# yuriyvnv/speech_transcript_embeddings

Measured on AMD Instinct MI355X. Metric: audio–text pairs/sec (whole node), 10s@16kHz + 64-tok, 1/2/4/8 MI355X, higher is better.
Workload: dtype bf16; 1 GPU; c2: global batch 64 = 1 GPU x 1 micro-batch(es) of 64 pairs, each pair 10s@16kHz audio + 64-tok clean + 64-tok corrupt; w2v-bert-2.0 Conformer 24L + XLM-R-base 12L, 3+3 unfrozen; GPU fbank -> fwd -> InfoNCE -> bwd -> allreduce -> clip+AdamW; global_batch=64, local_batch=64, micro_batch=64, accumulation_steps=1, seq_len_audio_frames=499, seq_len_text=64, parallelism=dp1

## Files before the change

### include/ste.h

```cpp
#ifndef STE_H_
#define STE_H_
#include <stdint.h>

#ifdef __cplusplus
extern "C" {
#endif

#define STE_OK 0
#define STE_ERR_ARG 1001
#define STE_ERR_SHAPE 1002

enum {
  STE_ACT_NONE = 0,
  STE_ACT_SWISH = 1,
  STE_ACT_GELU = 2,
  STE_ACT_TANH = 3,
  STE_ACT_RELU = 4,
  STE_ACT_SWISH_BWD = 11,
  STE_ACT_GELU_BWD = 12,
  STE_ACT_TANH_BWD_OUT = 13,
  STE_ACT_RELU_BWD = 14
};

typedef struct {
  int M, N, K, batch;
  const void* A; int64_t lda; int a_kc;
  const void* B; int64_t ldb; int b_kc;
  int64_t strideA, strideB, strideC, strideR;
  void* C; int64_t ldc; int c_bf16;
  void* C2; int64_t ldc2;
  void* C3; int64_t ldc3;
  const float* bias;
  const void* R; int64_t ldr; int r_bf16;
  const void* Z; int64_t ldz;
  float* colsum;
  const float* row_scale;
  float alpha, beta;
  int act;
  float drop_p; uint64_t seed; int64_t drop_ld;
  float* ws; int64_t ws_bytes;
  int c3_lo;
} ste_gemm_args;

int ste_gemm(const ste_gemm_args* args, void* stream);
int64_t ste_gemm_colsum_ws_floats(const ste_gemm_args* args);
int ste_gemm_tile_map(int t, int num_m, int num_n, int* tm, int* tn);

int ste_gemm_f32(const ste_gemm_args* args, void* stream);
int ste_gemm_f32_plan(const ste_gemm_args* args);
int ste_gemm_f32_plan_slab(const ste_gemm_args* args);
int64_t ste_gemm_f32_ws_floats(const ste_gemm_args* args);
int ste_gemm_f32_plan_tile(const ste_gemm_args* args);
int ste_gemm_f32_plan_max_tiles(int tiles);
int ste_gemm_f32_plan_small_tiles(int tiles);

#define STE_GEMM_KERNEL_SMALL 0
#define STE_GEMM_KERNEL_8PH 8
#define STE_GEMM_KERNEL_SPLITK 12
int ste_gemm_kernel(const ste_gemm_args* args);
int ste_gemm_kernel_name(const ste_gemm_args* args, char* buf, int len);

int ste_gemm_mx8(const ste_gemm_args* args, const void* a_scales, const void* b_scales, void* q_out, void* q_scales,
                 void* stream);
int ste_gemm_mx8_kernel(const ste_gemm_args* args, int q_out);
int ste_gemm_plan_min_tiles(int bf16_tiles, int mx8_tiles, int* prev_bf16, int* prev_mx8);
int ste_mx8_quant(const void* x, int64_t ldx, int rows, int K, void* q, void* scales, void* stream);

typedef struct {
  int rows, cols;
  const void* x; int64_t ldx; int x_bf16;
  const float* gamma; const float* beta; float eps;
  float* y; int64_t ldy;
  void* yb; int64_t ldyb;
  float* mean; float* rstd;
  const float* row_scale;
  int act;
  float drop_p; uint64_t seed;
  void* q8; void* q8s; int64_t ldq8;
  void* ylo; int64_t ldylo;
} ste_ln_fwd_args;
int ste_layernorm_fwd(const ste_ln_fwd_args* a, void* stream);

typedef struct {
  int rows, cols;
  const void* dy; int64_t lddy; int dy_bf16;
  const void* x; int64_t ldx; int x_bf16;
  const float* mean; const float* rstd;
  const float* gamma; const float* beta;
  const float* row_scale;
  int act;
  const float* dres; int64_t lddres;
  float* dx; int64_t lddx;
  void* dxb; int64_t lddxb;
  float* dgamma; float* dbeta;
  float drop_p; uint64_t seed; float out_scale;
  float in_drop_p; uint64_t in_seed;
  const float* out_row_scale;
  float* dsum;
  float* ws; int64_t ws_floats;
} ste_ln_bwd_args;
int ste_layernorm_bwd(const ste_ln_bwd_args* a, void* stream);
int64_t ste_layernorm_bwd_ws_floats(int rows, int cols);

int ste_layernorm_fwd_pair(const ste_ln_fwd_args* a, const ste_ln_fwd_args* b, void* stream);
int ste_layernorm_bwd_pair(const ste_ln_bwd_args* a, const ste_ln_bwd_args* b, void* stream);

typedef struct {
  int B, T, H;
  const void* q; int64_t ldq;
  const void* k; int64_t ldk;
  const void* v; int64_t ldv;
  void* o; int64_t ldo;
  float* lse;
  const int32_t* key_mask;
  const void* rel_E; int rel_left, rel_right;
  float scale;
  float drop_p; uint64_t seed;
  const void* dout; int64_t lddo;
  void* dq; int64_t lddq;
  void* dk; int64_t lddk;
  void* dv; int64_t lddv;
  float* delta;
  float* dE;
  float* gwork;
  void* o_lo; int64_t ldolo;
  int zero_masked_rows;
} ste_attn_args;
int ste_attention_fwd(const ste_attn_args* a, void* stream);
int ste_attention_fwd_f32(const ste_attn_args* a, float* o32, int64_t ldo32, void* stream);
int ste_attention_bwd(const ste_attn_args* a, void* stream);
int ste_attention_bwd_f32(const ste_attn_args* a, void* stream);

int ste_glu_dwconv_fwd(const void* pre, const float* w, void* out, int B, int T, int C, int K, void* stream);
int ste_glu_dwconv_bwd(const void* pre, const float* w, const void* dout, void* dpre, float* dw,
                       int B, int T, int C, int K, float* ws, int64_t ws_floats, void* stream);
int64_t ste_glu_dwconv_bwd_ws_floats(int B, int T, int C, int K);

int ste_fbank(const float* wav, int64_t ld_wav, const int32_t* lengths, int B, int Tmax, float pad_value,
              float* feats, int64_t* mask, int mask_mode, float* work, void* stream);

int ste_resample_plan(int sr_in, int sr_out, int* M, int* L, int* K);
int ste_resample_table(int sr_in, int sr_out, float* table, int64_t table_floats);
int ste_resample_tile(int M, int L, int K);
int ste_resample(const float* wav, int64_t ld_wav, const int32_t* lengths, int B, int M, int L, int K,
                 const float* table, float* out, int64_t ld_out, int n_out_max, int32_t* out_lengths, void* stream);

int ste_attn_pool_fwd(const void* t, const float* w2, const float* b2, const void* h, const int32_t* mask,
                      int B, int L, int Hh, int H, float* weights, float* pooled, void* pooled_bf16,
                      void* stream);
int ste_attn_pool_bwd_work_floats(int B, int L, int Hh);
int ste_attn_pool_bwd(const void* t, const float* w2, const void* h, const float* weights, const float* dpooled,
                      const int32_t* mask, int B, int L, int Hh, int H, float* dh, void* dt, void* dt_lo, float* dw2,
                      float* db2,
                      float* db1, float* work, void* stream);
int ste_attn_pool_fwd_f32(const float* t, const float* w2, const float* b2, const float* h, const int32_t* mask,
                          int B, int L, int Hh, int H, float* weights, float* pooled, void* pooled_bf16, void* stream);
int ste_attn_pool_bwd_f32(const float* t, const float* w2, const float* h, const float* weights, const float* dpooled,
                          const int32_t* mask, int B, int L, int Hh, int H, float* dh, float* dt, float* dw2,
                          float* db2, float* db1, float* work, void* stream);

int ste_mean_pool_fwd(const void* h, const int32_t* mask, int B, int L, int H, int cls, float* weights, float* pooled,
                      void* pooled_bf16, void* stream);
int ste_mean_pool_fwd_f32(const float* h, const int32_t* mask, int B, int L, int H, int cls, float* weights,
                          float* pooled, void* pooled_bf16, void* stream);
int ste_weighted_pool_bwd(const float* weights, const float* dpooled, int B, int L, int H, float* dh, void* stream);

int ste_xattn1_fwd(const float* q, const void* k, const void* v, int64_t ldkv, const int32_t* mask, int B, int S,
                   int P, int nh, float scale, float drop_p, uint64_t seed, float* probs, float* out, void* stream);
int ste_xattn1_bwd(const float* q, const void* k, const void* v, int64_t ldkv, const float* probs, const float* dout,
                   const int32_t* mask, int B, int S, int P, int nh, float scale, float drop_p, uint64_t seed,
                   float* dq, float* dk, float* dv, int64_t lddkv, void* stream);
int ste_xattn_fwd(const float* q, const void* k, const void* v, int64_t ldkv, const int32_t* mask, int B, int S, int P,
                  int nh, int nq, float scale, float drop_p, uint64_t seed0, uint64_t seed1, float* probs, float* out,
                  void* stream);
int ste_xattn_bwd(const float* q, const void* k, const void* v, int64_t ldkv, const float* probs, const float* dout,
                  const int32_t* mask, int B, int S, int P, int nh, int nq, float scale, float drop_p,
                  uint64_t seed0, uint64_t seed1, float* dq, float* dk, float* dv, int64_t lddkv, void* stream);
int ste_xattn_mq_fwd(const float* q, const int32_t* qrow, const void* k, const void* v, int64_t ldkv,
                     const int32_t* mask, int B, int C, int S, int P, int nh, float scale, float* out, void* stream);
int ste_xattn_gather_fwd(const float* q, const int32_t* qrow, const void* k, const void* v, int64_t ldkv,
                         const int32_t* kvblk, const int32_t* mask, int R, int S, int P, int nh, float scale,
                         float* out, void* stream);
int ste_xattn_bwd_bf16(const float* q, const void* k, const void* v, int64_t ldkv, const float* probs,
                       const float* dout, const int32_t* mask, int B, int S, int P, int nh, int nq, float scale,
                       float drop_p,
                       uint64_t seed0, uint64_t seed1, float* dq, void* dk, void* dv, int64_t lddkv,
                       float* colsum_part, void* stream);

int ste_align_attn_fwd(const void* q, int64_t ldq, const void* kv, int64_t ldkv, const int32_t* kmask, int B, int L,
                       int T, int P, int nh, float drop_p, uint64_t seed, float* probs, void* out, int64_t ldo,
                       void* stream);
int ste_align_attn_bwd(const void* q, int64_t ldq, const void* kv, int64_t ldkv, const float* probs,
                       const void* dout, int64_t lddo, int B, int L, int T, int P, int nh, float drop_p,
                       uint64_t seed, float* dsbuf, void* dq, int64_t lddq, float* dkv, int64_t lddkv, void* stream);
int ste_rank1_bwd(const float* a, const float* w, const void* z, int M, int K, int act, void* out, float* dw,
                  float* db, void* stream);

int ste_l2norm_fwd(const float* x, int rows, int cols, float* y, float* norms, void* stream);
int ste_l2norm_bwd(const float* y, const float* norms, const float* dy, int rows, int cols, float* dx,
                   void* stream);
int ste_similarity(const float* a, const float* t, int B, int NT, int P, float* S, void* stream);
int ste_pair_loss_fwd(const float* S, int64_t ldS, int off_neg, const float* align, int B, int L, float tau,
                      float aw, float gamma, float* s_pos, float* s_neg, float* loss, void* stream);
int ste_pair_loss_bwd(const float* s_pos, const float* s_neg, const float* align, int B, int L, float tau,
                      float aw, float gamma, const float* gscale, float* ds_pos, float* ds_neg, float* dalign,
                      void* stream);

int ste_pair_metrics(const float* S, int64_t ldS, int NB, int off_neg, float tau, const float* losses, int nloss,
                     float loss_w, double* acc, void* stream);
int ste_inbatch_ce(const float* S, int64_t ldS, int B, int NB, int row0, float tau, float weight, const float* gscale,
                   float* loss, float* dS, int64_t lddS, void* stream);
int ste_rowmat_f32(const float* X, int64_t sxr, int64_t sxc, const float* Y, int R, int C, int P, float* out,
                   void* stream);
int ste_pair_sim_bwd(const float* a, const float* tp, const float* tn, const float* ds_pos, const float* ds_neg,
                     int B, int P, float* da, float* dtp, float* dtn, void* stream);

int ste_text_embed_fwd(const int64_t* ids, int B, int L, int D, int pad_idx, const float* word, const float* pos,
                       const float* type0, float* out, int32_t* pos_ids, void* stream);
int ste_text_embed_bwd(const int64_t* ids, const int32_t* pos_ids, const float* dout, int B, int L, int D,
                       int pad_idx, float* dword, float* dpos, float* dtype0, float* ws, int64_t ws_floats,
                       void* stream);
int64_t ste_text_embed_bwd_ws_floats(int B, int L, int D);

int ste_rows_extract(const int64_t* ids, int n, int pad_idx, float* grad, int D, int32_t* flags,
                     int32_t* out_ids, float* rows, int cap, int32_t* count, void* stream);
int ste_rows_accumulate(float* grad, int D, const int32_t* ids, const float* rows, int cap, float scale,
                        void* stream);

int ste_sumsq(const float* g, int64_t n, double* acc, double* part, void* stream);
int ste_adamw(float* p, const float* g, float* m, float* v, void* p_bf16, int64_t n, float lr, float beta1,
              float beta2, float eps, float wd, int step, const double* sumsq, float max_norm, void* stream);

int ste_split_bf16(const float* x, int64_t ldx, int64_t rows, int K, void* y, int nblk, int lo_mask, void* stream);
int ste_cast_f32_bf16(const float* x, void* y, int64_t n, void* stream);
int ste_axpby2d(float* y, int64_t ldy, const float* x, int64_t ldx, int64_t rows, int cols, float alpha, float beta,
                void* stream);
int ste_copy2d(void* y, int64_t ldy, const void* x, int64_t ldx, int64_t rows, int cols, int elem_bytes,
               void* stream);
int ste_spec_mask_fwd(float* x, int64_t ld, const int32_t* spec, const float* valid, const float* embed,
                      int64_t rows, int cols, void* stream);
int ste_spec_mask_bwd(float* dx, int64_t ld, const int32_t* spec, const float* valid, float* dembed,
                      int64_t rows, int cols, float* ws, int64_t ws_floats, void* stream);
int64_t ste_spec_mask_bwd_ws_floats(int64_t rows, int cols);
int ste_transpose16(void* y, int64_t ldy, const void* x, int64_t ldx, int64_t rows, int cols, void* stream);
int ste_colsum(const void* x, int is_bf16, int64_t rows, int cols, int64_t ld, float* out, float* ws,
               int64_t ws_floats, void* stream);
int64_t ste_colsum_ws_floats(int64_t rows, int cols);
int ste_rowsum_ordered(const float* part, int64_t rows, int cols, int batch, float* out, void* stream);
int ste_scale_rows(float* x, const float* scale, int64_t rows, int cols, int64_t ld, void* stream);
int ste_mask_i64_to_f32(const int64_t* m, float* f, int32_t* i32, int64_t n, void* stream);

int ste_w2v_conv0_fwd(const float* wave, int64_t ldw, const float* w0, int B, int N, int T0, int C, int K0, int S0,
                      float* y, void* stream);
int64_t ste_w2v_gn_work(int B, int T0, int C, int K0);
int ste_w2v_gn_fwd(const float* y, const float* gamma, const float* beta, int B, int T0, int C, float eps,
                   float* mean, float* rstd, void* h, float* work, int64_t work_floats, void* stream);
int ste_w2v_gn_bwd(const float* dh, const float* y, const float* mean, const float* rstd, const float* gamma,
                   const float* beta, const float* wave, int64_t ldw, int B, int N, int T0, int C, int K0, int S0,
                   float* dgamma, float* dbeta, float* dw0, float* work, int64_t work_floats, void* stream);
int ste_w2v_slab_sum(float* out, const float* part, int64_t n, int S, void* stream);
int ste_w2v_conv_fold(const float* dcol, int64_t ldd, const void* z, int B, int Ti, int To, int C, int k, int s,
                      void* out, int out_bf16, void* stream);
int ste_w2v_perm12(const void* src, void* dst, int A, int P, int Q, int fp32_accumulate, void* stream);
int ste_w2v_pos_pack(const float* x, int B, int T, int D, int G, int K, int padl, void* out, void* stream);
int ste_w2v_pos_elem(int mode, const float* cpad, const float* bias, const float* src, const float* maskf, int B,
                     int T, int D, int Tp, float* out, void* stream);
int ste_w2v_wnorm_fwd(const float* v, const float* g, int D, int Cg, int K, float* norms, void* wr, void* wf,
                      void* stream);
int ste_w2v_wnorm_bwd(const float* dwr, const float* v, const float* g, const float* norms, int D, int Cg, int K,
                      float* dv, float* dg, void* stream);
int ste_w2v_frame_mask(const int64_t* mask, int B, int N, int Tf, int nconv, const int* kernels, const int* strides,
                       float* maskf, int32_t* mask32, void* stream);
int ste_w2v_wave_norm(const float* wave, int64_t ldw, const int32_t* lengths, int B, int N, float pad, float* out,
                      void* stream);
int ste_w2v_drop_rows(float* x, int M, int N, float p, uint64_t seed, const float* maskf, void* stream);

int ste_w2v_conv0_ln_fwd(const float* wave, int64_t ldw, const float* w0, const float* bias, const float* gamma,
                         const float* beta, int B, int N, int T0, int C, int K0, int S0, float eps, void* h,
                         float* mean, float* rstd, void* stream);
int64_t ste_w2v_conv0_ln_work(int B, int T0, int C, int K0);
int ste_w2v_conv0_ln_bwd(const float* dh, const float* wave, int64_t ldw, const float* mean, const float* rstd,
                         const float* w0, const float* bias, const float* gamma, const float* beta, int B, int N,
                         int T0, int C, int K0, int S0, float* dgamma, float* dbeta, float* dbias, float* dw0,
                         float* work, int64_t work_floats, void* stream);
int ste_w2v_ln_gelu_fwd(const void* z, const float* gamma, const float* beta, int64_t rows, int C, float eps, void* h,
                        int h_f32, float* mean, float* rstd, void* stream);
int64_t ste_w2v_ln_gelu_work(int64_t rows, int C);
int ste_w2v_ln_gelu_bwd(const void* dh, int dh_bf16, const void* z, const float* mean, const float* rstd,
                        const float* gamma, const float* beta, int64_t rows, int C, void* dz, float* dgamma,
                        float* dbeta, float* dbias, float* work, int64_t work_floats, void* stream);

int ste_topk_sim_plan(int Q, int N, int P, int k, int splits, int* splits_out, int64_t* ws_bytes);
int ste_topk_sim(const float* q, const void* corpus, int corpus_bf16, int Q, int N, int P, int k, int index_base,
                 const int32_t* target, const float* tscore, int splits, float* values, int32_t* indices,
                 int32_t* rank, void* ws, int64_t ws_bytes, void* stream);
int ste_topk_target_score(const float* q, const void* corpus, int corpus_bf16, int Q, int N, int P, int index_base,
                          const int32_t* target, float* tscore, void* stream);
int ste_topk_merge(const float* vals, const int32_t* idx, int Q, int C, int k, const int32_t* counts, int L,
                   float* out_v, int32_t* out_i, int32_t* out_rank, void* stream);

const char* ste_version(void);

#ifdef __cplusplus
}
#endif
#endif
```

### speech_transcript_embeddings_amd/_lib.py

```python
from __future__ import annotations

import ctypes as C
import os
from pathlib import Path

import torch

_PKG = Path(__file__).resolve().parent
LIB_PATH = Path(os.environ.get("STE_LIB", _PKG / "libste.so"))
AB_BUILD = LIB_PATH.name == "libste_ab.so"


def ab_env(name: str, default: str) -> str:
    return os.environ.get(name, default) if AB_BUILD else default

c_void_p, c_int, c_int64, c_float, c_uint64, c_char_p = C.c_void_p, C.c_int, C.c_int64, C.c_float, C.c_uint64, C.c_char_p
c_i32p = C.POINTER(C.c_int32)

ACT_NONE, ACT_SWISH, ACT_GELU, ACT_TANH, ACT_RELU = 0, 1, 2, 3, 4
ACT_SWISH_BWD, ACT_GELU_BWD, ACT_TANH_BWD_OUT, ACT_RELU_BWD = 11, 12, 13, 14


class GemmArgs(C.Structure):
    _fields_ = [
        ("M", c_int), ("N", c_int), ("K", c_int), ("batch", c_int),
        ("A", c_void_p), ("lda", c_int64), ("a_kc", c_int),
        ("B", c_void_p), ("ldb", c_int64), ("b_kc", c_int),
        ("strideA", c_int64), ("strideB", c_int64), ("strideC", c_int64), ("strideR", c_int64),
        ("C", c_void_p), ("ldc", c_int64), ("c_bf16", c_int),
        ("C2", c_void_p), ("ldc2", c_int64),
        ("C3", c_void_p), ("ldc3", c_int64),
        ("bias", c_void_p),
        ("R", c_void_p), ("ldr", c_int64), ("r_bf16", c_int),
        ("Z", c_void_p), ("ldz", c_int64),
        ("colsum", c_void_p),
        ("row_scale", c_void_p),
        ("alpha", c_float), ("beta", c_float),
        ("act", c_int),
        ("drop_p", c_float), ("seed", c_uint64), ("drop_ld", c_int64),
        ("ws", c_void_p), ("ws_bytes", c_int64),
        ("c3_lo", c_int),
    ]


class LnFwdArgs(C.Structure):
    _fields_ = [
        ("rows", c_int), ("cols", c_int),
        ("x", c_void_p), ("ldx", c_int64), ("x_bf16", c_int),
        ("gamma", c_void_p), ("beta", c_void_p), ("eps", c_float),
        ("y", c_void_p), ("ldy", c_int64),
        ("yb", c_void_p), ("ldyb", c_int64),
        ("mean", c_void_p), ("rstd", c_void_p),
        ("row_scale", c_void_p),
        ("act", c_int),
        ("drop_p", c_float), ("seed", c_uint64),
        ("q8", c_void_p), ("q8s", c_void_p), ("ldq8", c_int64),
        ("ylo", c_void_p), ("ldylo", c_int64),
    ]


class LnBwdArgs(C.Structure):
    _fields_ = [
        ("rows", c_int), ("cols", c_int),
        ("dy", c_void_p), ("lddy", c_int64), ("dy_bf16", c_int),
        ("x", c_void_p), ("ldx", c_int64), ("x_bf16", c_int),
        ("mean", c_void_p), ("rstd", c_void_p),
        ("gamma", c_void_p), ("beta", c_void_p),
        ("row_scale", c_void_p),
        ("act", c_int),
        ("dres", c_void_p), ("lddres", c_int64),
        ("dx", c_void_p), ("lddx", c_int64),
        ("dxb", c_void_p), ("lddxb", c_int64),
        ("dgamma", c_void_p), ("dbeta", c_void_p),
        ("drop_p", c_float), ("seed", c_uint64), ("out_scale", c_float),
        ("in_drop_p", c_float), ("in_seed", c_uint64),
        ("out_row_scale", c_void_p),
        ("dsum", c_void_p),
        ("ws", c_void_p), ("ws_floats", c_int64),
    ]


class AttnArgs(C.Structure):
    _fields_ = [
        ("B", c_int), ("T", c_int), ("H", c_int),
        ("q", c_void_p), ("ldq", c_int64),
        ("k", c_void_p), ("ldk", c_int64),
        ("v", c_void_p), ("ldv", c_int64),
        ("o", c_void_p), ("ldo", c_int64),
        ("lse", c_void_p),
        ("key_mask", c_void_p),
        ("rel_E", c_void_p), ("rel_left", c_int), ("rel_right", c_int),
        ("scale", c_float),
        ("drop_p", c_float), ("seed", c_uint64),
        ("dout", c_void_p), ("lddo", c_int64),
        ("dq", c_void_p), ("lddq", c_int64),
        ("dk", c_void_p), ("lddk", c_int64),
        ("dv", c_void_p), ("lddv", c_int64),
        ("delta", c_void_p),
        ("dE", c_void_p),
        ("gwork", c_void_p),
        ("o_lo", c_void_p), ("ldolo", c_int64),
        ("zero_masked_rows", c_int),
    ]


_SIGS = {
    "ste_gemm": (c_int, [C.POINTER(GemmArgs), c_void_p]),
    "ste_gemm_f32": (c_int, [C.POINTER(GemmArgs), c_void_p]),
    "ste_gemm_f32_plan": (c_int, [C.POINTER(GemmArgs)]),
    "ste_gemm_f32_plan_slab": (c_int, [C.POINTER(GemmArgs)]),
    "ste_gemm_f32_ws_floats": (c_int64, [C.POINTER(GemmArgs)]),
    "ste_gemm_f32_plan_max_tiles": (c_int, [c_int]),
    "ste_gemm_f32_plan_small_tiles": (c_int, [c_int]),
    "ste_gemm_f32_plan_tile": (c_int, [C.POINTER(GemmArgs)]),
    "ste_gemm_kernel": (c_int, [C.POINTER(GemmArgs)]),
    "ste_gemm_colsum_ws_floats": (c_int64, [C.POINTER(GemmArgs)]),
    "ste_gemm_tile_map": (c_int, [c_int, c_int, c_int, C.POINTER(c_int), C.POINTER(c_int)]),
    "ste_gemm_kernel_name": (c_int, [C.POINTER(GemmArgs), c_char_p, c_int]),
    "ste_rows_extract": (c_int, [c_void_p, c_int, c_int, c_void_p, c_int, c_void_p, c_void_p, c_void_p, c_int,
                                 c_void_p, c_void_p]),
    "ste_rows_accumulate": (c_int, [c_void_p, c_int, c_void_p, c_void_p, c_int, c_float, c_void_p]),
    "ste_layernorm_fwd": (c_int, [C.POINTER(LnFwdArgs), c_void_p]),
    "ste_layernorm_bwd": (c_int, [C.POINTER(LnBwdArgs), c_void_p]),
    "ste_layernorm_fwd_pair": (c_int, [C.POINTER(LnFwdArgs), C.POINTER(LnFwdArgs), c_void_p]),
    "ste_layernorm_bwd_pair": (c_int, [C.POINTER(LnBwdArgs), C.POINTER(LnBwdArgs), c_void_p]),
    "ste_layernorm_bwd_ws_floats": (c_int64, [c_int, c_int]),
    "ste_attention_fwd": (c_int, [C.POINTER(AttnArgs), c_void_p]),
    "ste_attention_bwd": (c_int, [C.POINTER(AttnArgs), c_void_p]),
    "ste_attention_fwd_f32": (c_int, [C.POINTER(AttnArgs), c_void_p, c_int64, c_void_p]),
    "ste_attention_bwd_f32": (c_int, [C.POINTER(AttnArgs), c_void_p]),
    "ste_split_bf16": (c_int, [c_void_p, c_int64, c_int64, c_int, c_void_p, c_int, c_int, c_void_p]),
    "ste_glu_dwconv_fwd": (c_int, [c_void_p, c_void_p, c_void_p, c_int, c_int, c_int, c_int, c_void_p]),
    "ste_glu_dwconv_bwd": (c_int, [c_void_p, c_void_p, c_void_p, c_void_p, c_void_p, c_int, c_int, c_int, c_int,
                                   c_void_p, c_int64, c_void_p]),
    "ste_glu_dwconv_bwd_ws_floats": (c_int64, [c_int, c_int, c_int, c_int]),
    "ste_fbank": (c_int, [c_void_p, c_int64, c_void_p, c_int, c_int, c_float, c_void_p, c_void_p, c_int, c_void_p,
                          c_void_p]),
    "ste_resample_plan": (c_int, [c_int, c_int, C.POINTER(c_int), C.POINTER(c_int), C.POINTER(c_int)]),
    "ste_resample_table": (c_int, [c_int, c_int, c_void_p, c_int64]),
    "ste_resample_tile": (c_int, [c_int, c_int, c_int]),
    "ste_resample": (c_int, [c_void_p, c_int64, c_void_p, c_int, c_int, c_int, c_int, c_void_p, c_void_p, c_int64,
                             c_int, c_void_p, c_void_p]),
    "ste_gemm_mx8": (c_int, [c_void_p, c_void_p, c_void_p, c_void_p, c_void_p, c_void_p]),
    "ste_gemm_mx8_kernel": (c_int, [C.POINTER(GemmArgs), c_int]),
    "ste_gemm_plan_min_tiles": (c_int, [c_int, c_int, C.POINTER(c_int), C.POINTER(c_int)]),
    "ste_mx8_quant": (c_int, [c_void_p, c_int64, c_int, c_int, c_void_p, c_void_p, c_void_p]),
    "ste_attn_pool_fwd": (c_int, [c_void_p, c_void_p, c_void_p, c_void_p, c_void_p, c_int, c_int, c_int, c_int,
                                  c_void_p, c_void_p, c_void_p, c_void_p]),
    "ste_attn_pool_bwd": (c_int, [c_void_p, c_void_p, c_void_p, c_void_p, c_void_p, c_void_p, c_int, c_int, c_int,
                                  c_int, c_void_p, c_void_p, c_void_p, c_void_p, c_void_p, c_void_p, c_void_p,
                                  c_void_p]),
    "ste_attn_pool_bwd_work_floats": (c_int, [c_int, c_int, c_int]),
    "ste_attn_pool_fwd_f32": (c_int, [c_void_p, c_void_p, c_void_p, c_void_p, c_void_p, c_int, c_int, c_int, c_int,
                                      c_void_p, c_void_p, c_void_p, c_void_p]),
    "ste_attn_pool_bwd_f32": (c_int, [c_void_p, c_void_p, c_void_p, c_void_p, c_void_p, c_void_p, c_int, c_int,
                                      c_int, c_int, c_void_p, c_void_p, c_void_p, c_void_p, c_void_p, c_void_p,
                                      c_void_p]),
    "ste_mean_pool_fwd": (c_int, [c_void_p, c_void_p, c_int, c_int, c_int, c_int, c_void_p, c_void_p, c_void_p,
                                  c_void_p]),
    "ste_mean_pool_fwd_f32": (c_int, [c_void_p, c_void_p, c_int, c_int, c_int, c_int, c_void_p, c_void_p, c_void_p,
                                      c_void_p]),
    "ste_weighted_pool_bwd": (c_int, [c_void_p, c_void_p, c_int, c_int, c_int, c_void_p, c_void_p]),
    "ste_xattn1_fwd": (c_int, [c_void_p, c_void_p, c_void_p, c_int64, c_void_p, c_int, c_int, c_int, c_int, c_float,
                               c_float, c_uint64, c_void_p, c_void_p, c_void_p]),
    "ste_xattn1_bwd": (c_int, [c_void_p, c_void_p, c_void_p, c_int64, c_void_p, c_void_p, c_void_p, c_int, c_int,
                               c_int, c_int, c_float, c_float, c_uint64, c_void_p, c_void_p, c_void_p, c_int64,
                               c_void_p]),
    "ste_xattn_fwd": (c_int, [c_void_p, c_void_p, c_void_p, c_int64, c_void_p, c_int, c_int, c_int, c_int, c_int,
                              c_float, c_float, c_uint64, c_uint64, c_void_p, c_void_p, c_void_p]),
    "ste_xattn_bwd": (c_int, [c_void_p, c_void_p, c_void_p, c_int64, c_void_p, c_void_p, c_void_p, c_int, c_int,
                              c_int, c_int, c_int, c_float, c_float, c_uint64, c_uint64, c_void_p, c_void_p,
                              c_void_p, c_int64, c_void_p]),
    "ste_xattn_bwd_bf16": (c_int, [c_void_p, c_void_p, c_void_p, c_int64, c_void_p, c_void_p, c_void_p, c_int,
                                   c_int, c_int, c_int, c_int, c_float, c_float, c_uint64, c_uint64, c_void_p,
                                   c_void_p, c_void_p, c_int64, c_void_p, c_void_p]),
    "ste_xattn_mq_fwd": (c_int, [c_void_p, c_void_p, c_void_p, c_void_p, c_int64, c_void_p, c_int, c_int, c_int,
                                 c_int, c_int, c_float, c_void_p, c_void_p]),
    "ste_xattn_gather_fwd": (c_int, [c_void_p, c_void_p, c_void_p, c_void_p, c_int64, c_void_p, c_void_p, c_int,
                                     c_int, c_int, c_int, c_float, c_void_p, c_void_p]),
    "ste_align_attn_fwd": (c_int, [c_void_p, c_int64, c_void_p, c_int64, c_void_p, c_int, c_int, c_int, c_int, c_int,
                                   c_float, c_uint64, c_void_p, c_void_p, c_int64, c_void_p]),
    "ste_align_attn_bwd": (c_int, [c_void_p, c_int64, c_void_p, c_int64, c_void_p, c_void_p, c_int64, c_int, c_int,
                                   c_int, c_int, c_int, c_float, c_uint64, c_void_p, c_void_p, c_int64, c_void_p,
                                   c_int64, c_void_p]),
    "ste_rank1_bwd": (c_int, [c_void_p, c_void_p, c_void_p, c_int, c_int, c_int, c_void_p, c_void_p, c_void_p,
                              c_void_p]),
    "ste_l2norm_fwd": (c_int, [c_void_p, c_int, c_int, c_void_p, c_void_p, c_void_p]),
    "ste_l2norm_bwd": (c_int, [c_void_p, c_void_p, c_void_p, c_int, c_int, c_void_p, c_void_p]),
    "ste_similarity": (c_int, [c_void_p, c_void_p, c_int, c_int, c_int, c_void_p, c_void_p]),
    "ste_pair_loss_fwd": (c_int, [c_void_p, c_int64, c_int, c_void_p, c_int, c_int, c_float, c_float, c_float,
                                  c_void_p, c_void_p, c_void_p, c_void_p]),
    "ste_pair_loss_bwd": (c_int, [c_void_p, c_void_p, c_void_p, c_int, c_int, c_float, c_float, c_float, c_void_p,
                                  c_void_p, c_void_p, c_void_p, c_void_p]),
    "ste_pair_sim_bwd": (c_int, [c_void_p, c_void_p, c_void_p, c_void_p, c_void_p, c_int, c_int, c_void_p, c_void_p,
                                 c_void_p, c_void_p]),
    "ste_pair_metrics": (c_int, [c_void_p, c_int64, c_int, c_int, c_float, c_void_p, c_int, c_float, c_void_p,
                                 c_void_p]),
    "ste_inbatch_ce": (c_int, [c_void_p, c_int64, c_int, c_int, c_int, c_float, c_float, c_void_p, c_void_p, c_void_p,
                               c_int64, c_void_p]),
    "ste_rowmat_f32": (c_int, [c_void_p, c_int64, c_int64, c_void_p, c_int, c_int, c_int, c_void_p, c_void_p]),
    "ste_text_embed_fwd": (c_int, [c_void_p, c_int, c_int, c_int, c_int, c_void_p, c_void_p, c_void_p, c_void_p,
                                   c_void_p, c_void_p]),
    "ste_text_embed_bwd": (c_int, [c_void_p, c_void_p, c_void_p, c_int, c_int, c_int, c_int, c_void_p, c_void_p,
                                   c_void_p, c_void_p, c_int64, c_void_p]),
    "ste_text_embed_bwd_ws_floats": (c_int64, [c_int, c_int, c_int]),
    "ste_sumsq": (c_int, [c_void_p, c_int64, c_void_p, c_void_p, c_void_p]),
    "ste_adamw": (c_int, [c_void_p, c_void_p, c_void_p, c_void_p, c_void_p, c_int64, c_float, c_float, c_float,
                          c_float, c_float, c_int, c_void_p, c_float, c_void_p]),
    "ste_cast_f32_bf16": (c_int, [c_void_p, c_void_p, c_int64, c_void_p]),
    "ste_colsum": (c_int, [c_void_p, c_int, c_int64, c_int, c_int64, c_void_p, c_void_p, c_int64, c_void_p]),
    "ste_colsum_ws_floats": (c_int64, [c_int64, c_int]),
    "ste_rowsum_ordered": (c_int, [c_void_p, c_int64, c_int, c_int, c_void_p, c_void_p]),
    "ste_axpby2d": (c_int, [c_void_p, c_int64, c_void_p, c_int64, c_int64, c_int, c_float, c_float, c_void_p]),
    "ste_copy2d": (c_int, [c_void_p, c_int64, c_void_p, c_int64, c_int64, c_int, c_int, c_void_p]),
    "ste_transpose16": (c_int, [c_void_p, c_int64, c_void_p, c_int64, c_int64, c_int, c_void_p]),
    "ste_spec_mask_fwd": (c_int, [c_void_p, c_int64, c_void_p, c_void_p, c_void_p, c_int64, c_int, c_void_p]),
    "ste_spec_mask_bwd": (c_int, [c_void_p, c_int64, c_void_p, c_void_p, c_void_p, c_int64, c_int, c_void_p, c_int64,
                                  c_void_p]),
    "ste_spec_mask_bwd_ws_floats": (c_int64, [c_int64, c_int]),
    "ste_scale_rows": (c_int, [c_void_p, c_void_p, c_int64, c_int, c_int64, c_void_p]),
    "ste_mask_i64_to_f32": (c_int, [c_void_p, c_void_p, c_void_p, c_int64, c_void_p]),
    "ste_w2v_conv0_fwd": (c_int, [c_void_p, c_int64, c_void_p, c_int, c_int, c_int, c_int, c_int, c_int, c_void_p,
                                  c_void_p]),
    "ste_w2v_gn_work": (c_int64, [c_int, c_int, c_int, c_int]),
    "ste_w2v_gn_fwd": (c_int, [c_void_p, c_void_p, c_void_p, c_int, c_int, c_int, c_float, c_void_p, c_void_p,
                               c_void_p, c_void_p, c_int64, c_void_p]),
    "ste_w2v_gn_bwd": (c_int, [c_void_p, c_void_p, c_void_p, c_void_p, c_void_p, c_void_p, c_void_p, c_int64, c_int,
                               c_int, c_int, c_int, c_int, c_int, c_void_p, c_void_p, c_void_p, c_void_p, c_int64,
                               c_void_p]),
    "ste_w2v_slab_sum": (c_int, [c_void_p, c_void_p, c_int64, c_int, c_void_p]),
    "ste_w2v_conv_fold": (c_int, [c_void_p, c_int64, c_void_p, c_int, c_int, c_int, c_int, c_int, c_int, c_void_p,
                                  c_int, c_void_p]),
    "ste_w2v_perm12": (c_int, [c_void_p, c_void_p, c_int, c_int, c_int, c_int, c_void_p]),
    "ste_w2v_pos_pack": (c_int, [c_void_p, c_int, c_int, c_int, c_int, c_int, c_int, c_void_p, c_void_p]),
    "ste_w2v_pos_elem": (c_int, [c_int, c_void_p, c_void_p, c_void_p, c_void_p, c_int, c_int, c_int, c_int, c_void_p,
                                 c_void_p]),
    "ste_w2v_wnorm_fwd": (c_int, [c_void_p, c_void_p, c_int, c_int, c_int, c_void_p, c_void_p, c_void_p, c_void_p]),
    "ste_w2v_wnorm_bwd": (c_int, [c_void_p, c_void_p, c_void_p, c_void_p, c_int, c_int, c_int, c_void_p, c_void_p,
                                  c_void_p]),
    "ste_w2v_frame_mask": (c_int, [c_void_p, c_int, c_int, c_int, c_int, C.POINTER(c_int), C.POINTER(c_int), c_void_p,
                                   c_void_p, c_void_p]),
    "ste_w2v_wave_norm": (c_int, [c_void_p, c_int64, c_void_p, c_int, c_int, c_float, c_void_p, c_void_p]),
    "ste_w2v_drop_rows": (c_int, [c_void_p, c_int, c_int, c_float, c_uint64, c_void_p, c_void_p]),
    "ste_w2v_conv0_ln_fwd": (c_int, [c_void_p, c_int64, c_void_p, c_void_p, c_void_p, c_void_p, c_int, c_int, c_int,
                                     c_int, c_int, c_int, c_float, c_void_p, c_void_p, c_void_p, c_void_p]),
    "ste_w2v_conv0_ln_work": (c_int64, [c_int, c_int, c_int, c_int]),
    "ste_w2v_conv0_ln_bwd": (c_int, [c_void_p, c_void_p, c_int64, c_void_p, c_void_p, c_void_p, c_void_p, c_void_p,
                                     c_void_p, c_int, c_int, c_int, c_int, c_int, c_int, c_void_p, c_void_p,
                                     c_void_p, c_void_p, c_void_p, c_int64, c_void_p]),
    "ste_w2v_ln_gelu_fwd": (c_int, [c_void_p, c_void_p, c_void_p, c_int64, c_int, c_float, c_void_p, c_int, c_void_p,
                                    c_void_p, c_void_p]),
    "ste_w2v_ln_gelu_work": (c_int64, [c_int64, c_int]),
    "ste_w2v_ln_gelu_bwd": (c_int, [c_void_p, c_int, c_void_p, c_void_p, c_void_p, c_void_p, c_void_p, c_int64, c_int,
                                    c_void_p, c_void_p, c_void_p, c_void_p, c_void_p, c_int64, c_void_p]),
    "ste_topk_sim_plan": (c_int, [c_int, c_int, c_int, c_int, c_int, C.POINTER(c_int), C.POINTER(c_int64)]),
    "ste_topk_sim": (c_int, [c_void_p, c_void_p, c_int, c_int, c_int, c_int, c_int, c_int, c_void_p, c_void_p, c_int,
                             c_void_p, c_void_p, c_void_p, c_void_p, c_int64, c_void_p]),
    "ste_topk_target_score": (c_int, [c_void_p, c_void_p, c_int, c_int, c_int, c_int, c_int, c_void_p, c_void_p,
                                      c_void_p]),
    "ste_topk_merge": (c_int, [c_void_p, c_void_p, c_int, c_int, c_int, c_void_p, c_int, c_void_p, c_void_p, c_void_p,
                               c_void_p]),
    "ste_version": (C.c_char_p, []),
}

SYMBOLS = tuple(_SIGS)
_lib = None


class SteError(RuntimeError):
    pass


def load() -> C.CDLL:
    global _lib
    if _lib is None:
        if not LIB_PATH.exists():
            raise SteError(f"{LIB_PATH} not found — build it with __graft_entry__.build() "
                           "(speech_transcript_embeddings_amd/_build.py); there is no fallback path")
        _lib = C.CDLL(str(LIB_PATH))
    return _lib


_fns: dict = {}


def fn(name: str):
    f = _fns.get(name)
    if f is None:
        f = getattr(load(), name)
        f.restype, f.argtypes = _SIGS[name]
        _fns[name] = f
    return f


def call(name: str, *args) -> None:
    rc = fn(name)(*args)
    if rc != 0:
        raise SteError(f"{name} failed with status {rc}")


def stream_ptr(device=None) -> int:
    return torch.cuda.current_stream(device).cuda_stream


def ptr(t) -> int | None:
    return None if t is None else t.data_ptr()
```

### speech_transcript_embeddings_amd/csrc/embed_optim.hip

```cpp
#include "common.h"
#include "../../include/ste.h"

namespace {

constexpr int NT = 256;

__global__ __launch_bounds__(NT) void embed_fwd_kernel(const int64_t* ids, int L, int D, int pad, const float* word,
                                                     const float* pos, const float* type0, float* out,
                                                     int32_t* pos_ids) {
  __shared__ int spos[2048];
  const int b = blockIdx.x, tid = threadIdx.x;
  if (tid == 0) {
    int c = 0;
    for (int l = 0; l < L; ++l) {
      const int nz = ids[(int64_t)b * L + l] != pad;
      c += nz;
      spos[l] = nz ? c + pad : pad;
    }
  }
  __syncthreads();
  for (int l = tid; l < L; l += NT) pos_ids[(int64_t)b * L + l] = spos[l];
  for (int i = tid * 4; i < L * D; i += NT * 4) {
    const int l = i / D, c = i % D;
    const int64_t id = ids[(int64_t)b * L + l];
    f32x4 v = *reinterpret_cast<const f32x4*>(word + id * D + c);
    v += *reinterpret_cast<const f32x4*>(pos + (int64_t)spos[l] * D + c);
    v += *reinterpret_cast<const f32x4*>(type0 + c);
    *reinterpret_cast<f32x4*>(out + ((int64_t)b * L + l) * D + c) = v;
  }
}

constexpr int EMB_WAVES = 16;
constexpr int EMB_LDS_IDS = 16384;
template <typename IdT>
__global__ __launch_bounds__(EMB_WAVES * 64) void embed_rows_ordered_kernel(const IdT* __restrict__ ids, int rows,
                                                                          int D, int pad,
                                                                          const float* __restrict__ dout,
                                                                          float* __restrict__ table) {
  extern __shared__ int sids[];
  const bool in_lds = rows <= EMB_LDS_IDS;
  if (in_lds)
    for (int i = threadIdx.x; i < rows; i += EMB_WAVES * 64) sids[i] = (int)ids[i];
  __syncthreads();
  const int lane = threadIdx.x & 63, r = blockIdx.x * EMB_WAVES + (threadIdx.x >> 6);
  if (r >= rows) return;
  auto id_at = [&](int j) { return in_lds ? sids[j] : (int)ids[j]; };
  const int id = id_at(r);
  if (id == pad || id < 0) return;
  for (int j0 = 0; j0 < r; j0 += 64) {
    const int j = j0 + lane;
    if (__ballot(j < r && id_at(j) == id)) return;
  }
  f32x4 acc[4] = {};
  for (int j0 = r; j0 < rows; j0 += 64) {
    const int j = j0 + lane;
    uint64_t m = __ballot(j < rows && id_at(j) == id);
    while (m) {
      const int k = __builtin_ctzll(m);
      m &= m - 1;
      const float* src = dout + (int64_t)(j0 + k) * D;
#pragma unroll
      for (int q = 0; q < 4; ++q) {
        const int c = (lane + 64 * q) * 4;
        if (c < D) acc[q] += *reinterpret_cast<const f32x4*>(src + c);
      }
    }
  }
  float* dst = table + (int64_t)id * D;
#pragma unroll
  for (int q = 0; q < 4; ++q) {
    const int c = (lane + 64 * q) * 4;
    if (c < D) *reinterpret_cast<f32x4*>(dst + c) += acc[q];
  }
}

__global__ __launch_bounds__(NT) void sumsq_kernel(const float* g, int64_t n, double* acc, double* part) {
  __shared__ double red[NT / 64];
  double s = 0.0;
  float sf = 0.f;
  int cnt = 0;
  for (int64_t i = ((int64_t)blockIdx.x * NT + threadIdx.x) * 4; i < n; i += (int64_t)gridDim.x * NT * 4) {
    if (i + 3 < n) {
      const f32x4 v = *reinterpret_cast<const f32x4*>(g + i);
      sf += v[0] * v[0] + v[1] * v[1] + v[2] * v[2] + v[3] * v[3];
    } else {
      for (int64_t j = i; j < n; ++j) sf += g[j] * g[j];
    }
    if (++cnt == 64) { s += sf; sf = 0.f; cnt = 0; }
  }
  s += sf;
  s = wave_sum_d(s);
  const int w = threadIdx.x >> 6, lane = threadIdx.x & 63;
  if (lane == 0) red[w] = s;
  __syncthreads();
  if (threadIdx.x == 0) {
    double t = 0.0;
    for (int i = 0; i < NT / 64; ++i) t += red[i];
    if (part) part[blockIdx.x] = t;
    else atomicAdd(acc, t);
  }
}

__global__ __launch_bounds__(64) void sumsq_final_kernel(const double* part, int nb, double* acc) {
  double t = 0.0;
  for (int b = threadIdx.x; b < nb; b += 64) t += part[b];
  t = wave_sum_d(t);
  if (threadIdx.x == 0) acc[0] += t;
}

__device__ __forceinline__ void adamw_elem(float& p, float g, float& m, float& v, float coef, float decay, float b1,
                                           float b2, float step, float bc2_sqrt, float eps) {
#pragma clang fp contract(off)
  const float gc = g * coef;
  m = __builtin_fmaf(b1, m, (1.f - b1) * gc);
  v = __builtin_fmaf(b2, v, ((1.f - b2) * gc) * gc);
  const float den = sqrtf(v) / bc2_sqrt + eps;
  p = __builtin_fmaf(-step, m / den, p * decay);
}

template <bool NTL>
__global__ __launch_bounds__(NT) void adamw_kernel(float* __restrict__ p, const float* __restrict__ g,
                                                 float* __restrict__ m, float* __restrict__ v, bf16* __restrict__ pb,
                                                 int64_t n, float lr, float b1, float b2, float eps, float wd,
                                                 float bc1, float bc2_sqrt, const double* sumsq, float max_norm) {
  float coef = 1.f;
  if (sumsq) {
    const float tn = (float)sqrt(*sumsq);
    coef = fminf(1.f, max_norm / (tn + 1e-6f));
  }
  const float step = lr / bc1;
  const float decay = 1.f - lr * wd;
  auto upd4 = [&](f32x4& pv, const f32x4& gv, f32x4& mv, f32x4& vv) {
#pragma unroll
    for (int e = 0; e < 4; ++e) {
      float pe = pv[e], me = mv[e], ve = vv[e];
      adamw_elem(pe, gv[e], me, ve, coef, decay, b1, b2, step, bc2_sqrt, eps);
      pv[e] = pe;
      mv[e] = me;
      vv[e] = ve;
    }
  };
  auto ld = [](const float* q) -> f32x4 {
    if constexpr (NTL) return __builtin_nontemporal_load(reinterpret_cast<const f32x4*>(q));
    else return *reinterpret_cast<const f32x4*>(q);
  };
  auto st = [](float* q, f32x4 x) {
    if constexpr (NTL) __builtin_nontemporal_store(x, reinterpret_cast<f32x4*>(q));
    else *reinterpret_cast<f32x4*>(q) = x;
  };
  const int64_t stride = (int64_t)gridDim.x * NT * 4;
  int64_t i = ((int64_t)blockIdx.x * NT + threadIdx.x) * 4;
  for (; i + stride + 3 < n; i += 2 * stride) {
    f32x4 pv0 = ld(p + i), pv1 = ld(p + i + stride);
    const f32x4 gv0 = ld(g + i), gv1 = ld(g + i + stride);
    f32x4 mv0 = ld(m + i), mv1 = ld(m + i + stride);
    f32x4 vv0 = ld(v + i), vv1 = ld(v + i + stride);
    upd4(pv0, gv0, mv0, vv0);
    upd4(pv1, gv1, mv1, vv1);
    st(p + i, pv0);
    st(m + i, mv0);
    st(v + i, vv0);
    st(p + i + stride, pv1);
    st(m + i + stride, mv1);
    st(v + i + stride, vv1);
    if (pb) {
      store_bf16x4(pb + i, pv0);
      store_bf16x4(pb + i + stride, pv1);
    }
  }
  for (; i < n; i += stride) {
    if (i + 3 < n) {
      f32x4 pv = *reinterpret_cast<f32x4*>(p + i);
      const f32x4 gv = *reinterpret_cast<const f32x4*>(g + i);
      f32x4 mv = *reinterpret_cast<f32x4*>(m + i);
      f32x4 vv = *reinterpret_cast<f32x4*>(v + i);
      upd4(pv, gv, mv, vv);
      *reinterpret_cast<f32x4*>(p + i) = pv;
      *reinterpret_cast<f32x4*>(m + i) = mv;
      *reinterpret_cast<f32x4*>(v + i) = vv;
      if (pb) store_bf16x4(pb + i, pv);
    } else {
      for (int64_t j = i; j < n; ++j) {
        float pv = p[j], mv = m[j], vv = v[j];
        adamw_elem(pv, g[j], mv, vv, coef, decay, b1, b2, step, bc2_sqrt, eps);
        p[j] = pv;
        m[j] = mv;
        v[j] = vv;
        if (pb) pb[j] = (bf16)pv;
      }
    }
  }
}

inline unsigned grid_for(int64_t n) {
  int64_t b = (n / 4 + NT - 1) / NT;
  if (b > 8192) b = 8192;
  return (unsigned)(b < 1 ? 1 : b);
}

}

namespace {
__global__ __launch_bounds__(NT) void rows_reset_kernel(int32_t* out_ids, int cap, int32_t* count) {
  const int i = blockIdx.x * NT + threadIdx.x;
  if (i < cap) out_ids[i] = -1;
  if (i == 0) *count = 0;
}
__global__ __launch_bounds__(NT) void rows_claim_kernel(const int64_t* ids, int n, int pad, int32_t* flags,
                                                       int32_t* out_ids, int cap, int32_t* count) {
  const int i = blockIdx.x * NT + threadIdx.x;
  if (i >= n) return;
  const int64_t id = ids[i];
  if (id == pad || id < 0) return;
  if (atomicCAS(flags + id, 0, 1) == 0) {
    const int slot = atomicAdd(count, 1);
    if (slot < cap) out_ids[slot] = (int32_t)id;
  }
}
__global__ __launch_bounds__(NT) void rows_extract_kernel(float* grad, int D, const int32_t* out_ids, int32_t* flags,
                                                         float* rows) {
  const int sidx = blockIdx.x;
  const int id = out_ids[sidx];
  float* dst = rows + (int64_t)sidx * D;
  if (id < 0) {
    for (int c = threadIdx.x * 4; c < D; c += NT * 4) *reinterpret_cast<f32x4*>(dst + c) = f32x4{0.f, 0.f, 0.f, 0.f};
    return;
  }
  float* src = grad + (int64_t)id * D;
  for (int c = threadIdx.x * 4; c < D; c += NT * 4) {
    *reinterpret_cast<f32x4*>(dst + c) = *reinterpret_cast<const f32x4*>(src + c);
    *reinterpret_cast<f32x4*>(src + c) = f32x4{0.f, 0.f, 0.f, 0.f};
  }
  if (threadIdx.x == 0) flags[id] = 0;
}
__global__ __launch_bounds__(NT) void rows_accumulate_kernel(float* grad, int D, const int32_t* ids, const float* rows,
                                                            float scale) {
  const int sidx = blockIdx.x;
  const int id = ids[sidx];
  if (id < 0) return;
  float* dst = grad + (int64_t)id * D;
  const float* src = rows + (int64_t)sidx * D;
  for (int c = threadIdx.x * 4; c < D; c += NT * 4)
    *reinterpret_cast<f32x4*>(dst + c) += *reinterpret_cast<const f32x4*>(src + c) * scale;
}
}

extern "C" int ste_rows_extract(const int64_t* ids, int n, int pad_idx, float* grad, int D, int32_t* flags,
                                int32_t* out_ids, float* rows, int cap, int32_t* count, void* stream) {
  if (n < 0 || cap <= 0 || (D & 3) || !grad || !flags || !out_ids || !rows || !count) return STE_ERR_ARG;
  hipStream_t s = (hipStream_t)stream;
  hipLaunchKernelGGL(rows_reset_kernel, dim3((cap + NT - 1) / NT), dim3(NT), 0, s, out_ids, cap, count);
  STE_CHECK_LAUNCH();
  if (n > 0) {
    hipLaunchKernelGGL(rows_claim_kernel, dim3((n + NT - 1) / NT), dim3(NT), 0, s, ids, n, pad_idx, flags, out_ids,
                       cap, count);
    STE_CHECK_LAUNCH();
  }
  hipLaunchKernelGGL(rows_extract_kernel, dim3(cap), dim3(NT), 0, s, grad, D, out_ids, flags, rows);
  STE_CHECK_LAUNCH();
  return 0;
}

extern "C" int ste_rows_accumulate(float* grad, int D, const int32_t* ids, const float* rows, int cap, float scale,
                                   void* stream) {
  if (cap <= 0 || (D & 3) || !grad || !ids || !rows) return STE_ERR_ARG;
  hipLaunchKernelGGL(rows_accumulate_kernel, dim3(cap), dim3(NT), 0, (hipStream_t)stream, grad, D, ids, rows, scale);
  STE_CHECK_LAUNCH();
  return 0;
}



extern "C" int ste_text_embed_fwd(const int64_t* ids, int B, int L, int D, int pad_idx, const float* word,
                                  const float* pos, const float* type0, float* out, int32_t* pos_ids, void* stream) {
  if (B <= 0 || L <= 0 || L > 2048 || (D & 3)) return STE_ERR_SHAPE;
  hipLaunchKernelGGL(embed_fwd_kernel, dim3(B), dim3(NT), 0, (hipStream_t)stream, ids, L, D, pad_idx, word, pos, type0,
                     out, pos_ids);
  STE_CHECK_LAUNCH();
  return 0;
}

extern "C" int64_t ste_text_embed_bwd_ws_floats(int B, int L, int D) {
  return ste_colsum_ws_floats((int64_t)B * L, D);
}

extern "C" int ste_text_embed_bwd(const int64_t* ids, const int32_t* pos_ids, const float* dout, int B, int L, int D,
                                  int pad_idx, float* dword, float* dpos, float* dtype0, float* ws, int64_t ws_floats,
                                  void* stream) {
  const int rows = B * L;
  if (rows <= 0 || (D & 3) || D > 1024) return STE_ERR_SHAPE;
  hipStream_t s = (hipStream_t)stream;
  const dim3 grid((rows + EMB_WAVES - 1) / EMB_WAVES);
  const size_t lds = rows <= EMB_LDS_IDS ? (size_t)rows * 4 : 0;
  if (dword) {
    hipLaunchKernelGGL(embed_rows_ordered_kernel<int64_t>, grid, dim3(EMB_WAVES * 64), lds, s, ids, rows, D, pad_idx,
                       dout, dword);
    STE_CHECK_LAUNCH();
  }
  if (dpos) {
    hipLaunchKernelGGL(embed_rows_ordered_kernel<int32_t>, grid, dim3(EMB_WAVES * 64), lds, s, pos_ids, rows, D,
                       pad_idx, dout, dpos);
    STE_CHECK_LAUNCH();
  }
  if (dtype0) return ste_colsum(dout, 0, rows, D, D, dtype0, ws, ws_floats, stream);
  return 0;
}

extern "C" int ste_sumsq(const float* g, int64_t n, double* acc, double* part, void* stream) {
  if (n <= 0) return 0;
  if (((uintptr_t)g) & 15) return STE_ERR_ARG;
  unsigned gr = grid_for(n);
  if (gr > 2048) gr = 2048;
  hipLaunchKernelGGL(sumsq_kernel, dim3(gr), dim3(NT), 0, (hipStream_t)stream, g, n, acc, part);
  STE_CHECK_LAUNCH();
  if (part) {
    hipLaunchKernelGGL(sumsq_final_kernel, dim3(1), dim3(64), 0, (hipStream_t)stream, part, (int)gr, acc);
    STE_CHECK_LAUNCH();
  }
  return 0;
}

extern "C" int ste_adamw(float* p, const float* g, float* m, float* v, void* p_bf16, int64_t n, float lr, float beta1,
                         float beta2, float eps, float wd, int step, const double* sumsq, float max_norm,
                         void* stream) {
  if (n <= 0) return 0;
  if (step < 1) return STE_ERR_ARG;
  if ((((uintptr_t)p) | ((uintptr_t)g) | ((uintptr_t)m) | ((uintptr_t)v)) & 15) return STE_ERR_ARG;
  if (p_bf16 && (((uintptr_t)p_bf16) & 7)) return STE_ERR_ARG;
  const float bc1 = 1.f - powf(beta1, (float)step);
  const float bc2s = sqrtf(1.f - powf(beta2, (float)step));
  const char* ent = STE_AB_ENV("STE_ADAMW_NT");
  if (!(ent && ent[0] == '0'))
    hipLaunchKernelGGL(adamw_kernel<true>, dim3(grid_for(n)), dim3(NT), 0, (hipStream_t)stream, p, g, m, v,
                       (bf16*)p_bf16, n, lr, beta1, beta2, eps, wd, bc1, bc2s, sumsq, max_norm);
  else
  hipLaunchKernelGGL(adamw_kernel<false>, dim3(grid_for(n)), dim3(NT), 0, (hipStream_t)stream, p, g, m, v, (bf16*)p_bf16, n,
                     lr, beta1, beta2, eps, wd, bc1, bc2s, sumsq, max_norm);
  STE_CHECK_LAUNCH();
  return 0;
}
```

### speech_transcript_embeddings_amd/engine.py

```python
from __future__ import annotations

import math

import torch

from . import _lib, ops
from ._lib import (ACT_GELU, ACT_GELU_BWD, ACT_NONE, ACT_RELU, ACT_RELU_BWD, ACT_SWISH, ACT_SWISH_BWD,
                   ACT_TANH)

BF16, F32 = torch.bfloat16, torch.float32
_GOLD = 0x9E3779B97F4A7C15
_M64 = (1 << 64) - 1


def _site_seed(base: int, site: int) -> int:
    x = (base + (site + 1) * _GOLD) & _M64
    x ^= x >> 31
    return (x * 0xBF58476D1CE4E5B9) & _M64


XLMR_NAMES = dict(layer="text_encoder.encoder.layer.{i}.", q="attention.self.query", o="attention.output.dense",
                  ln1="attention.output.LayerNorm", fi="intermediate.dense", fo="output.dense", ln2="output.LayerNorm")
W2V2_NAMES = dict(layer="audio_encoder.encoder.layers.{i}.", q="attention.q_proj", o="attention.out_proj",
                  ln1="layer_norm", fi="feed_forward.intermediate_dense", fo="feed_forward.output_dense",
# ... 394 lines not shown
        ap = c.attention_probs_dropout_prob if train else 0.0
        x = self._e(M, D)
        if self.precise_text:
            xb = self._e(M, 2 * D, dtype=BF16)
            st = self._ln(emb, "text_encoder.embeddings.LayerNorm", c.layer_norm_eps, y=x, yb=xb[:, :D], ylo=xb[:, D:],
                          drop_p=hp, seed=_site_seed(base_seed, 1))
        else:
            xb = self._e(M, D, dtype=BF16)
            st = self._ln(emb, "text_encoder.embeddings.LayerNorm", c.layer_norm_eps, y=x, yb=xb, drop_p=hp,
                          seed=_site_seed(base_seed, 1))
        ctx.update(t_nb=nb, t_L=L, t_mask32=mask32, t_ids=ids, t_emb=emb, t_pos=pos_ids, t_st=st, t_hp=hp, t_ap=ap,
                   t_seed=base_seed)
        layers = []
        for i in range(c.num_hidden_layers):
            x, xb, sv = self._xlmr_fwd(i, x, xb, nb, L, mask32, hp, ap, _site_seed(base_seed, 10 + i), save)
            layers.append(sv if save else None)
        ctx["t_layers"] = layers
        return x, (xb[:, :D] if self.precise_text else xb)

    def _xlmr_fwd(self, i, x, xb, nb, L, mask32, hp, ap, seed, save=True):
        if self.precise_text:
            return self._postln_fwd_x2(self.tcfg, XLMR_NAMES, i, x, xb, nb, L, mask32, hp, ap, seed, save)
        return self._postln_fwd(self.tcfg, XLMR_NAMES, i, x, xb, nb, L, mask32, hp, ap, seed, save)

    def _xlmr_bwd(self, i, sv, dx2, nb, L, mask32, hp, ap):
        if self.precise_text and self.precise_text_bwd:
            return self._postln_bwd_x2(self.tcfg, XLMR_NAMES, i, sv, dx2, nb, L, mask32, hp, ap)
        return self._postln_bwd(self.tcfg, XLMR_NAMES, i, sv, dx2, nb, L, mask32, hp, ap)

    def _postln_fwd(self, c, nm, i, x, xb, nb, L, mask32, hp, ap, seed, save=True, act_p=0.0):
        s = self.s
        pre = nm["layer"].format(i=i)
        M, D, F_ = x.shape[0], c.hidden_size, c.intermediate_size
        H = c.num_attention_heads
        eps = c.layer_norm_eps
        tr = s.trainable_layer(pre + nm["q"] + ".weight")
        sv = {"tr": tr, "seed": seed, "act_p": act_p}
        qkv = ops.linear(xb, s.fused(pre + nm["q"] + ".weight", 3, "w"), s.fused(pre + nm["q"] + ".bias", 3, "p"),
                         out_bf16=True)
        o = self._e(M, D, dtype=BF16)
        o_lo = self._e(M, D, dtype=BF16) if save else None
        lse = self._e(nb * H * L)
        ops.attention_fwd(qkv[:, :D], qkv[:, D:2 * D], qkv[:, 2 * D:], B=nb, T=L, H=H, o=o, lse=lse,
                          key_mask=mask32, scale=1.0 / math.sqrt(D // H), drop_p=ap, seed=_site_seed(seed, 1),
                          o_lo=o_lo, zero_masked_rows=True)
        y1 = ops.linear(o, s.w(pre + nm["o"] + ".weight"), s.p(pre + nm["o"] + ".bias"),
                        residual=x, drop_p=hp, seed=_site_seed(seed, 2))
        x1 = self._e(M, D)
        x1b = self._e(M, D, dtype=BF16)
        sv["st1"] = self._ln(y1, pre + nm["ln1"], eps, y=x1, yb=x1b)
        zt = self._e(M, F_, dtype=BF16) if save else None
        h = ops.linear(x1b, s.w(pre + nm["fi"] + ".weight"), s.p(pre + nm["fi"] + ".bias"),
                       act=ACT_GELU, pre_out=zt, out_bf16=True, drop_p=act_p, seed=_site_seed(seed, 4))
        y2 = ops.linear(h, s.w(pre + nm["fo"] + ".weight"), s.p(pre + nm["fo"] + ".bias"), residual=x1, drop_p=hp,
                        seed=_site_seed(seed, 3))
        x2 = self._e(M, D)
        x2b = self._e(M, D, dtype=BF16)
        sv["st2"] = self._ln(y2, pre + nm["ln2"], eps, y=x2, yb=x2b)
        sv.update(qkv=qkv, o=o, o_lo=o_lo, lse=lse, y1=y1, zt=zt, y2=y2)
        if tr:
            sv.update(xb=xb, x1b=x1b, h=h)
        return x2, x2b, sv

    def _postln_fwd_x2(self, c, nm, i, x, xs, nb, L, mask32, hp, ap, seed, save=True, act_p=0.0):
        s = self.s
        pre = nm["layer"].format(i=i)
        M, D, F_ = x.shape[0], c.hidden_size, c.intermediate_size
        H = c.num_attention_heads
        eps = c.layer_norm_eps
        tr = s.trainable_layer(pre + nm["q"] + ".weight")
        sv = {"tr": tr, "seed": seed, "act_p": act_p}
        qkvb = self._e(M, 3 * D, dtype=BF16) if (save and not self.precise_text_bwd) else None
        qkv = ops.linear(xs, s.w2(pre + nm["q"] + ".weight", 3), s.fused(pre + nm["q"] + ".bias", 3, "p"),
                         out_bf16_copy=qkvb)
        os_ = self._e(M, 2 * D, dtype=BF16)
        lse = self._e(nb * H * L)
        ops.attention_fwd_f32(qkv[:, :D], qkv[:, D:2 * D], qkv[:, 2 * D:], B=nb, T=L, H=H, o32=None, lse=lse,
                              o=os_[:, :D], o_lo=os_[:, D:], key_mask=mask32, scale=1.0 / math.sqrt(D // H),
                              drop_p=ap, seed=_site_seed(seed, 1), zero_masked_rows=True)
        y1 = ops.linear(os_, s.w2(pre + nm["o"] + ".weight"), s.p(pre + nm["o"] + ".bias"), residual=x, drop_p=hp,
                        seed=_site_seed(seed, 2))
        x1 = self._e(M, D)
        x1s = self._e(M, 2 * D, dtype=BF16)
        sv["st1"] = self._ln(y1, pre + nm["ln1"], eps, y=x1, yb=x1s[:, :D], ylo=x1s[:, D:])
        zt = self._e(M, F_, dtype=BF16) if save else None
        hs_ = self._e(M, 2 * F_, dtype=BF16)
        ops.linear(x1s, s.w2(pre + nm["fi"] + ".weight"), s.p(pre + nm["fi"] + ".bias"), act=ACT_GELU, pre_out=zt,
                   drop_p=act_p, seed=_site_seed(seed, 4), out=hs_[:, :F_], out_bf16_copy=hs_[:, F_:], copy_lo=True)
        y2 = ops.linear(hs_, s.w2(pre + nm["fo"] + ".weight"), s.p(pre + nm["fo"] + ".bias"), residual=x1, drop_p=hp,
                        seed=_site_seed(seed, 3), ws=self.ws)
        x2 = self._e(M, D)
        x2s = self._e(M, 2 * D, dtype=BF16)
        sv["st2"] = self._ln(y2, pre + nm["ln2"], eps, y=x2, yb=x2s[:, :D], ylo=x2s[:, D:])
        if save and self.precise_text_bwd:
            sv.update(qkv=qkv, os=os_, lse=lse, y1=y1, zt=zt, y2=y2)
            if tr:
                sv.update(xs=xs, x1s=x1s, hs=hs_)
        elif save:
            sv.update(qkv=qkvb, o=os_[:, :D], o_lo=os_[:, D:], lse=lse, y1=y1, zt=zt, y2=y2)
            if tr:
                sv.update(xb=xs[:, :D], x1b=x1s[:, :D], h=hs_[:, :F_])
        return x2, x2s, sv

    def _dw2(self, dys, xs, wname, fused=1):
        g = self.s.fused(wname, fused, "g")
        if g is None:
            return
        g2 = g.view(g.shape[0], -1)
        n, k = dys.shape[1] // 2, xs.shape[1] // 2
        for dy, x in ((dys[:, :n], xs[:, :k]), (dys[:, n:], xs[:, :k]), (dys[:, :n], xs[:, k:])):
            ops.linear_dw(dy, x, out=g2, beta=1.0, ws=self.ws)

    def _postln_bwd_x2(self, c, nm, i, sv, dx2, nb, L, mask32, hp, ap):
        s = self.s
        pre = nm["layer"].format(i=i)
        M, D, F_ = dx2.shape[0], c.hidden_size, c.intermediate_size
        H = c.num_attention_heads
        tr = sv["tr"]
        seed = sv["seed"]
        dy2 = self._e(M, D)
        self._ln_bwd(dx2, sv["y2"], sv["st2"], pre + nm["ln2"], dx=dy2, drop_p=hp, seed=_site_seed(seed, 3),
                     dsum=s.g(pre + nm["fo"] + ".bias"))
        dy2s = ops.split_bf16(dy2, 2, 2)
        dzs = self._e(M, 2 * F_, dtype=BF16)
        ops.linear(dy2s, s.wt2(pre + nm["fo"] + ".weight"), act=ACT_GELU_BWD, z=sv["zt"], out=dzs[:, :F_],
                   out_bf16_copy=dzs[:, F_:], copy_lo=True, colsum=s.g(pre + nm["fi"] + ".bias"),
                   drop_p=sv["act_p"], seed=_site_seed(seed, 4), ws=self.ws)
        if tr:
            self._dw2(dy2s, sv["hs"], pre + nm["fo"] + ".weight")
        del dy2s
        dx1 = ops.linear(dzs, s.wt2(pre + nm["fi"] + ".weight"), residual=dy2, ws=self.ws)
        if tr:
            self._dw2(dzs, sv["x1s"], pre + nm["fi"] + ".weight")
        del dzs, dy2
        dy1 = self._e(M, D)
        self._ln_bwd(dx1, sv["y1"], sv["st1"], pre + nm["ln1"], dx=dy1, drop_p=hp, seed=_site_seed(seed, 2),
                     dsum=s.g(pre + nm["o"] + ".bias"))
        del dx1
        dy1s = ops.split_bf16(dy1, 2, 2)
        do = ops.linear(dy1s, s.wt2(pre + nm["o"] + ".weight"), ws=self.ws)
        if tr:
            self._dw2(dy1s, sv["os"], pre + nm["o"] + ".weight")
        del dy1s
        qkv, os_ = sv["qkv"], sv["os"]
        dqkv = self._e(M, 3 * D)
        ops.attention_bwd_f32(qkv[:, :D], qkv[:, D:2 * D], qkv[:, 2 * D:], os_[:, :D], os_[:, D:], sv["lse"], do,
                              dqkv[:, :D], dqkv[:, D:2 * D], dqkv[:, 2 * D:], B=nb, T=L, H=H, key_mask=mask32,
                              scale=1.0 / math.sqrt(D // H), drop_p=ap, seed=_site_seed(seed, 1),
                              zero_masked_rows=True)
        del do
        if tr:
            self._db(dqkv, pre + nm["q"] + ".bias", fused=3)
        dqkvs = ops.split_bf16(dqkv, 2, 2)
        del dqkv
        dx0 = ops.linear(dqkvs, s.wt2(pre + nm["q"] + ".weight", 3), residual=dy1, ws=self.ws)
        if tr:
            self._dw2(dqkvs, sv["xs"], pre + nm["q"] + ".weight", fused=3)
        return dx0

    def _postln_bwd(self, c, nm, i, sv, dx2, nb, L, mask32, hp, ap):
        s = self.s
        pre = nm["layer"].format(i=i)
        M, D = dx2.shape[0], c.hidden_size
        H = c.num_attention_heads
        tr = sv["tr"]
        seed = sv["seed"]
        dy2 = self._e(M, D)
        dy2b = self._e(M, D, dtype=BF16)
        self._ln_bwd(dx2, sv["y2"], sv["st2"], pre + nm["ln2"], dx=dy2, dxb=dy2b, drop_p=hp,
                     seed=_site_seed(seed, 3), dsum=s.g(pre + nm["fo"] + ".bias"))
        dzt = self._dx(dy2b, pre + nm["fo"] + ".weight", act=ACT_GELU_BWD, z=sv["zt"], out_bf16=True,
                       colsum=s.g(pre + nm["fi"] + ".bias"), drop_p=sv["act_p"], seed=_site_seed(seed, 4))
        if tr:
            self._dw(dy2b, sv["h"], pre + nm["fo"] + ".weight")
        del dy2b
        dx1 = self._dx(dzt, pre + nm["fi"] + ".weight", residual=dy2)
        if tr:
            self._dw(dzt, sv["x1b"], pre + nm["fi"] + ".weight")
        del dzt, dy2
        dy1 = self._e(M, D)
        dy1b = self._e(M, D, dtype=BF16)
        self._ln_bwd(dx1, sv["y1"], sv["st1"], pre + nm["ln1"], dx=dy1, dxb=dy1b, drop_p=hp,
                     seed=_site_seed(seed, 2), dsum=s.g(pre + nm["o"] + ".bias"))
        del dx1
        do = self._dx(dy1b, pre + nm["o"] + ".weight", out_bf16=True)
        if tr:
            self._dw(dy1b, sv["o"], pre + nm["o"] + ".weight")
        del dy1b
        qkv = sv["qkv"]
        dqkv = self._e(M, 3 * D, dtype=BF16)
        delta = self._e(nb * H * L)
        ops.attention_bwd(qkv[:, :D], qkv[:, D:2 * D], qkv[:, 2 * D:], sv["o"], sv["lse"], do, dqkv[:, :D],
                          dqkv[:, D:2 * D], dqkv[:, 2 * D:], B=nb, T=L, H=H, delta=delta, key_mask=mask32,
                          scale=1.0 / math.sqrt(D // H), drop_p=ap, seed=_site_seed(seed, 1), o_lo=sv["o_lo"])
        del do, delta
        dx0 = self._dx(dqkv, pre + nm["q"] + ".weight", 3, residual=dy1)
        if tr:
            self._dw(dqkv, sv["xb"], pre + nm["q"] + ".weight", fused=3)
            self._db(dqkv, pre + nm["q"] + ".bias", fused=3)
        return dx0

    def _preln_fwd(self, c, nm, i, x, nb, L, mask32, hp, ap, seed, save=True, act_p=0.0):
        s = self.s
        pre = nm["layer"].format(i=i)
        M, D, F_ = x.shape[0], c.hidden_size, c.intermediate_size
        H = c.num_attention_heads
        eps = c.layer_norm_eps
        tr = s.trainable_layer(pre + nm["q"] + ".weight")
        sv = {"tr": tr, "seed": seed, "act_p": act_p}
        a1 = self._e(M, D, dtype=BF16)
        sv["st1"] = self._ln(x, pre + nm["ln1"], eps, yb=a1)
        qkv = ops.linear(a1, s.fused(pre + nm["q"] + ".weight", 3, "w"), s.fused(pre + nm["q"] + ".bias", 3, "p"),
                         out_bf16=True)
        o = self._e(M, D, dtype=BF16)
        o_lo = self._e(M, D, dtype=BF16) if save else None
        lse = self._e(nb * H * L)
        ops.attention_fwd(qkv[:, :D], qkv[:, D:2 * D], qkv[:, 2 * D:], B=nb, T=L, H=H, o=o, lse=lse,
                          key_mask=mask32, scale=1.0 / math.sqrt(D // H), drop_p=ap, seed=_site_seed(seed, 1),
                          o_lo=o_lo, zero_masked_rows=True)
        x1 = ops.linear(o, s.w(pre + nm["o"] + ".weight"), s.p(pre + nm["o"] + ".bias"),
                        residual=x, drop_p=hp, seed=_site_seed(seed, 2))
        a2 = self._e(M, D, dtype=BF16)
        sv["st2"] = self._ln(x1, pre + nm["ln2"], eps, yb=a2)
        zt = self._e(M, F_, dtype=BF16) if save else None
        h = ops.linear(a2, s.w(pre + nm["fi"] + ".weight"), s.p(pre + nm["fi"] + ".bias"),
                       act=ACT_GELU, pre_out=zt, out_bf16=True, drop_p=act_p, seed=_site_seed(seed, 4))
        x2 = ops.linear(h, s.w(pre + nm["fo"] + ".weight"), s.p(pre + nm["fo"] + ".bias"), residual=x1, drop_p=hp,
                        seed=_site_seed(seed, 3))
        sv.update(qkv=qkv, o=o, o_lo=o_lo, lse=lse, x=x, x1=x1, zt=zt)
        if tr:
            sv.update(a1=a1, a2=a2, h=h)
        return x2, sv

    def _preln_out_grad(self, c, nm, i, sv, hp):
        pre = nm["layer"].format(i=i)
        M, D = sv["x"].shape
        return dict(dxb=self._e(M, D, dtype=BF16), drop_p=hp, seed=_site_seed(sv["seed"], 3),
                    dsum=self.s.g(pre + nm["fo"] + ".bias"))

    def _preln_bwd(self, c, nm, i, sv, dx2, dx2b, nb, L, mask32, hp, ap, below=None):
        s = self.s
        pre = nm["layer"].format(i=i)
        M, D = dx2.shape[0], c.hidden_size
        H = c.num_attention_heads
        tr = sv["tr"]
        seed = sv["seed"]
        dzt = self._dx(dx2b, pre + nm["fo"] + ".weight", act=ACT_GELU_BWD, z=sv["zt"], out_bf16=True,
                       colsum=s.g(pre + nm["fi"] + ".bias"), drop_p=sv["act_p"], seed=_site_seed(seed, 4))
        if tr:
            self._dw(dx2b, sv["h"], pre + nm["fo"] + ".weight")
        da2 = self._dx(dzt, pre + nm["fi"] + ".weight", out_bf16=True)
        if tr:
            self._dw(dzt, sv["a2"], pre + nm["fi"] + ".weight")
        del dzt
        dx1 = self._e(M, D)
        dx1b = self._e(M, D, dtype=BF16)
        self._ln_bwd(da2, sv["x1"], sv["st2"], pre + nm["ln2"], dres=dx2, dx=dx1, dxb=dx1b, drop_p=hp,
                     seed=_site_seed(seed, 2), dsum=s.g(pre + nm["o"] + ".bias"))
        del da2
        do = self._dx(dx1b, pre + nm["o"] + ".weight", out_bf16=True)
        if tr:
            self._dw(dx1b, sv["o"], pre + nm["o"] + ".weight")
        del dx1b
        qkv = sv["qkv"]
        dqkv = self._e(M, 3 * D, dtype=BF16)
        delta = self._e(nb * H * L)
        ops.attention_bwd(qkv[:, :D], qkv[:, D:2 * D], qkv[:, 2 * D:], sv["o"], sv["lse"], do, dqkv[:, :D],
                          dqkv[:, D:2 * D], dqkv[:, 2 * D:], B=nb, T=L, H=H, delta=delta, key_mask=mask32,
                          scale=1.0 / math.sqrt(D // H), drop_p=ap, seed=_site_seed(seed, 1), o_lo=sv["o_lo"])
        del do, delta
        da1 = self._dx(dqkv, pre + nm["q"] + ".weight", 3, out_bf16=True)
        if tr:
            self._dw(dqkv, sv["a1"], pre + nm["q"] + ".weight", fused=3)
            self._db(dqkv, pre + nm["q"] + ".bias", fused=3)
        del dqkv
        dx0 = self._e(M, D)
        self._ln_bwd(da1, sv["x"], sv["st1"], pre + nm["ln1"], dres=dx1, dx=dx0, **(below or {}))
        return dx0

    def text_backward(self, dh, ctx, layers_done=None):
        c = self.tcfg
        s = self.s
        nb, L = ctx["t_nb"], ctx["t_L"]
        lo = next((i for i in range(c.num_hidden_layers)
                   if s.trainable_layer(XLMR_NAMES["layer"].format(i=i) + XLMR_NAMES["q"] + ".weight")), None)
        if lo is None and layers_done is not None:
            layers_done()
        dx = dh
        for i in reversed(range(c.num_hidden_layers)):
            dx = self._xlmr_bwd(i, ctx["t_layers"][i], dx, nb, L, ctx["t_mask32"], ctx["t_hp"], ctx["t_ap"])
            ctx["t_layers"][i] = None
            if i == lo and layers_done is not None:
                layers_done()
        gw = s.g("text_encoder.embeddings.word_embeddings.weight")
        gp = s.g("text_encoder.embeddings.position_embeddings.weight")
        gt = s.g("text_encoder.embeddings.token_type_embeddings.weight")
        ln_needed = any(g is not None for g in (gw, gp, gt, s.g("text_encoder.embeddings.LayerNorm.weight")))
        if not ln_needed:
            return
        demb = self._e(dx.shape[0], c.hidden_size)
        self._ln_bwd(dx, ctx["t_emb"], ctx["t_st"], "text_encoder.embeddings.LayerNorm", dx=demb,
                     in_drop_p=ctx["t_hp"], in_seed=_site_seed(ctx["t_seed"], 1))
        if gw is not None or gp is not None or gt is not None:
            ops.text_embed_bwd(ctx["t_ids"], ctx["t_pos"], demb, c.pad_token_id, gw, gp, gt)

    def _w32(self, name):
        w = self.s.p(name)
        return w.view(w.shape[0], -1)

    def _dw32(self, dy, x, wname):
        g = self.s.g(wname)
        if g is not None:
            ops.linear_dw(dy, x, out=g.view(g.shape[0], -1), beta=1.0, ws=self.ws)

    def _db32(self, dy, bname):
        g = self.s.g(bname)
        if g is not None:
            ops.colsum(dy, g)

    def _proj_fwd(self, name, x, rows, train, seed, sv):
        s = self.s
        p_drop = self.m.dropout if train else 0.0
        zp = self._e(rows, s.slots[name + ".projection.0.weight"].shape[0])
        h = ops.linear(x, self._w32(name + ".projection.0.weight"), s.p(name + ".projection.0.bias"), act=ACT_GELU,
                       pre_out=zp, drop_p=p_drop, seed=seed)
        y = ops.linear(h, self._w32(name + ".projection.3.weight"), s.p(name + ".projection.3.bias"))
        out = self._e(rows, y.shape[1])
        st = self._ln(y, name + ".projection.4", 1e-5, y=out)
        sv.update(x=x, zp=zp, h=h, y=y, st=st, p=p_drop, seed=seed)
        return out

    def _proj_bwd(self, name, sv, dout, dx_out):
        s = self.s
        dy = self._e(*dout.shape)
        self._ln_bwd(dout, sv["y"], sv["st"], name + ".projection.4", dx=dy, dsum=s.g(name + ".projection.3.bias"))
        dz = ops.linear_dx(dy, self._w32(name + ".projection.3.weight"), act=ACT_GELU_BWD, z=sv["zp"], drop_p=sv["p"],
                           seed=sv["seed"], colsum=s.g(name + ".projection.0.bias"))
        self._dw32(dy, sv["h"], name + ".projection.3.weight")
        ops.linear_dx(dz, self._w32(name + ".projection.0.weight"), out=dx_out, beta=1.0)
        self._dw32(dz, sv["x"], name + ".projection.0.weight")

    def _pool_fwd(self, name, h, hb, mask32, nb, L, sv, hs=None):
        s = self.s
        H = h.shape[1]
        w = self._e(nb * L)
        pooled = self._e(nb, H)
        if not self.m.use_attentive_pooling:
            ops.mean_pool_fwd(h, mask32, nb, L, name == "text_pooling", w, pooled)
            sv.update(w=w)
            return pooled
        f32 = name == "text_pooling" or hb is None or hs is not None
        w2, b2 = s.p(name + ".attention.2.weight").view(-1), s.p(name + ".attention.2.bias")
        if f32:
            if hs is not None:
                t = ops.linear(hs, s.w2(name + ".attention.0.weight"), s.p(name + ".attention.0.bias"), act=ACT_TANH)
            else:
                t = ops.linear(h, self._w32(name + ".attention.0.weight"), s.p(name + ".attention.0.bias"),
                               act=ACT_TANH)
            ops.attn_pool_fwd_f32(t, w2, b2, h, mask32, nb, L, w, pooled)
            sv.update(hs=hs)
        else:
            t = ops.linear(hb, s.w(name + ".attention.0.weight"), s.p(name + ".attention.0.bias"), act=ACT_TANH,
                           out_bf16=True)
            ops.attn_pool_fwd(t, w2, b2, hb, mask32, nb, L, w, pooled)
        sv.update(t=t, w=w, h=h if f32 else hb, mask=mask32, f32=f32)
        return pooled

    def _pool_bwd(self, name, sv, dpooled, dh, nb, L):
        s = self.s
        if not self.m.use_attentive_pooling:
            ops.weighted_pool_bwd(sv["w"], dpooled, nb, L, dh)
            return
        t = sv["t"]
        gw1 = s.g(name + ".attention.0.weight")
        gw2 = s.g(name + ".attention.2.weight")
        w2 = s.p(name + ".attention.2.weight").view(-1)
        dw2 = None if gw2 is None else gw2.view(-1)
        if sv["f32"]:
            dz = self._e(*t.shape)
            ops.attn_pool_bwd_f32(t, w2, sv["h"], sv["w"], dpooled, nb, L, dh, dz, dw2, s.g(name + ".attention.2.bias"),
                                  db1=s.g(name + ".attention.0.bias"), mask=sv["mask"])
            hs = sv.get("hs")
            if hs is None:
                ops.linear_dx(dz, self._w32(name + ".attention.0.weight"), out=dh, beta=1.0)
                self._dw32(dz, sv["h"], name + ".attention.0.weight")
                return
            Hh, D = t.shape[1], hs.shape[1] // 2
            dzs = ops.split_bf16(dz, 2, 2)
            ops.linear_dx(dzs[:, :Hh], s.w(name + ".attention.0.weight"), out=dh, beta=1.0)
            if gw1 is not None:
                self._dw(dzs[:, :Hh], hs[:, :D], name + ".attention.0.weight")
                self._dw(dzs[:, Hh:], hs[:, :D], name + ".attention.0.weight")
                self._dw(dzs[:, :Hh], hs[:, D:], name + ".attention.0.weight")
            return
        dz = self._e(*t.shape, dtype=BF16)
        dz_lo = self._e(*t.shape, dtype=BF16) if gw1 is not None else None
        ops.attn_pool_bwd(t, w2, sv["h"], sv["w"], dpooled, nb, L, dh, dz, dw2, s.g(name + ".attention.2.bias"),
                          db1=s.g(name + ".attention.0.bias"), dz_lo=dz_lo, mask=sv["mask"])
        ops.linear_dx(dz, s.w(name + ".attention.0.weight"), out=dh, beta=1.0)
        self._dw(dz, sv["h"], name + ".attention.0.weight")
        if dz_lo is not None:
            self._dw(dz_lo, sv["h"], name + ".attention.0.weight")

    def _xq_fwd(self, name, qin, kv, mask32, B, S, seeds, p_x):
        s = self.s
        rows, P = qin.shape
        nh = self.m.xattn_heads
        q = ops.linear(qin, self._w32(name + ".query.weight"), s.p(name + ".query.bias"))
        probs = self._e(rows * nh * S)
        att = self._e(rows, P)
        ops.xattn_fwd(q, kv[:, :P], kv[:, P:], mask32, B, S, nh, probs, att, seeds, drop_p=p_x)
        cat = self._e(rows, 2 * P)
        ops.linear(att, self._w32(name + ".out_proj.weight"), s.p(name + ".out_proj.bias"), out=cat[:, P:])
        ops.copy2d(cat[:, :P], qin)
        return cat, dict(qin=qin, q=q, probs=probs, att=att, cat=cat, kv=kv, mask=mask32, B=B, S=S, seeds=seeds, p=p_x)

    def _xq_bwd(self, name, xs, dcat, d_qin, dkvb):
        s = self.s
        P = d_qin.shape[1]
        datt = dcat[:, P:]
        _add_(d_qin, dcat[:, :P])
        dq_in = ops.linear_dx(datt, self._w32(name + ".out_proj.weight"))
        self._dw32(datt, xs["att"], name + ".out_proj.weight")
        self._db32(datt, name + ".out_proj.bias")
        dq = self._e(*xs["q"].shape)
        kv = xs["kv"]
        ops.xattn_bwd(xs["q"], kv[:, :P], kv[:, P:], xs["probs"], dq_in, xs["B"], xs["S"], self.m.xattn_heads, dq,
                      dkvb[:, :P], dkvb[:, P:], xs["seeds"], drop_p=xs["p"],
                      colsum=s.fused(name + ".key.bias", 2, "g") if dkvb.dtype == BF16 else None, mask=xs["mask"])
        ops.linear_dx(dq, self._w32(name + ".query.weight"), out=d_qin, beta=1.0)
        self._dw32(dq, xs["qin"], name + ".query.weight")
        self._db32(dq, name + ".query.bias")

    def _kv_src_bwd(self, name, src, dkvb, seqb, xb, dx):
        s = self.s
        if dkvb.dtype == F32:
            P2 = dkvb.shape[1]
            dkvs = ops.split_bf16(dkvb, 2, 2)
            self._db(dkvb, name + ".key.bias", fused=2)
            self._dw(dkvs[:, :P2], seqb, name + ".key.weight", fused=2)
            self._dw(dkvs[:, P2:], seqb, name + ".key.weight", fused=2)
            dseq = ops.linear(dkvs, s.wt2(name + ".key.weight", 2), colsum=s.g(src + ".bias"))
            P = dseq.shape[1]
            dseqs = ops.split_bf16(dseq, 2, 2)
            self._dw(dseqs[:, :P], xb, src + ".weight")
            self._dw(dseqs[:, P:], xb, src + ".weight")
            ops.linear(dseqs, s.wt2(src + ".weight"), out=dx, beta=1.0)
            return
        dseqb = self._dx(dkvb, name + ".key.weight", 2, out_bf16=True, colsum=s.g(src + ".bias"))
        self._dw(dkvb, seqb, name + ".key.weight", fused=2)
        self._dx(dseqb, src + ".weight", out=dx, beta=1.0)
        self._dw(dseqb, xb, src + ".weight")

    def _fuse_fwd(self, name, cat):
        y = ops.linear(cat, self._w32(name + ".0.weight"), self.s.p(name + ".0.bias"))
        out = self._e(*y.shape)
        st = self._ln(y, name + ".1", 1e-5, y=out)
        return out, (y, st, cat)

    def _fuse_bwd(self, name, d_out, saved):
        y, st, cat = saved
        dy = self._e(*d_out.shape)
        self._ln_bwd(d_out, y, st, name + ".1", dx=dy, dsum=self.s.g(name + ".0.bias"))
        dcat = ops.linear_dx(dy, self._w32(name + ".0.weight"))
        self._dw32(dy, cat, name + ".0.weight")
        return dcat

    def _kv(self, name, src, xb):
        s = self.s
        seqb = ops.linear(xb, s.w(src + ".weight"), s.p(src + ".bias"), out_bf16=True)
        kv = ops.linear(seqb, s.fused(name + ".key.weight", 2, "w"), s.fused(name + ".key.bias", 2, "p"), out_bf16=True)
        return kv, seqb

    def heads_forward(self, th, thb, ah, ahb, train, base_seed, ctx):
        self._await_params("late", "text")
        m = self.m
        nb, L = ctx["t_nb"], ctx["t_L"]
        b = nb // 2
        ab, T = ctx["a_b"], ctx["a_T"]
        hs = {}
        tpool_sv, apool_sv, tproj_sv, aproj_sv = {}, {}, {}, {}
        tpooled = self._pool_fwd("text_pooling", th, thb, ctx["t_mask32"], nb, L, tpool_sv)
        apooled = self._pool_fwd("audio_pooling", ah, ahb, ctx["a_mask32"], ab, T, apool_sv, hs=ctx.get("a_hs"))
        tproj = self._proj_fwd("text_projection", tpooled, nb, train, _site_seed(base_seed, 201), tproj_sv)
        aproj = self._proj_fwd("audio_projection", apooled, ab, train, _site_seed(base_seed, 202), aproj_sv)
        hs.update(tpool=tpool_sv, apool=apool_sv, tproj=tproj_sv, aproj=aproj_sv)
        if m.use_cross_modal:
            p_x = m.dropout if train else 0.0
            kva, aseqb = self._kv("text_to_audio_attention", "audio_seq_to_projection", ahb)
            seed_t = _site_seed(base_seed, 203)
            tcat, hs["tx"] = self._xq_fwd("text_to_audio_attention", tproj, kva, ctx["a_mask32"], b, T,
                                          (_site_seed(seed_t, 0), _site_seed(seed_t, 1)), p_x)
            kvt, tseqb = self._kv("audio_to_text_attention", "text_seq_to_projection", thb[: b * L])
            acat, hs["ax"] = self._xq_fwd("audio_to_text_attention", aproj[:b], kvt, ctx["t_mask32"][: b * L], b, L,
                                          (_site_seed(base_seed, 204),), p_x)
            tfused, hs["tf"] = self._fuse_fwd("text_fusion", tcat)
            afused, hs["af"] = self._fuse_fwd("audio_fusion", acat)
            hs.update(aseqb=aseqb, tseqb=tseqb)
        else:
            tfused, afused = tproj, aproj[:b]
        align = None
        if m.use_word_alignment:
            align = self._align_fwd(th, thb[: b * L], ahb, b, L, T, ctx, train, _site_seed(base_seed, 205), hs)
        ctx["heads"] = hs
        return tfused, afused, align

    def heads_backward(self, d_tfused, d_afused, d_align, ctx, dth, dah):
        m = self.m
        hs = ctx["heads"]
        nb, L = ctx["t_nb"], ctx["t_L"]
        b = nb // 2
        ab, T = ctx["a_b"], ctx["a_T"]
        P = m.projection_dim
        d_tproj = self._z(nb, P)
        d_aproj = self._z(ab, P)
        if d_align is not None and m.use_word_alignment:
            self._align_bwd(d_align, hs, ctx, dth, dah)
        if m.use_cross_modal:
            dtcat = self._fuse_bwd("text_fusion", d_tfused, hs["tf"])
            dacat = self._fuse_bwd("audio_fusion", d_afused, hs["af"])
            dkvb = self._e(ab * T, 2 * P, dtype=BF16)
            self._xq_bwd("text_to_audio_attention", hs["tx"], dtcat, d_tproj, dkvb)
            self._kv_src_bwd("text_to_audio_attention", "audio_seq_to_projection", dkvb, hs["aseqb"], ctx["_ahb"],
                             dah)
            del dkvb
            dkvtb = self._e(b * L, 2 * P, dtype=BF16)
            self._xq_bwd("audio_to_text_attention", hs["ax"], dacat, d_aproj[:b], dkvtb)
            self._kv_src_bwd("audio_to_text_attention", "text_seq_to_projection", dkvtb, hs["tseqb"],
                             ctx["_thb"][: b * L], dth[: b * L])
        else:
            _add_(d_tproj, d_tfused)
            _add_(d_aproj[:b], d_afused)
        dtpooled = self._z(nb, self.tcfg.hidden_size)
        dapooled = self._z(ab, self.acfg.hidden_size)
        self._proj_bwd("text_projection", hs["tproj"], d_tproj, dtpooled)
        self._proj_bwd("audio_projection", hs["aproj"], d_aproj, dapooled)
        self._pool_bwd("text_pooling", hs["tpool"], dtpooled, dth, nb, L)
        self._pool_bwd("audio_pooling", hs["apool"], dapooled, dah, ab, T)

    def _mask32(self, mask_i64, n):
        m = self._e(n, dtype=torch.int32)
        _lib.call("ste_mask_i64_to_f32", mask_i64.contiguous().data_ptr(), None, m.data_ptr(), n, _lib.stream_ptr())
        return m

    def cross_forward(self, tproj, th, tmask, aproj, ah, amask, train, seed):
        m = self.m
        b, L, Ht = th.shape
        T, Ha = ah.shape[1], ah.shape[2]
        p_x = m.dropout if train else 0.0
        thb = ops.cast_bf16(th.contiguous(), self._e(b * L, Ht, dtype=BF16))
        ahb = ops.cast_bf16(ah.contiguous(), self._e(b * T, Ha, dtype=BF16))
        tm32 = self._mask32(tmask, b * L) if tmask is not None else None
        if amask is not None and self.raw_audio and amask.shape[-1] != T:
            from .wav2vec2 import frame_mask
            am32 = frame_mask(self.acfg, amask, b, amask.shape[-1], T, self.s.device)[1]
        else:
            am32 = self._mask32(amask, b * T) if amask is not None else None
        kva, aseqb = self._kv("text_to_audio_attention", "audio_seq_to_projection", ahb)
        tcat, tx = self._xq_fwd("text_to_audio_attention", tproj.float().contiguous(), kva, am32, b, T,
                                (_site_seed(seed, 1),), p_x)
        kvt, tseqb = self._kv("audio_to_text_attention", "text_seq_to_projection", thb)
        acat, ax = self._xq_fwd("audio_to_text_attention", aproj.float().contiguous(), kvt, tm32, b, L,
                                (_site_seed(seed, 2),), p_x)
        tfused, tf = self._fuse_fwd("text_fusion", tcat)
        afused, af = self._fuse_fwd("audio_fusion", acat)
        sv = dict(b=b, L=L, T=T, thb=thb, ahb=ahb, aseqb=aseqb, tseqb=tseqb, tx=tx, ax=ax, tf=tf, af=af)
        return tfused, afused, sv

    @torch.no_grad()
    def score_pairs(self, tproj, th, tmask, aproj, ah, amask, candidates, audio_context=None):
        m, dev = self.m, self.s.device
        U, L, Ht = th.shape
        B, T, Ha = ah.shape
        P = m.projection_dim
        cand = candidates.to(dev, torch.int32).contiguous()
        if cand.dim() != 2 or cand.shape[0] != B or cand.shape[1] < 1:
            raise ValueError(f"candidates must be [{B}, C >= 1], got {tuple(cand.shape)}")
        C = cand.shape[1]
        lo, hi = (int(x) for x in torch.stack((cand.min(), cand.max())).tolist())
        if lo < -1 or hi >= U:
            raise ValueError(f"candidates must lie in [-1, {U}), got [{lo}, {hi}]")
        if audio_context is not None and not 0 <= int(audio_context) < C:
            raise ValueError(f"audio_context must be a column of candidates, got {audio_context}")
        R = B * C
        slot = cand.view(-1)
        tproj, aproj = tproj.float().contiguous(), aproj.float().contiguous()
        scores = torch.full((R,), float("-inf"), device=dev, dtype=F32)

        def unit(x):
            y = self._e(*x.shape)
            ops.l2norm_fwd(x, y, self._e(x.shape[0]))
            return y

        arep = torch.arange(B, device=dev, dtype=torch.int32).repeat_interleave(C)
        if not m.use_cross_modal:
            ops.topk_target_score(unit(aproj).index_select(0, arep.long()), unit(tproj), slot, scores)
            return scores.view(B, C)
        nh = m.xattn_heads
        thb = ops.cast_bf16(th.contiguous(), self._e(U * L, Ht, dtype=BF16))
        ahb = ops.cast_bf16(ah.contiguous(), self._e(B * T, Ha, dtype=BF16))
        tm32 = self._mask32(tmask, U * L) if tmask is not None else None
        if amask is not None and self.raw_audio and amask.shape[-1] != T:
            from .wav2vec2 import frame_mask
            am32 = frame_mask(self.acfg, amask, B, amask.shape[-1], T, dev)[1]
        else:
            am32 = self._mask32(amask, B * T) if amask is not None else None
        kva, _ = self._kv("text_to_audio_attention", "audio_seq_to_projection", ahb)
# ... 132 lines not shown
```

### speech_transcript_embeddings_amd/ops.py

```python
from __future__ import annotations

import ctypes as C
import os

import torch

from . import _lib
from ._lib import GemmArgs, LnFwdArgs, LnBwdArgs, AttnArgs, ptr, call, fn

BF16 = torch.bfloat16
F32 = torch.float32


def _s():
    return _lib.stream_ptr()


def _ld(t: torch.Tensor) -> int:
    assert t.dim() >= 2 and t.stride(-1) == 1, "row-major operand required"
    return t.stride(-2)


ATOMIC_SUMS = _lib.ab_env("STE_ATOMIC_SUMS", "0") == "1"
_WS = {}
# ... 412 lines not shown
def fbank(wav, lengths, Tmax, *, pad_value=1.0, mask_mode=0, feats=None, mask=None, work=None):
    B = wav.shape[0]
    dev = wav.device
    if feats is None:
        feats = torch.empty((B, Tmax, 160), device=dev, dtype=F32)
    if mask is None:
        mask = torch.empty((B, Tmax), device=dev, dtype=torch.int64)
    if work is None:
        work = torch.empty(B * 2 * Tmax * 80 + B * 160, device=dev, dtype=F32)
    nbytes = 4 * B * wav.shape[1] + _nb(feats) + _nb(mask)
    _traced("fbank", nbytes, lambda: call("ste_fbank", ptr(wav), wav.stride(0), ptr(lengths), B, Tmax,
                                          float(pad_value), ptr(feats), ptr(mask), int(mask_mode), ptr(work), _s()))
    return feats, mask


def resample_plan(sr_in, sr_out=16000):
    M, L, K = C.c_int(), C.c_int(), C.c_int()
    call("ste_resample_plan", int(sr_in), int(sr_out), C.byref(M), C.byref(L), C.byref(K))
    return M.value, L.value, K.value


def resampled_length(n, sr_in, sr_out=16000):
    if sr_in == sr_out:
        return int(n)
    M, L, _ = resample_plan(sr_in, sr_out)
    return (int(n) * L + M - 1) // M


def resample_tile(sr_in, sr_out=16000):
    return fn("ste_resample_tile")(*resample_plan(sr_in, sr_out))


_RESAMPLE_TABLES = {}


def _resample_table(sr_in, sr_out, dev):
    key = (int(sr_in), int(sr_out), dev)
    t = _RESAMPLE_TABLES.get(key)
    if t is None:
        _, L, K = resample_plan(sr_in, sr_out)
        host = torch.empty(L * K, dtype=F32)
        call("ste_resample_table", int(sr_in), int(sr_out), host.data_ptr(), host.numel())
        t = _RESAMPLE_TABLES[key] = host.to(dev)
    return t


def resample(wav, lengths, sr_in, sr_out=16000, *, out=None):
    if int(sr_in) == int(sr_out):
        return wav, lengths
    M, L, K = resample_plan(sr_in, sr_out)
    B, N = wav.shape
    dev = wav.device
    if not wav.is_cuda or lengths.device != dev or lengths.shape != (B,):
        raise ValueError("resample expects wav [B, N] and lengths [B] on the same GPU")
    assert wav.dtype == F32 and wav.stride(1) == 1 and lengths.dtype == torch.int32 and lengths.is_contiguous()
    if out is None:
        out = torch.empty((B, (N * L + M - 1) // M), device=dev, dtype=F32)
    assert out.device == dev and out.dtype == F32 and out.shape[0] == B and (out.shape[1] <= 1 or out.stride(1) == 1)
    if B == 0 or N == 0 or out.shape[1] == 0:
        return out.zero_(), torch.zeros(B, device=dev, dtype=torch.int32)
    out_lengths = torch.empty(B, device=dev, dtype=torch.int32)
    table = _resample_table(sr_in, sr_out, dev)
    call("ste_resample", ptr(wav), wav.stride(0), ptr(lengths), B, M, L, K, ptr(table), ptr(out),
         out.stride(0), out.shape[1], ptr(out_lengths), _s())
    return out, out_lengths


def attn_pool_fwd(t, w2, b2, h, mask, B, L, weights, pooled, pooled_bf16=None):
    call("ste_attn_pool_fwd", ptr(t), ptr(w2), ptr(b2), ptr(h), ptr(mask), B, L, t.shape[-1], h.shape[-1],
         ptr(weights), ptr(pooled), ptr(pooled_bf16), _s())


def attn_pool_fwd_f32(t, w2, b2, h, mask, B, L, weights, pooled, pooled_bf16=None):
    assert t.dtype == F32 and h.dtype == F32
    call("ste_attn_pool_fwd_f32", ptr(t), ptr(w2), ptr(b2), ptr(h), ptr(mask), B, L, t.shape[-1], h.shape[-1],
         ptr(weights), ptr(pooled), ptr(pooled_bf16), _s())


def attn_pool_bwd_f32(t, w2, h, weights, dpooled, B, L, dh, dz, dw2=None, db2=None, db1=None, mask=None):
    assert t.dtype == F32 and h.dtype == F32 and dz.dtype == F32
    nwork = fn("ste_attn_pool_bwd_work_floats")(B, L, t.shape[-1])
    if nwork < 0:
        raise _lib.SteError(f"ste_attn_pool_bwd_work_floats failed with status {nwork}")
    work = torch.empty(nwork, device=t.device, dtype=F32)
    call("ste_attn_pool_bwd_f32", ptr(t), ptr(w2), ptr(h), ptr(weights), ptr(dpooled), ptr(mask), B, L, t.shape[-1],
         h.shape[-1], ptr(dh), ptr(dz), ptr(dw2), ptr(db2), ptr(db1), ptr(work), _s())


def attn_pool_bwd(t, w2, h, weights, dpooled, B, L, dh, dz, dw2=None, db2=None, db1=None, dz_lo=None, mask=None):
    nwork = fn("ste_attn_pool_bwd_work_floats")(B, L, t.shape[-1])
    if nwork < 0:
        raise _lib.SteError(f"ste_attn_pool_bwd_work_floats failed with status {nwork}")
    work = torch.empty(nwork, device=t.device, dtype=F32)
    call("ste_attn_pool_bwd", ptr(t), ptr(w2), ptr(h), ptr(weights), ptr(dpooled), ptr(mask), B, L, t.shape[-1],
         h.shape[-1], ptr(dh), ptr(dz), ptr(dz_lo), ptr(dw2), ptr(db2), ptr(db1), ptr(work), _s())


def mean_pool_fwd(h, mask, B, L, cls, weights, pooled, pooled_bf16=None):
    if h.dtype == F32:
        call("ste_mean_pool_fwd_f32", ptr(h), ptr(mask), B, L, h.shape[-1], int(bool(cls)), ptr(weights), ptr(pooled),
             ptr(pooled_bf16), _s())
        return
    call("ste_mean_pool_fwd", ptr(h), ptr(mask), B, L, h.shape[-1], int(bool(cls)), ptr(weights), ptr(pooled),
         ptr(pooled_bf16), _s())


def weighted_pool_bwd(weights, dpooled, B, L, dh):
    call("ste_weighted_pool_bwd", ptr(weights), ptr(dpooled), B, L, dh.shape[-1], ptr(dh), _s())


def xattn1_fwd(q, k, v, mask, B, S, nh, probs, out, drop_p=0.0, seed=0):
    P = q.shape[-1]
    call("ste_xattn1_fwd", ptr(q), ptr(k), ptr(v), _ld(k), ptr(mask), B, S, P, nh, float((P // nh) ** -0.5),
         float(drop_p), int(seed) & (2**64 - 1), ptr(probs), ptr(out), _s())


def xattn1_bwd(q, k, v, probs, dout, B, S, nh, dq, dk, dv, drop_p=0.0, seed=0, colsum=None, mask=None):
    if dk.dtype == BF16:
        return xattn_bwd(q, k, v, probs, dout, B, S, nh, dq, dk, dv, (seed,), drop_p=drop_p, colsum=colsum,
                         mask=mask)
    P = q.shape[-1]
    assert _ld(dk) == _ld(dv)
    call("ste_xattn1_bwd", ptr(q), ptr(k), ptr(v), _ld(k), ptr(probs), ptr(dout), ptr(mask), B, S, P, nh,
         float((P // nh) ** -0.5), float(drop_p), int(seed) & (2**64 - 1), ptr(dq), ptr(dk), ptr(dv), _ld(dk), _s())


def xattn_fwd(q, k, v, mask, B, S, nh, probs, out, seeds, drop_p=0.0):
    P = q.shape[-1]
    nq = len(seeds)
    assert q.shape[0] == nq * B and out.shape[0] == nq * B and probs.numel() >= nq * B * nh * S
    call("ste_xattn_fwd", ptr(q), ptr(k), ptr(v), _ld(k), ptr(mask), B, S, P, nh, nq, float((P // nh) ** -0.5),
         float(drop_p), int(seeds[0]) & (2**64 - 1), int(seeds[-1]) & (2**64 - 1), ptr(probs), ptr(out), _s())


def xattn_mq_fwd(q, qrow, k, v, mask, B, C, S, nh, out):
    P = q.shape[-1]
    assert q.dtype == F32 and q.is_contiguous() and qrow.dtype == torch.int32 and qrow.numel() == B * C
    assert k.dtype == BF16 and v.dtype == BF16 and _ld(k) == _ld(v) and k.shape[0] >= B * S
    assert out.dtype == F32 and out.is_contiguous() and out.shape == (B * C, P)
    assert mask is None or (mask.dtype == torch.int32 and mask.numel() == B * S)
    call("ste_xattn_mq_fwd", ptr(q), ptr(qrow), ptr(k), ptr(v), _ld(k), ptr(mask), B, C, S, P, nh,
         float((P // nh) ** -0.5), ptr(out), _s())


def xattn_gather_fwd(q, qrow, k, v, kvblk, mask, R, S, nh, out):
    P = q.shape[-1]
    assert q.dtype == F32 and q.is_contiguous() and out.dtype == F32 and out.shape == (R, P) and out.is_contiguous()
    assert qrow.dtype == torch.int32 and kvblk.dtype == torch.int32 and qrow.numel() == R and kvblk.numel() == R
    assert k.dtype == BF16 and v.dtype == BF16 and _ld(k) == _ld(v)
    assert mask is None or mask.dtype == torch.int32
    call("ste_xattn_gather_fwd", ptr(q), ptr(qrow), ptr(k), ptr(v), _ld(k), ptr(kvblk), ptr(mask), R, S, P, nh,
         float((P // nh) ** -0.5), ptr(out), _s())


def xattn_bwd(q, k, v, probs, dout, B, S, nh, dq, dk, dv, seeds, drop_p=0.0, colsum=None, mask=None):
    P = q.shape[-1]
    nq = len(seeds)
    assert _ld(dk) == _ld(dv) and q.shape[0] == nq * B and dq.shape[0] == nq * B and dout.shape[0] == nq * B
    if dk.dtype == BF16:
        assert dv.dtype == BF16
        part = torch.empty(B, 2 * P, device=q.device, dtype=F32)
        call("ste_xattn_bwd_bf16", ptr(q), ptr(k), ptr(v), _ld(k), ptr(probs), ptr(dout), ptr(mask), B, S, P, nh, nq,
             float((P // nh) ** -0.5), float(drop_p), int(seeds[0]) & (2**64 - 1), int(seeds[-1]) & (2**64 - 1),
             ptr(dq), ptr(dk), ptr(dv), _ld(dk), ptr(part), _s())
        if colsum is not None:
            w = _red_ws(q.device, int(fn("ste_colsum_ws_floats")(B, 2 * P)))
            call("ste_colsum", ptr(part), 0, B, 2 * P, 2 * P, ptr(colsum), *_ws_args(w), _s())
        return
    assert colsum is None
    call("ste_xattn_bwd", ptr(q), ptr(k), ptr(v), _ld(k), ptr(probs), ptr(dout), ptr(mask), B, S, P, nh, nq,
         float((P // nh) ** -0.5), float(drop_p), int(seeds[0]) & (2**64 - 1), int(seeds[-1]) & (2**64 - 1),
         ptr(dq), ptr(dk), ptr(dv), _ld(dk), _s())


def align_attn_fwd(q, kv, kmask, B, L, T, nh, probs, out, drop_p=0.0, seed=0):
    P = kv.shape[-1] // 2
    call("ste_align_attn_fwd", ptr(q), _ld(q), ptr(kv), _ld(kv), ptr(kmask), B, L, T, P, nh, float(drop_p),
         int(seed) & (2**64 - 1), ptr(probs), ptr(out), _ld(out), _s())


def align_attn_bwd(q, kv, probs, dout, B, L, T, nh, dsbuf, dq, dkv, drop_p=0.0, seed=0):
    P = kv.shape[-1] // 2
    call("ste_align_attn_bwd", ptr(q), _ld(q), ptr(kv), _ld(kv), ptr(probs), ptr(dout), _ld(dout), B, L, T, P, nh,
         float(drop_p), int(seed) & (2**64 - 1), ptr(dsbuf), ptr(dq), _ld(dq), ptr(dkv), _ld(dkv), _s())


def rank1_bwd(a, w, z, act, out, dw=None, db=None):
    M, K = z.shape
    call("ste_rank1_bwd", ptr(a), ptr(w), ptr(z), M, K, int(act), ptr(out), ptr(dw), ptr(db), _s())


def l2norm_fwd(x, y, norms):
    call("ste_l2norm_fwd", ptr(x), x.shape[0], x.shape[1], ptr(y), ptr(norms), _s())


def l2norm_bwd(y, norms, dy, dx):
    call("ste_l2norm_bwd", ptr(y), ptr(norms), ptr(dy), y.shape[0], y.shape[1], ptr(dx), _s())


def similarity(a, t, S):
    call("ste_similarity", ptr(a), ptr(t), a.shape[0], t.shape[0], a.shape[1], ptr(S), _s())


def topk_sim_plan(Q, N, P, k, splits=0):
    s, b = C.c_int(), C.c_int64()
    call("ste_topk_sim_plan", int(Q), int(N), int(P), int(k), int(splits), C.byref(s), C.byref(b))
    return s.value, b.value


def _corpus(corpus, P):
    if corpus.dtype not in (F32, BF16):
        raise TypeError(f"corpus must be fp32 or bf16, got {corpus.dtype}")
    if corpus.dim() != 2 or corpus.shape[1] != P or not corpus.is_contiguous():
        raise ValueError(f"corpus must be contiguous [N, {P}], got {tuple(corpus.shape)}")
    return int(corpus.dtype == BF16)


def topk_sim(q, corpus, k, *, index_base=0, target=None, tscore=None, splits=0):
    Q, P = q.shape
    assert q.dtype == F32 and q.is_contiguous()
    bf = _corpus(corpus, P)
    N = corpus.shape[0]
    _, ws_bytes = topk_sim_plan(Q, N, P, k, splits)
    dev = q.device
    values = torch.empty(Q, k, device=dev, dtype=F32)
    indices = torch.empty(Q, k, device=dev, dtype=torch.int32)
    ranks = None
    if target is not None:
        assert target.dtype == torch.int32 and target.shape == (Q,) and target.is_contiguous()
        assert tscore is None or (tscore.dtype == F32 and tscore.shape == (Q,) and tscore.is_contiguous())
        ranks = torch.empty(Q, device=dev, dtype=torch.int32)
    ws = torch.empty(ws_bytes, device=dev, dtype=torch.uint8)
    call("ste_topk_sim", ptr(q), ptr(corpus), bf, Q, N, P, int(k), int(index_base), ptr(target), ptr(tscore),
         int(splits), ptr(values), ptr(indices), ptr(ranks), ptr(ws), ws_bytes, _s())
    return (values, indices) if ranks is None else (values, indices, ranks)


def topk_target_score(q, corpus, target, tscore, *, index_base=0):
    Q, P = q.shape
    bf = _corpus(corpus, P)
    call("ste_topk_target_score", ptr(q), ptr(corpus), bf, Q, corpus.shape[0], P, int(index_base), ptr(target),
         ptr(tscore), _s())
    return tscore


def topk_merge(values, indices, k, counts=None):
    Q, Cn = values.shape
    assert values.dtype == F32 and indices.dtype == torch.int32 and indices.shape == values.shape
    values, indices = values.contiguous(), indices.contiguous()
    ov = torch.empty(Q, k, device=values.device, dtype=F32)
    oi = torch.empty(Q, k, device=values.device, dtype=torch.int32)
    ranks, L = None, 0
    if counts is not None:
        assert counts.dtype == torch.int32 and counts.shape[0] == Q
        counts, L = counts.contiguous(), counts.shape[1]
        ranks = torch.empty(Q, device=values.device, dtype=torch.int32)
    call("ste_topk_merge", ptr(values), ptr(indices), Q, Cn, int(k), ptr(counts), L, ptr(ov), ptr(oi), ptr(ranks), _s())
    return (ov, oi) if ranks is None else (ov, oi, ranks)


def pair_loss_fwd(S, off_neg, align, B, L, tau, aw, gamma, s_pos, s_neg, loss):
    call("ste_pair_loss_fwd", ptr(S), _ld(S), off_neg, ptr(align), B, L, float(tau), float(aw), float(gamma),
         ptr(s_pos), ptr(s_neg), ptr(loss), _s())


def pair_loss_bwd(s_pos, s_neg, align, B, L, tau, aw, gamma, gscale, ds_pos, ds_neg, dalign=None):
    call("ste_pair_loss_bwd", ptr(s_pos), ptr(s_neg), ptr(align), B, L, float(tau), float(aw), float(gamma),
         ptr(gscale), ptr(ds_pos), ptr(ds_neg), ptr(dalign), _s())


def pair_sim_bwd(a, tp, tn, ds_pos, ds_neg, da, dtp, dtn):
    call("ste_pair_sim_bwd", ptr(a), ptr(tp), ptr(tn), ptr(ds_pos), ptr(ds_neg), a.shape[0], a.shape[1], ptr(da),
         ptr(dtp), ptr(dtn), _s())


def pair_metrics(S, off_neg, tau, acc, losses=None, loss_w=1.0):
    call("ste_pair_metrics", ptr(S), _ld(S), S.shape[0], int(off_neg), float(tau), ptr(losses),
         0 if losses is None else losses.numel(), float(loss_w), ptr(acc), _s())


def inbatch_ce(S, B, NB, row0, tau, weight, gscale, loss, dS):
    call("ste_inbatch_ce", ptr(S), _ld(S), B, NB, int(row0), float(tau), float(weight), ptr(gscale), ptr(loss),
         ptr(dS), _ld(dS), _s())


def rowmat(X, Y, out, transpose_x=False):
    if transpose_x:
        C, R = X.shape
        sxr, sxc = X.stride(1), X.stride(0)
    else:
        R, C = X.shape
        sxr, sxc = X.stride(0), X.stride(1)
    assert Y.shape[0] == C and Y.is_contiguous() and out.shape == (R, Y.shape[1]) and out.is_contiguous()
    call("ste_rowmat_f32", ptr(X), sxr, sxc, ptr(Y), R, C, Y.shape[1], ptr(out), _s())
    return out


def text_embed_fwd(ids, pad_idx, word, pos, type0, out, pos_ids):
    B, L = ids.shape
    call("ste_text_embed_fwd", ptr(ids), B, L, word.shape[1], pad_idx, ptr(word), ptr(pos), ptr(type0), ptr(out),
         ptr(pos_ids), _s())


def text_embed_bwd(ids, pos_ids, dout, pad_idx, dword, dpos, dtype0):
    B, L = ids.shape
    ws = _red_ws(dout.device, int(fn("ste_text_embed_bwd_ws_floats")(B, L, dout.shape[-1]))) if dtype0 is not None \
        else None
    call("ste_text_embed_bwd", ptr(ids), ptr(pos_ids), ptr(dout), B, L, dout.shape[-1], pad_idx, ptr(dword),
         ptr(dpos), ptr(dtype0), *_ws_args(ws), _s())


SUMSQ_PARTS = 2048


def sumsq(g, acc, part=None):
    if ATOMIC_SUMS:
        part = None
    assert part is None or (part.dtype == torch.float64 and part.numel() >= SUMSQ_PARTS)
    _traced("sumsq", 4 * g.numel(), lambda: call("ste_sumsq", ptr(g), g.numel(), ptr(acc), ptr(part), _s()))


def adamw(p, g, m, v, p_bf16, *, lr, beta1, beta2, eps, wd, step, sumsq_acc=None, max_norm=1.0):
    nbytes = p.numel() * (28 + (2 if p_bf16 is not None else 0))
    _traced("adamw", nbytes, lambda: call("ste_adamw", ptr(p), ptr(g), ptr(m), ptr(v), ptr(p_bf16), p.numel(), float(lr),
                                          float(beta1), float(beta2), float(eps), float(wd), int(step), ptr(sumsq_acc),
                                          float(max_norm), _s()))


def cast_bf16(x, y):
    call("ste_cast_f32_bf16", ptr(x), ptr(y), x.numel(), _s())
    return y


def axpby(y, x, alpha=1.0, beta=1.0):
    y2 = y if y.dim() == 2 else y.view(1, -1)
    x2 = x if x.dim() == 2 else x.view(1, -1)
    assert y2.shape == x2.shape and y.dtype == F32 and x.dtype == F32
    call("ste_axpby2d", ptr(y2), _ld(y2), ptr(x2), _ld(x2), y2.shape[0], y2.shape[1], float(alpha), float(beta), _s())
    return y


def copy2d(dst, src):
    assert dst.shape == src.shape and dst.dtype == src.dtype
    d2 = dst if dst.dim() == 2 else dst.view(1, -1)
    s2 = src if src.dim() == 2 else src.view(1, -1)
    call("ste_copy2d", ptr(d2), _ld(d2), ptr(s2), _ld(s2), d2.shape[0], d2.shape[1], dst.element_size(), _s())
    return dst


def spec_mask_fwd(x, spec, valid, embed):
    call("ste_spec_mask_fwd", ptr(x), _ld(x), ptr(spec), ptr(valid), ptr(embed), x.shape[0], x.shape[1], _s())


def spec_mask_bwd(dx, spec, valid, dembed=None):
    ws = _red_ws(dx.device, int(fn("ste_spec_mask_bwd_ws_floats")(dx.shape[0], dx.shape[1]))) if dembed is not None \
        else None
    call("ste_spec_mask_bwd", ptr(dx), _ld(dx), ptr(spec), ptr(valid), ptr(dembed), dx.shape[0], dx.shape[1],
         *_ws_args(ws), _s())


def transpose16(src, dst=None):
    assert src.dim() == 2 and src.stride(1) == 1 and src.element_size() == 2
    rows, cols = src.shape
    if dst is None:
        dst = torch.empty(cols, rows, device=src.device, dtype=src.dtype)
    assert dst.shape == (cols, rows) and dst.stride(1) == 1 and dst.dtype == src.dtype
    call("ste_transpose16", ptr(dst), _ld(dst), ptr(src), _ld(src), rows, cols, _s())
    return dst


def colsum(x, out):
    ws = _red_ws(x.device, int(fn("ste_colsum_ws_floats")(x.shape[0], x.shape[1])))
    call("ste_colsum", ptr(x), int(x.dtype == BF16), x.shape[0], x.shape[1], _ld(x), ptr(out), *_ws_args(ws), _s())
    return out


def rows_extract(ids, pad_idx, grad2d, flags, out_ids, rows, count):
    assert ids.dtype == torch.int64 and grad2d.dtype == F32 and rows.shape[0] == out_ids.numel()
    call("ste_rows_extract", ptr(ids), ids.numel(), int(pad_idx), ptr(grad2d), grad2d.shape[1], ptr(flags),
         ptr(out_ids), ptr(rows), out_ids.numel(), ptr(count), _s())


def rows_accumulate(grad2d, ids, rows, scale):
    call("ste_rows_accumulate", ptr(grad2d), grad2d.shape[1], ptr(ids), ptr(rows), ids.numel(), float(scale), _s())
```

### speech_transcript_embeddings_amd/store.py

```python
from __future__ import annotations

from dataclasses import dataclass

import torch

from . import ops

ALIGN = 8


def _fuse_groups(names):
    groups = {}
    sets = [("attention.self.query", "attention.self.key", "attention.self.value"),
            ("self_attn.linear_q", "self_attn.linear_k", "self_attn.linear_v"),
            ("attention.q_proj", "attention.k_proj", "attention.v_proj"),
            ("_attention.key", "_attention.value")]
    nameset = set(names)
    for n in names:
        for trio in sets:
            for leaf in ("weight", "bias"):
                head = trio[0] + "." + leaf
                if n.endswith(head):
                    prefix = n[: -len(head)]
                    grp = tuple(prefix + t + "." + leaf for t in trio)
                    if all(g in nameset for g in grp):
                        for g in grp:
                            groups[g] = grp
    return groups


@dataclass
class Slot:
    name: str
    offset: int
    numel: int
    shape: tuple
    segment: str

    @property
    def has_grad(self) -> bool:
        return self.segment in ("enc", "head")


@dataclass(frozen=True)
class Form:
    source: str
    build: object
    prebuilt: bool = False


def _twice(wt, old):
    n, k = wt.shape
    dst = old if old is not None else torch.empty((n, 2 * k), device=wt.device, dtype=wt.dtype)
    ops.copy2d(dst[:, :k], wt)
    ops.copy2d(dst[:, k:], wt)
    return dst


def _mx8(src, old):
    return ops.mx8_quant(src, *(old or (None, None)))


FORMS = {"wt": Form("shadow", lambda w, old: ops.transpose16(w, old), prebuilt=True),
         "w2": Form("master", lambda p, old: ops.split_bf16(p, 2, 0, old), prebuilt=True),
         "wt2": Form("wt", _twice),
         "wq": Form("shadow", _mx8),
         "wtq": Form("wt", _mx8)}


class ParamStore:
    def __init__(self, model: torch.nn.Module, device, has_grad: set[str]):
        named = list(model.named_parameters())
        names = [n for n, _ in named]
        params = dict(named)
        groups = _fuse_groups(names)

        def seg_of(n, p):
            if not p.requires_grad:
                return "frozen"
            if n not in has_grad:
                return "nograd"
            return "enc" if ("text_encoder" in n or "audio_encoder" in n) else "head"

        order = {"enc": [], "head": [], "nograd": [], "frozen": []}
        seen = set()
        for n, p in named:
            if n in seen:
                continue
            grp = groups.get(n, (n,))
            segs = {seg_of(g, params[g]) for g in grp}
            if len(segs) != 1:
                grp = (n,)
            for g in grp:
                order[seg_of(g, params[g])].append(g)
                seen.add(g)
        self.slots: dict[str, Slot] = {}
        off = 0
        self.seg_range = {}
        for seg in ("enc", "head", "nograd", "frozen"):
            start = off
            for n in order[seg]:
                p = params[n]
                grp = groups.get(n)
                if grp is None or n == grp[0]:
                    off = (off + ALIGN - 1) // ALIGN * ALIGN
                self.slots[n] = Slot(n, off, p.numel(), tuple(p.shape), seg)
                off += p.numel()
            off = (off + ALIGN - 1) // ALIGN * ALIGN
            self.seg_range[seg] = (start, off)
        self.numel = off
        self.n_grad = self.seg_range["head"][1]
        self.device = torch.device(device)
        self.master = torch.zeros(self.numel, device=self.device, dtype=torch.float32)
        self.shadow = torch.zeros(self.numel, device=self.device, dtype=torch.bfloat16)
        self.grad = torch.zeros(self.n_grad, device=self.device, dtype=torch.float32)
        for n, s in self.slots.items():
            p = params[n]
            view = self.master[s.offset:s.offset + s.numel].view(s.shape)
            if p.device.type != "meta":
                with torch.no_grad():
                    view.copy_(p.detach().to(self.device, torch.float32))
            owner, leaf = (model.get_submodule(n.rsplit(".", 1)[0]), n.rsplit(".", 1)[1]) if "." in n \
                else (model, n)
            newp = torch.nn.Parameter(view, requires_grad=p.requires_grad)
            owner._parameters[leaf] = newp
            params[n] = newp
        self.params = params
        self._versions = {}
        self._cache = {form: {} for form in FORMS}
        self._members = {}
        self.opt_epoch = 0
        self._prebuilt = None
        self.sync_shadow(force=True)

    def p(self, name):
        s = self.slots[name]
        return self.master[s.offset:s.offset + s.numel].view(s.shape)

    def w(self, name, rows=None):
        s = self.slots[name]
        v = self.shadow[s.offset:s.offset + s.numel]
        return v.view(s.shape[0], -1) if rows is None else v.view(rows, -1)

    def g(self, name):
        s = self.slots[name]
        if not s.has_grad:
            return None
        return self.grad[s.offset:s.offset + s.numel].view(s.shape)

    def fused(self, first: str, count: int, which: str):
        s = self.slots[first]
        n = s.numel * count
        if which == "w":
            return self.shadow[s.offset:s.offset + n].view(s.shape[0] * count, -1)
        if which == "p":
            base = self.master[s.offset:s.offset + n]
            return base.view(s.shape[0] * count, *s.shape[1:]) if len(s.shape) > 1 else base
        if not s.has_grad:
            return None
        base = self.grad[s.offset:s.offset + n]
        return base.view(s.shape[0] * count, *s.shape[1:]) if len(s.shape) > 1 else base

    def _token(self, name, count):
        names = self._members.get((name, count))
        if names is None:
            s = self.slots[name]
            names = self._members[name, count] = (name,) if count == 1 else tuple(
                n for n, t in self.slots.items() if s.offset <= t.offset < s.offset + s.numel * count)
        return tuple(self.params[n]._version for n in names), self.opt_epoch if self.slots[name].has_grad else None

    def _form(self, form, name, count):
        f = FORMS[form]
        if f.source == "wt":
            src, _, token = self._form("wt", name, count)
        else:
            token = self._token(name, count)
        ent = self._cache[form].get((name, count))
        if ent is not None:
            if f.prebuilt:
                self._wait_prebuilt()
            if ent[1] == token:
                return ent
        if f.source != "wt":
            src = self.fused(name, count, "w" if f.source == "shadow" else "p").flatten(1)
        old, builds = (ent[0], ent[2]) if ent is not None else (None, 0)
        ent = self._cache[form][name, count] = (f.build(src, old), token, builds + 1)
        return ent

    def _wait_prebuilt(self):
        if self._prebuilt is None:
            return
        ev, stream, waited = self._prebuilt
        cur = torch.cuda.current_stream(self.device)
        if cur.cuda_stream != stream.cuda_stream and cur.cuda_stream not in waited:
            cur.wait_event(ev)
            waited.add(cur.cuda_stream)

    def cached(self, form: str) -> int:
        return len(self._cache[form])

    def wt(self, name: str, count: int = 1):
        return self._form("wt", name, count)[0]

    def w2(self, name: str, count: int = 1):
        return self._form("w2", name, count)[0]

    def wt2(self, name: str, count: int = 1):
        return self._form("wt2", name, count)[0]

    def wq(self, name: str, count: int = 1):
        return self._form("wq", name, count)[0]

    def wtq(self, name: str, count: int = 1):
        return self._form("wtq", name, count)[0]

    def _stale_prebuilt(self, inside=lambda slot: True):
        return [(form, *key) for form, f in FORMS.items() if f.prebuilt
                for key, ent in self._cache[form].items()
                if self.slots[key[0]].has_grad and ent[1][1] != self.opt_epoch and inside(self.slots[key[0]])]

    def refresh_transposes(self, stream):
        if stream is None or self.device.type != "cuda":
            return
        stale = self._stale_prebuilt()
        if not stale:
            return
        stream.wait_stream(torch.cuda.current_stream(self.device))
        self._prebuilt = None
        with torch.cuda.stream(stream):
            for key in stale:
                self._form(*key)
            ev = torch.cuda.Event()
            ev.record(stream)
        self._prebuilt = (ev, stream, set())

    def refresh_transposes_in(self, runs):
        if self.device.type != "cuda":
            return
        self._prebuilt = None
        for key in self._stale_prebuilt(lambda slot: any(a <= slot.offset < b for a, b in runs)):
            self._form(*key)

    def trainable_layer(self, name: str) -> bool:
        return self.slots[name].has_grad

    def sync_shadow(self, force=False):
        if self.device.type != "cuda":
            return
        for n, s in self.slots.items():
            v = self.params[n]._version
            if force or self._versions.get(n) != v:
                src = self.master[s.offset:s.offset + s.numel]
                dst = self.shadow[s.offset:s.offset + s.numel]
                ops.cast_bf16(src, dst)
                self._versions[n] = self.params[n]._version

    def mark_synced(self):
        for n in self.slots:
            self._versions[n] = self.params[n]._version
        self.opt_epoch += 1

    def attach_grads(self):
        names = [n for n, s in self.slots.items() if s.has_grad]
        reset = any(self.params[n].grad is None for n in names)
        if reset:
            self.grad.zero_()
            for n in names:
                self.params[n].grad = self.g(n)
        return reset
```

### speech_transcript_embeddings_amd/train.py

```python
from __future__ import annotations

import math

import torch
import torch.distributed as dist

from . import _lib, ops
from .model import EnhancedAudioTextModel

F32 = torch.float32


class LinearWarmupSchedule:

    def __init__(self, warmup: int, total: int):
        self.warmup, self.total, self.step_count = warmup, total, 0

    def factor(self, step=None):
        s = self.step_count if step is None else step
        if s < self.warmup:
            return s / max(1, self.warmup)
        return max(0.0, (self.total - s) / max(1, self.total - self.warmup))

    def step(self):
        self.step_count += 1


class FusedAdamW:

    def __init__(self, model: EnhancedAudioTextModel, lr=2.1e-3, encoder_lr_div=50.0, weight_decay=0.01,
                 betas=(0.9, 0.999), eps=1e-8, max_norm=1.0):
        st = model.store
        self.model = model
        self.store = st
        self.partial = getattr(model, "freeze_encoders", "partial") == "partial"
        div = encoder_lr_div if self.partial else 1.0
        self.groups = [{"range": st.seg_range["enc"], "lr": lr / div},
                       {"range": st.seg_range["head"], "lr": lr}]
        self.wd, self.betas, self.eps, self.max_norm = weight_decay, betas, eps, max_norm
        self.exp_avg = torch.zeros(st.n_grad, device=st.device, dtype=F32)
        self.exp_avg_sq = torch.zeros(st.n_grad, device=st.device, dtype=F32)
        self.sumsq = torch.zeros(1, device=st.device, dtype=torch.float64)
        self.sumsq_part = torch.zeros(ops.SUMSQ_PARTS, device=st.device, dtype=torch.float64)
        self.t = 0
        self.last_factor = 1.0
        self.tail = None

    def sync(self):
        if self.tail is not None:
            torch.cuda.current_stream(self.store.device).wait_event(self.tail)

    def _ref_groups(self):
        named = [(n, p) for n, p in self.model.named_parameters() if p.requires_grad]
        if not self.partial:
            return [[n for n, _ in named]]
        enc = [n for n, _ in named if "text_encoder" in n or "audio_encoder" in n]
        rest = [n for n, _ in named if not ("text_encoder" in n or "audio_encoder" in n)]
        return [enc, rest]

    def _group_hparams(self, gi):
        base = self.groups[0]["lr"] if (self.partial and gi == 0) else self.groups[1]["lr"]
        return {"lr": base * self.last_factor, "weight_decay": self.wd, "betas": tuple(self.betas), "eps": self.eps,
                "amsgrad": False, "maximize": False, "foreach": None, "capturable": False, "differentiable": False,
                "fused": None, "decoupled_weight_decay": True, "initial_lr": base}

    def state_dict(self, lr_factor: float | None = None):
        if lr_factor is not None:
            saved, self.last_factor = self.last_factor, lr_factor
            try:
                return self.state_dict()
            finally:
                self.last_factor = saved
        self.sync()
        st = self.store
        state, groups, idx = {}, [], 0
        for gi, names in enumerate(self._ref_groups()):
            ids = []
            for n in names:
                s = st.slots[n]
                if self.t > 0 and s.has_grad:
                    sl = slice(s.offset, s.offset + s.numel)
                    state[idx] = {"step": torch.tensor(float(self.t), dtype=F32),
                                  "exp_avg": self.exp_avg[sl].view(s.shape).clone(),
                                  "exp_avg_sq": self.exp_avg_sq[sl].view(s.shape).clone()}
                ids.append(idx)
                idx += 1
            groups.append({**self._group_hparams(gi), "params": ids})
        return {"state": state, "param_groups": groups}

    def load_state_dict(self, sd):
        st = self.store
        self.sync()
        ref = self._ref_groups()
        pgs = sd["param_groups"]
        if len(pgs) != len(ref) or any(len(g["params"]) != len(r) for g, r in zip(pgs, ref)):
            raise ValueError("optimizer state_dict does not match this model's parameter groups "
                             f"({[len(g['params']) for g in pgs]} vs {[len(r) for r in ref]})")
        steps = set()
        self.exp_avg.zero_()
        self.exp_avg_sq.zero_()
        for g, names in zip(pgs, ref):
            for i, n in zip(g["params"], names):
                ps = sd["state"].get(i)
                if ps is None:
                    continue
                s = st.slots[n]
                if not s.has_grad:
                    continue
                sl = slice(s.offset, s.offset + s.numel)
                self.exp_avg[sl].copy_(ps["exp_avg"].reshape(-1).to(self.exp_avg.device, F32))
                self.exp_avg_sq[sl].copy_(ps["exp_avg_sq"].reshape(-1).to(self.exp_avg_sq.device, F32))
                steps.add(int(float(ps["step"])))
        if len(steps) > 1:
            raise ValueError(f"parameters at different step counts {sorted(steps)}: not supported by the fused "
                             "optimizer (one shared step)")
        self.t = steps.pop() if steps else 0
        bases = [g.get("initial_lr", g["lr"]) for g in pgs]
        if self.partial:
            self.groups[0]["lr"], self.groups[1]["lr"] = bases[0], bases[1]
            self.last_factor = pgs[1]["lr"] / bases[1] if bases[1] else 1.0
        else:
            self.groups[0]["lr"] = self.groups[1]["lr"] = bases[0]
            self.last_factor = pgs[0]["lr"] / bases[0] if bases[0] else 1.0
        g0 = pgs[0]
        self.wd, self.betas, self.eps = float(g0["weight_decay"]), tuple(g0["betas"]), float(g0["eps"])

    def total_norm(self):
        self.sync()
        return math.sqrt(float(self.sumsq.item()))

    def step(self, lr_factor: float = 1.0, phases=None, on_phase=None):
        st = self.store
        self.t += 1
        self.last_factor = lr_factor
        self.sumsq.zero_()
        if self.max_norm is not None:
            ops.sumsq(st.grad[: st.n_grad], self.sumsq, self.sumsq_part)

        def upd(a, b, lr):
            ops.adamw(st.master[a:b], st.grad[a:b], self.exp_avg[a:b], self.exp_avg_sq[a:b], st.shadow[a:b],
                      lr=lr * lr_factor, beta1=self.betas[0], beta2=self.betas[1], eps=self.eps, wd=self.wd,
                      step=self.t, sumsq_acc=self.sumsq if self.max_norm is not None else None,
                      max_norm=self.max_norm or 1.0)
        events = {}
        if phases is None:
            for gr in self.groups:
                a, b = gr["range"]
                if b > a:
                    upd(a, b, gr["lr"])
            st.mark_synced()
            return events
        st.mark_synced()
        for name, runs in phases:
            for a, b in runs:
                gr = next(g for g in self.groups if g["range"][0] <= a and b <= g["range"][1])
                upd(a, b, gr["lr"])
            if on_phase is not None:
                on_phase(runs)
            ev = torch.cuda.Event()
            ev.record()
            events[name] = ev
        return events

    def zero_grad(self):
        self.sync()
        self.store.grad.zero_()


class GradSync:

    WORDS = "text_encoder.embeddings.word_embeddings.weight"
    STAGES = ("heads", "audio_layers", "audio", "text_layers", "text")

    def __init__(self, store, bucket_mb: int = 256, pad_id: int = 1, word_capacity: int | None = None):
        self.store = store
        self.bucket = max(1, bucket_mb * 1024 * 1024 // 4)
        self.pad_id = pad_id
        self.works = []
        self.sparse = None
        self.capacity = None if word_capacity is None else int(word_capacity)
        self.configured = word_capacity is not None
        self._agreed = False
        self._pending_cap = None
        self._cap_stream = None
        grad_slots = [sl for sl in store.slots.values() if sl.has_grad]

        ordered = sorted(grad_slots, key=lambda x: x.offset)

        def span(pred):
            runs, cur = [], None
            for x in ordered:
                if pred(x):
                    cur = [x.offset, x.offset + x.numel] if cur is None else [cur[0], x.offset + x.numel]
                elif cur is not None:
                    runs.append(tuple(cur))
                    cur = None
            if cur is not None:
                runs.append(tuple(cur))
            return runs

        words = store.slots.get(self.WORDS)
        self.words = words if words is not None and words.segment == "enc" else None
        self.ranges = {"heads": span(lambda x: x.segment == "head"),
                       "audio_layers": span(lambda x: x.segment == "enc" and
                                            x.name.startswith("audio_encoder.encoder.layers.")),
                       "audio": span(lambda x: x.segment == "enc" and x.name.startswith("audio_encoder.") and
                                     not x.name.startswith("audio_encoder.encoder.layers.")),
                       "text_layers": span(lambda x: x.segment == "enc" and
                                           x.name.startswith("text_encoder.encoder.layer.")),
                       "text": span(lambda x: x.segment == "enc" and x.name.startswith("text_encoder.") and
                                    not x.name.startswith("text_encoder.encoder.layer."))}
        if self.words is not None and self.ranges["text"]:
            w0, w1 = self.words.offset, self.words.offset + self.words.numel
            cut = []
            for a, b in self.ranges["text"]:
                cut += [r for r in ((a, min(b, w0)), (max(a, w1), b)) if r[1] > r[0]] if a < w1 and w0 < b else [(a, b)]
            self.ranges["text"] = cut
        cov = sorted(r for rs in self.ranges.values() for r in rs)
        for (a0, b0), (a1, b1) in zip(cov, cov[1:]):
            assert b0 <= a1, "gradient blocks overlap"
        for x in grad_slots:
            if self.words is not None and x.name == self.WORDS:
                continue
            inside = [k for k, rs in self.ranges.items()
                      if any(a <= x.offset and x.offset + x.numel <= b for a, b in rs)]
            assert len(inside) == 1, f"gradient slot {x.name} is in {len(inside)} sync blocks"
        self._flags = None

    @staticmethod
    def active():
        return dist.is_available() and dist.is_initialized() and dist.get_world_size() > 1

    def _avg_op(self):
        return dist.ReduceOp.AVG if dist.get_backend() == "nccl" else dist.ReduceOp.SUM

    def _reduce(self, ranges):
        g = self.store.grad
        ws = dist.get_world_size()
        op = self._avg_op()
        for a, b in ranges:
            for c in range(a, b, self.bucket):
                t = g[c:min(b, c + self.bucket)]
                if op == dist.ReduceOp.SUM:
                    t.mul_(1.0 / ws)
                self.works.append(dist.all_reduce(t, op=op, async_op=True))

    def ensure_capacity(self, n_ids: int) -> int:
        if not self.active() or self.words is None:
            return int(n_ids)
        if not self.configured:
            dev = self.store.device
            t = torch.tensor([int(n_ids)], dtype=torch.int64,
                             device=dev if dist.get_backend() == "nccl" and dev.type == "cuda" else "cpu")
            dist.all_reduce(t, op=dist.ReduceOp.MAX)
            self.capacity = int(t.item())
            self._agreed = True
            self._pending_cap = None
        elif n_ids > self.capacity:
            raise RuntimeError(f"{n_ids} token ids in one step exceed the word-table exchange capacity "
                               f"{self.capacity} (TrainStep(micro_batch=, max_text_length=) sets it)")
        return self.capacity

    def start_capacity(self, n_ids: int):
        if not self.active() or self.words is None:
            return
        dev = self.store.device
        if self.configured or not (dist.get_backend() == "nccl" and dev.type == "cuda"):
            self.ensure_capacity(n_ids)
            return
        if self._cap_stream is None:
            self._cap_stream = torch.cuda.Stream(device=dev)
        with torch.cuda.stream(self._cap_stream):
            t = torch.tensor([int(n_ids)], dtype=torch.int64, device=dev)
            dist.all_reduce(t, op=dist.ReduceOp.MAX, async_op=True).wait()
            host = torch.empty(1, dtype=torch.int64, pin_memory=True)
            host.copy_(t, non_blocking=True)
            ev = torch.cuda.Event()
            ev.record()
        self._pending_cap = (ev, host, t)
        self._agreed = True

    def _agreed_capacity(self) -> int:
        if self._pending_cap is not None:
            ev, host, _ = self._pending_cap
            ev.synchronize()
            self.capacity = int(host.item())
            self._pending_cap = None
        return self.capacity

    def _sparse_words(self, ids, cap_ids):
        st, sl = self.store, self.words
        D = sl.shape[1]
        g2 = st.grad[sl.offset:sl.offset + sl.numel].view(sl.shape)
        dev = st.device
        if self._flags is None:
            self._flags = torch.zeros(sl.shape[0], device=dev, dtype=torch.int32)
        cap = min(cap_ids, sl.shape[0])
        out_ids = torch.empty(cap, device=dev, dtype=torch.int32)
        rows = torch.empty(cap, D, device=dev, dtype=F32)
        count = torch.empty(1, device=dev, dtype=torch.int32)
        ops.rows_extract(ids, self.pad_id, g2, self._flags, out_ids, rows, count)
        ws = dist.get_world_size()
        all_ids = torch.empty(ws * cap, device=dev, dtype=torch.int32)
        all_rows = torch.empty(ws * cap, D, device=dev, dtype=F32)
        w1 = dist.all_gather_into_tensor(all_ids, out_ids, async_op=True)
        w2 = dist.all_gather_into_tensor(all_rows, rows, async_op=True)
        self.sparse = (g2, all_ids, all_rows, cap, ws, (w1, w2), (out_ids, rows))

    def sparse_pays(self, n_ids: int) -> bool:
        ws = dist.get_world_size()
        return ws * min(n_ids, self.words.shape[0]) < self.words.shape[0] // 2

    def stage_done(self, stage, ids=None):
        if not self.active():
            return
        self._reduce(self.ranges[stage])
        if stage == "text" and self.words is not None:
            if self.configured or not self._agreed:
                n = self.ensure_capacity(ids.numel() if ids is not None else 0)
            else:
                n = self._agreed_capacity()
            self._agreed = False
            if ids is not None and self.sparse_pays(n):
                self._sparse_words(ids, n)
            else:
                self._reduce([(self.words.offset, self.words.offset + self.words.numel)])

    def finish(self):
        for w in self.works:
            w.wait()
        self.works = []
        if self.sparse is not None:
            g2, all_ids, all_rows, cap, ws, waits, keep = self.sparse
            for w in waits:
                w.wait()
            if all_ids.is_cuda:
                cur = torch.cuda.current_stream(all_ids.device)
                for t in (all_ids, all_rows, *keep):
                    t.record_stream(cur)
            for r in range(ws):
                ops.rows_accumulate(g2, all_ids[r * cap:(r + 1) * cap], all_rows[r * cap:(r + 1) * cap], 1.0 / ws)
            self.sparse = None


class EmbeddingExchange:

    FORCE_COLLECTIVES = False

    def __init__(self, tau: float = 0.1, in_batch_weight: float = 0.0):
        self.tau, self.weight = float(tau), float(in_batch_weight)
        self.acc = None
        self.steps = 0
        self._pending = None

    @staticmethod
    def world():
        if dist.is_available() and dist.is_initialized():
            return dist.get_world_size(), dist.get_rank()
        return 1, 0

    def _collective(self, ws):
        return ws > 1 or (self.FORCE_COLLECTIVES and dist.is_available() and dist.is_initialized())

    def start(self, an, tn_all):
        ws, rank = self.world()
        B, P = an.shape
        NB = ws * B
        if not self._collective(ws):
            self._pending = (an, tn_all, [], B, 1, 0)
            return
        A_g = torch.empty(NB, P, device=an.device, dtype=F32)
        T_g = torch.empty(2 * NB, P, device=an.device, dtype=F32)
        works = [dist.all_gather_into_tensor(A_g, an, async_op=True),
                 dist.all_gather_into_tensor(T_g[:NB], tn_all[:B], async_op=True),
                 dist.all_gather_into_tensor(T_g[NB:], tn_all[B:], async_op=True)]
        self._pending = (A_g, T_g, works, B, ws, rank)

    def _wait(self):
        A_g, T_g, works, B, ws, rank = self._pending
        for w in works:
            w.wait()
        self._pending = (A_g, T_g, [], B, ws, rank)
        return A_g, T_g, B, ws, rank

    def in_batch(self, an, gscale, loss, dan, dtp):
        A_g, T_g, B, ws, rank = self._wait()
        NB = ws * B
        e = lambda *sh: torch.empty(sh, device=an.device, dtype=F32)
        S = e(B, NB)
        ops.similarity(an, T_g[:NB], S)
        dS = e(B, NB)
        ops.inbatch_ce(S, B, NB, rank * B, self.tau, self.weight, gscale, loss, dS)
        ops.rowmat(dS, T_g[:NB], dan)
        dT = torch.zeros(NB, an.shape[1], device=an.device, dtype=F32)
        ops.rowmat(dS, an, dT, transpose_x=True)
        if self._collective(ws):
            if dist.get_backend() == "gloo" and dT.is_cuda:
                mine = torch.empty(B, an.shape[1], dtype=F32)
                dist.reduce_scatter_tensor(mine, dT.cpu(), op=dist.ReduceOp.SUM, async_op=True).wait()
                mine = mine.to(dT.device)
            else:
                mine = e(B, an.shape[1])
                dist.reduce_scatter_tensor(mine, dT, op=dist.ReduceOp.SUM, async_op=True).wait()
            ops.axpby(dtp, mine)
        else:
            ops.axpby(dtp, dT)

    def finish(self, loss):
        if self._pending is None:
            return
        A_g, T_g, B, ws, rank = self._wait()
        self._pending = None
        NB = ws * B
        dev = A_g.device
        if self.acc is None:
            self.acc = torch.zeros(6, device=dev, dtype=torch.float64)
        S = torch.empty(NB, 2 * NB, device=dev, dtype=F32)
        ops.similarity(A_g, T_g, S)
        ops.pair_metrics(S, NB, self.tau, self.acc, losses=loss, loss_w=float(B))
        self.last_S = S
        self.steps += 1

    def epoch_metrics(self, reset: bool = True):
        ws, _ = self.world()
        if self.acc is None:
            if ws > 1:
                raise RuntimeError("epoch_metrics() before any finish() on this rank")
            return {}
        a = self.acc.cpu().tolist()
        if ws > 1:
            lsum = self.acc[5:6].clone()
            if dist.get_backend() == "gloo" and lsum.is_cuda:
                lsum = lsum.cpu()
            dist.all_reduce(lsum, op=dist.ReduceOp.SUM)
            a[5] = float(lsum.item())
        n = a[4]
        if n == 0:
            return {}
        out = {"loss": a[5] / n, "clean_similarity": a[0] / n, "corrupt_similarity": a[1] / n,
               "similarity_gap": (a[0] - a[1]) / n, "pair_accuracy": a[2] / n, "in_batch_top1": a[3] / n,
               "samples": int(n)}
        if reset:
            self.acc.zero_()
        return out


class TrainStep:

    def __init__(self, model: EnhancedAudioTextModel, lr=2.1e-3, warmup=100, total_steps=10000, temperature=0.1,
                 alignment_weight=0.5, corrupt_gamma=0.35, max_norm=1.0, pad_value=1.0, gather_embeddings=True,
                 accumulation_steps=1, in_batch_weight=0.0, micro_batch=None, max_text_length=None,
                 overlap_optimizer=False):
        self.model = model
        self.acc = max(1, int(accumulation_steps))
        self._micro = 0
        self._ids = []
        self.opt = FusedAdamW(model, lr=lr, max_norm=max_norm)
        self.sched = LinearWarmupSchedule(warmup, total_steps)
        cap = None
        if micro_batch is not None and max_text_length is not None:
            cap = 2 * int(micro_batch) * int(max_text_length) * self.acc
        self.gradsync = GradSync(model.store, pad_id=model.text_cfg.pad_token_id, word_capacity=cap)
        self.tau, self.aw, self.gamma = temperature, alignment_weight, corrupt_gamma
        self.pad_value = pad_value
        self.gather_embeddings = gather_embeddings or in_batch_weight > 0
        self.exchange = EmbeddingExchange(temperature, in_batch_weight) if self.gather_embeddings else None
        self.in_batch_weight = float(in_batch_weight)
        self.last = {}
        st = model.store
        self.overlap = bool(overlap_optimizer) and st.device.type == "cuda"
        self._opt_stream = torch.cuda.Stream(device=st.device) if self.overlap else None
        self._opt_tail = None
        if self.overlap:
            gs = self.gradsync
            text = gs.ranges["text"] + gs.ranges["text_layers"]
            if gs.words is not None:
                text = text + [(gs.words.offset, gs.words.offset + gs.words.numel)]
            self._phases = [("audio", gs.ranges["audio"]), ("text", sorted(text)),
                            ("late", gs.ranges["audio_layers"] + gs.ranges["heads"])]
        self._sync_layerdrop_seed()

    def _sync_layerdrop_seed(self):
        seed = torch.randint(0, 2**62, (1,), dtype=torch.int64)
        if GradSync.active():
            t = seed.to(self.model.store.device) if dist.get_backend() == "nccl" else seed.clone()
            dist.broadcast(t, src=0)
            seed = t.cpu()
        self.model.engine.layerdrop_gen = torch.Generator().manual_seed(int(seed.item()))

    def features(self, wav, lengths):
        if self.model.engine.raw_audio:
            from .wav2vec2 import wave_normalize
            B, n = wav.shape
            lengths = lengths.to(device=wav.device, dtype=torch.int32)
            mask = (torch.arange(n, device=wav.device).view(1, n) < lengths.view(B, 1)).to(torch.int64)
            return wave_normalize(wav, lengths), mask
        n = int(wav.shape[1])
        T = ((1 + (n - 400) // 160) + 1) // 2
        lengths = lengths.to(device=wav.device, dtype=torch.int32, non_blocking=True)
        return ops.fbank(wav, lengths, T, pad_value=self.pad_value, mask_mode=0)

    def __call__(self, wav, lengths, ids_pos, mask_pos, ids_neg, mask_neg, sampling_rate=None):
        host = lengths.tolist() if lengths.device.type == "cpu" else None
        if sampling_rate is not None and int(sampling_rate) != 16000:
            wav, lengths = ops.resample(wav, lengths.to(device=wav.device, dtype=torch.int32), int(sampling_rate))
            if host is not None:
                host = [ops.resampled_length(n, sampling_rate) for n in host]
        feats, amask = self.features(wav, lengths)
        batch = {"input_ids_pos": ids_pos, "attention_mask_pos": mask_pos, "input_ids_neg": ids_neg,
                 "attention_mask_neg": mask_neg, "input_values": feats, "attention_mask_audio": amask}
        if host is not None:
            from .features import num_frames
            batch["audio_lengths"] = host if self.model.engine.raw_audio else [num_frames(int(x)) for x in host]
        return self.step_batch(batch)

    def step_batch(self, batch):
        m = self.model
        m.train()
        st = m.store
        st.sync_shadow()
        eng = m.engine
        if self._micro + 1 == self.acc:
            n_ids = batch["input_ids_pos"].numel() + batch["input_ids_neg"].numel()
            self.gradsync.start_capacity(n_ids + sum(int(t.numel()) for t in (self._ids if self._micro else [])))
        tf_p, tf_n, af, align, ctx = eng.forward(batch, True)
        B, P = af.shape
        e = lambda *s: torch.empty(s, device=st.device, dtype=F32)
        tn_all = e(2 * B, P)
        an = e(B, P)
        nrm = e(3 * B)
        ops.l2norm_fwd(tf_p, tn_all[:B], nrm[:B])
        ops.l2norm_fwd(tf_n, tn_all[B:], nrm[B:2 * B])
        ops.l2norm_fwd(af, an, nrm[2 * B:])
        S = e(B, 2 * B)
        ops.similarity(an, tn_all, S)
        sp, sn, loss = e(B), e(B), e(1)
        L = align.shape[1] if align is not None else 0
        ops.pair_loss_fwd(S, B, align, B, L, self.tau, self.aw, self.gamma, sp, sn, loss)
        if self.exchange is not None:
            self.exchange.start(an, tn_all)
        dsp, dsn = e(B), e(B)
        dal = e(B, L) if align is not None else None
        gscale = None if self.acc == 1 else torch.full((1,), 1.0 / self.acc, device=st.device, dtype=F32)
        ops.pair_loss_bwd(sp, sn, align, B, L, self.tau, self.aw, self.gamma, gscale, dsp, dsn, dal)
        dan, dtp, dtn = e(B, P), e(B, P), e(B, P)
        ops.pair_sim_bwd(an, tn_all[:B], tn_all[B:], dsp, dsn, dan, dtp, dtn)
        if self.in_batch_weight > 0:
            self.exchange.in_batch(an, gscale, loss, dan, dtp)
        g_tp, g_tn, g_a = e(B, P), e(B, P), e(B, P)
        ops.l2norm_bwd(tn_all[:B], nrm[:B], dtp, g_tp)
        ops.l2norm_bwd(tn_all[B:], nrm[B:2 * B], dtn, g_tn)
        ops.l2norm_bwd(an, nrm[2 * B:], dan, g_a)
        if self._micro == 0:
            self._await_optimizer()
            st.grad.zero_()
            self._ids = []
        self._ids.append(ctx["t_ids"].reshape(-1))
        self._micro += 1
        final = self._micro == self.acc
        ids_all = self._ids[0] if len(self._ids) == 1 else torch.cat(self._ids)
        eng.backward(ctx, g_tp, g_tn, g_a, dal,
                     stage_done=(lambda stg: self.gradsync.stage_done(stg, ids_all)) if final else None)
        self.last = {"loss": loss, "s_pos": sp, "s_neg": sn}
        if self.exchange is not None:
            self.exchange.finish(loss)
        if final:
            self._optimizer_step()
        return loss

    def epoch_metrics(self):
        self._await_optimizer()
        out = self.exchange.epoch_metrics() if self.exchange is not None else {}
        out["optimizer_steps"] = self.opt.t
        return out

    def _optimizer_step(self):
        eng = self.model.engine
        if self.overlap:
            main = torch.cuda.current_stream(self.model.store.device)
            self._opt_stream.wait_stream(main)
            with torch.cuda.stream(self._opt_stream):
                self.gradsync.finish()
                eng.param_events = self.opt.step(self.sched.factor(), phases=self._phases,
                                                 on_phase=self.model.store.refresh_transposes_in)
                self.sched.step()
                self._opt_tail = torch.cuda.Event()
                self._opt_tail.record()
            self.opt.tail = self._opt_tail
        else:
            self.gradsync.finish()
            self.opt.step(self.sched.factor())
            self.sched.step()
            self.model.store.refresh_transposes(eng._side_stream())
        self._micro = 0
        self._ids = []

    def _await_optimizer(self):
        if self._opt_tail is not None:
            torch.cuda.current_stream(self.model.store.device).wait_event(self._opt_tail)

    def sync(self):
        self._await_optimizer()

    def flush(self):
        if self._micro == 0:
            return False
        ids_all = torch.cat(self._ids)
        for stg in GradSync.STAGES:
            self.gradsync.stage_done(stg, ids_all)
        self._optimizer_step()
        return True

    def optimizer_state_dict(self):
        self._await_optimizer()
        return self.opt.state_dict(lr_factor=self.sched.factor())

    def load_optimizer_state_dict(self, sd):
        self._await_optimizer()
        self.opt.load_state_dict(sd)
        self.sched.step_count = self.opt.t


def synthetic_batch(B, n_samples, L, vocab=250000, device="cuda", seed=0, rank=0):
    g = torch.Generator(device=device).manual_seed(seed * 1000 + rank)
    t = torch.arange(n_samples, device=device, dtype=F32) / 16000.0
    wav = 0.1 * torch.randn(B, n_samples, device=device, generator=g)
    freqs = 100 + 2900 * torch.rand(B, 3, 1, device=device, generator=g)
    wav = wav + 0.05 * torch.sin(2 * math.pi * freqs * t.view(1, 1, -1)).sum(1)
    wav = wav.clamp_(-1, 1).contiguous()
    lengths = torch.full((B,), n_samples, device=device, dtype=torch.int32)
    ids = torch.randint(5, vocab, (B, L), device=device, generator=g)
    ids[:, 0], ids[:, -1] = 0, 2
    corrupt = torch.rand(B, L, device=device, generator=g) < 0.2
    corrupt[:, 0] = False
    corrupt[:, -1] = False
    neg = torch.where(corrupt, torch.randint(5, vocab, (B, L), device=device, generator=g), ids)
    mask = torch.ones(B, L, device=device, dtype=torch.int64)
    return wav, lengths, ids, mask, neg.contiguous(), mask.clone()


__all__ = ["TrainStep", "FusedAdamW", "LinearWarmupSchedule", "GradSync", "EmbeddingExchange", "synthetic_batch",
           "_lib"]
```

Measured before the change: 490.6 pairs/s.

## Track dirty word-embedding rows to sparsify grad zeroing, norm, and AdamW

Adds per-row dirty flags for the XLM-R word-embedding gradient, set by the embedding backward and the sparse row accumulation. Gradient zeroing, the clip-norm sum of squares and AdamW then skip untouched rows. AdamW keeps a 'live' mask of rows whose moments are nonzero, so rows with zero gradient and zero moments get only the decay update. This avoids streaming the full 250k×768 table's grad, m and v every step, at the cost of extra bookkeeping and the risk that the live-mask rebuilds fall out of sync.

```diff
diff --git a/include/ste.h b/include/ste.h
--- a/include/ste.h
+++ b/include/ste.h
@@ -231,6 +231,19 @@
 int ste_adamw(float* p, const float* g, float* m, float* v, void* p_bf16, int64_t n, float lr, float beta1,
               float beta2, float eps, float wd, int step, const double* sumsq, float max_norm, void* stream);
 
+int ste_text_embed_bwd_rows(const int64_t* ids, const int32_t* pos_ids, const float* dout, int B, int L, int D,
+                            int pad_idx, float* dword, float* dpos, float* dtype0, float* ws, int64_t ws_floats,
+                            int32_t* dirty, void* stream);
+int ste_rows_accumulate_rows(float* grad, int D, const int32_t* ids, const float* rows, int cap, float scale,
+                             int32_t* dirty, void* stream);
+int ste_zero_rows(float* g, int64_t n, int64_t t0, int rows, int D, int32_t* dirty, void* stream);
+int ste_sumsq_rows(const float* g, int64_t n, int64_t t0, int rows, int D, const int32_t* dirty, double* acc,
+                   double* part, void* stream);
+int ste_adamw_rows(float* p, const float* g, float* m, float* v, void* p_bf16, int rows, int D, const int32_t* dirty,
+                   int32_t* live, float lr, float beta1, float beta2, float eps, float wd, int step,
+                   const double* sumsq, float max_norm, void* stream);
+int ste_rows_live(const float* m, const float* v, int rows, int D, int32_t* live, void* stream);
+
 int ste_split_bf16(const float* x, int64_t ldx, int64_t rows, int K, void* y, int nblk, int lo_mask, void* stream);
 int ste_cast_f32_bf16(const float* x, void* y, int64_t n, void* stream);
 int ste_axpby2d(float* y, int64_t ldy, const float* x, int64_t ldx, int64_t rows, int cols, float alpha, float beta,
diff --git a/speech_transcript_embeddings_amd/_lib.py b/speech_transcript_embeddings_amd/_lib.py
--- a/speech_transcript_embeddings_amd/_lib.py
+++ b/speech_transcript_embeddings_amd/_lib.py
@@ -207,7 +207,15 @@
     "ste_sumsq": (c_int, [c_void_p, c_int64, c_void_p, c_void_p, c_void_p]),
     "ste_adamw": (c_int, [c_void_p, c_void_p, c_void_p, c_void_p, c_void_p, c_int64, c_float, c_float, c_float,
                           c_float, c_float, c_int, c_void_p, c_float, c_void_p]),
-    "ste_cast_f32_bf16": (c_int, [c_void_p, c_void_p, c_int64, c_void_p]),
+    "ste_text_embed_bwd_rows": (c_int, [c_void_p, c_void_p, c_void_p, c_int, c_int, c_int, c_int, c_void_p, c_void_p,
+                                        c_void_p, c_void_p, c_int64, c_void_p, c_void_p]),
+    "ste_rows_accumulate_rows": (c_int, [c_void_p, c_int, c_void_p, c_void_p, c_int, c_float, c_void_p, c_void_p]),
+    "ste_zero_rows": (c_int, [c_void_p, c_int64, c_int64, c_int, c_int, c_void_p, c_void_p]),
+    "ste_sumsq_rows": (c_int, [c_void_p, c_int64, c_int64, c_int, c_int, c_void_p, c_void_p, c_void_p, c_void_p]),
+    "ste_adamw_rows": (c_int, [c_void_p, c_void_p, c_void_p, c_void_p, c_void_p, c_int, c_int, c_void_p, c_void_p,
+                               c_float, c_float, c_float, c_float, c_float, c_int, c_void_p, c_float, c_void_p]),
+    "ste_rows_live": (c_int, [c_void_p, c_void_p, c_int, c_int, c_void_p, c_void_p]),
+    "ste_cast_f32_bf16":(c_int, [c_void_p, c_void_p, c_int64, c_void_p]),
     "ste_colsum": (c_int, [c_void_p, c_int, c_int64, c_int, c_int64, c_void_p, c_void_p, c_int64, c_void_p]),
     "ste_colsum_ws_floats": (c_int64, [c_int64, c_int]),
     "ste_rowsum_ordered": (c_int, [c_void_p, c_int64, c_int, c_int, c_void_p, c_void_p]),
diff --git a/speech_transcript_embeddings_amd/csrc/embed_optim.hip b/speech_transcript_embeddings_amd/csrc/embed_optim.hip
--- a/speech_transcript_embeddings_amd/csrc/embed_optim.hip
+++ b/speech_transcript_embeddings_amd/csrc/embed_optim.hip
@@ -36,7 +36,8 @@
 __global__ __launch_bounds__(EMB_WAVES * 64) void embed_rows_ordered_kernel(const IdT* __restrict__ ids, int rows,
                                                                           int D, int pad,
                                                                           const float* __restrict__ dout,
-                                                                          float* __restrict__ table) {
+                                                                          float* __restrict__ table,
+                                                                          int32_t* __restrict__ dirty) {
   extern __shared__ int sids[];
   const bool in_lds = rows <= EMB_LDS_IDS;
   if (in_lds)
@@ -72,17 +73,40 @@
     const int c = (lane + 64 * q) * 4;
     if (c < D) *reinterpret_cast<f32x4*>(dst + c) += acc[q];
   }
-}
-
-__global__ __launch_bounds__(NT) void sumsq_kernel(const float* g, int64_t n, double* acc, double* part) {
+  if (dirty && lane == 0) dirty[id] = 1;
+}
+
+template <bool ROWS>
+__global__ __launch_bounds__(NT) void sumsq_kernel(const float* g, int64_t n, double* acc, double* part, int64_t t0,
+                                                 int64_t t1, int D, const int32_t* __restrict__ dirty) {
   __shared__ double red[NT / 64];
   double s = 0.0;
   float sf = 0.f;
   int cnt = 0;
-  for (int64_t i = ((int64_t)blockIdx.x * NT + threadIdx.x) * 4; i < n; i += (int64_t)gridDim.x * NT * 4) {
+  const int64_t stride = (int64_t)gridDim.x * NT * 4;
+  const int qs = ROWS ? (int)(stride / D) : 0, rs = ROWS ? (int)(stride % D) : 0;
+  int row = -1, col = 0;
+  for (int64_t i = ((int64_t)blockIdx.x * NT + threadIdx.x) * 4; i < n; i += stride) {
+    bool skip = false;
+    if constexpr (ROWS) {
+      if (i >= t0 && i < t1) {
+        if (row < 0) {
+          row = (int)((i - t0) / D);
+          col = (int)((i - t0) - (int64_t)row * D);
+        }
+        skip = dirty[row] == 0;
+      }
+      if (row >= 0) {
+        row += qs;
+        col += rs;
+        if (col >= D) { col -= D; ++row; }
+      }
+    }
     if (i + 3 < n) {
-      const f32x4 v = *reinterpret_cast<const f32x4*>(g + i);
-      sf += v[0] * v[0] + v[1] * v[1] + v[2] * v[2] + v[3] * v[3];
+      if (!skip) {
+        const f32x4 v = *reinterpret_cast<const f32x4*>(g + i);
+        sf += v[0] * v[0] + v[1] * v[1] + v[2] * v[2] + v[3] * v[3];
+      }
     } else {
       for (int64_t j = i; j < n; ++j) sf += g[j] * g[j];
     }
@@ -192,6 +216,140 @@
   }
 }
 
+constexpr int ROW_WAVES = NT / 64;
+template <bool NTL>
+__global__ __launch_bounds__(NT) void adamw_rows_kernel(float* __restrict__ p, const float* __restrict__ g,
+                                                      float* __restrict__ m, float* __restrict__ v,
+                                                      bf16* __restrict__ pb, int rows, int D,
+                                                      const int32_t* __restrict__ dirty, int32_t* __restrict__ live,
+                                                      float lr, float b1, float b2, float eps, float wd, float bc1,
+                                                      float bc2_sqrt, const double* sumsq, float max_norm) {
+  float coef = 1.f;
+  if (sumsq) {
+    const float tn = (float)sqrt(*sumsq);
+    coef = fminf(1.f, max_norm / (tn + 1e-6f));
+  }
+  const float step = lr / bc1;
+  const float decay = 1.f - lr * wd;
+  auto upd4 = [&](f32x4& pv, const f32x4& gv, f32x4& mv, f32x4& vv) {
+#pragma unroll
+    for (int e = 0; e < 4; ++e) {
+      float pe = pv[e], me = mv[e], ve = vv[e];
+      adamw_elem(pe, gv[e], me, ve, coef, decay, b1, b2, step, bc2_sqrt, eps);
+      pv[e] = pe;
+      mv[e] = me;
+      vv[e] = ve;
+    }
+  };
+  auto ld = [](const float* q) -> f32x4 {
+    if constexpr (NTL) return __builtin_nontemporal_load(reinterpret_cast<const f32x4*>(q));
+    else return *reinterpret_cast<const f32x4*>(q);
+  };
+  auto st = [](float* q, f32x4 x) {
+    if constexpr (NTL) __builtin_nontemporal_store(x, reinterpret_cast<f32x4*>(q));
+    else *reinterpret_cast<f32x4*>(q) = x;
+  };
+  const int lane = threadIdx.x & 63, nw = gridDim.x * ROW_WAVES;
+  for (int r = blockIdx.x * ROW_WAVES + (threadIdx.x >> 6); r < rows; r += nw) {
+    const bool act = __builtin_amdgcn_readfirstlane(live[r] | dirty[r]) != 0;
+    const int64_t base = (int64_t)r * D;
+    if (act) {
+      for (int c0 = lane * 4; c0 < D; c0 += 512) {
+        f32x4 pv[2], gv[2], mv[2], vv[2];
+#pragma unroll
+        for (int q = 0; q < 2; ++q) {
+          const int c = c0 + 256 * q;
+          if (c < D) {
+            pv[q] = ld(p + base + c);
+            gv[q] = ld(g + base + c);
+            mv[q] = ld(m + base + c);
+            vv[q] = ld(v + base + c);
+          }
+        }
+#pragma unroll
+        for (int q = 0; q < 2; ++q) {
+          const int c = c0 + 256 * q;
+          if (c < D) {
+            upd4(pv[q], gv[q], mv[q], vv[q]);
+            st(p + base + c, pv[q]);
+            st(m + base + c, mv[q]);
+            st(v + base + c, vv[q]);
+            if (pb) store_bf16x4(pb + base + c, pv[q]);
+          }
+        }
+      }
+    } else {
+      const f32x4 zero = {0.f, 0.f, 0.f, 0.f};
+      for (int c0 = lane * 4; c0 < D; c0 += 1024) {
+        f32x4 pv[4];
+#pragma unroll
+        for (int q = 0; q < 4; ++q) {
+          const int c = c0 + 256 * q;
+          if (c < D) pv[q] = ld(p + base + c);
+        }
+#pragma unroll
+        for (int q = 0; q < 4; ++q) {
+          const int c = c0 + 256 * q;
+          if (c < D) {
+            f32x4 mv = zero, vv = zero;
+            upd4(pv[q], zero, mv, vv);
+            st(p + base + c, pv[q]);
+            if (pb) store_bf16x4(pb + base + c, pv[q]);
+          }
+        }
+      }
+    }
+    if (act && lane == 0) live[r] = 1;
+  }
+}
+
+typedef uint32_t u32x4 __attribute__((ext_vector_type(4)));
+__global__ __launch_bounds__(NT) void rows_live_kernel(const float* __restrict__ m, const float* __restrict__ v,
+                                                     int rows, int D, int32_t* __restrict__ live) {
+  const int lane = threadIdx.x & 63, nw = gridDim.x * ROW_WAVES;
+  for (int r = blockIdx.x * ROW_WAVES + (threadIdx.x >> 6); r < rows; r += nw) {
+    const int64_t base = (int64_t)r * D;
+    uint32_t any = 0;
+    for (int c = lane * 4; c < D; c += 256) {
+      const u32x4 a = *reinterpret_cast<const u32x4*>(m + base + c);
+      const u32x4 b = *reinterpret_cast<const u32x4*>(v + base + c);
+      any |= a[0] | a[1] | a[2] | a[3] | b[0] | b[1] | b[2] | b[3];
+    }
+    const uint64_t set = __ballot(any != 0);
+    if (lane == 0) live[r] = set != 0;
+  }
+}
+
+__global__ __launch_bounds__(NT) void zero_rows_kernel(float* __restrict__ g, int64_t n, int64_t t0, int rows, int D,
+                                                     int32_t* __restrict__ dirty, int row_blocks) {
+  const f32x4 zero = {0.f, 0.f, 0.f, 0.f};
+  const int64_t tn = (int64_t)rows * D;
+  if ((int)blockIdx.x < row_blocks) {
+    const int lane = threadIdx.x & 63, nw = row_blocks * ROW_WAVES;
+    for (int r0 = (blockIdx.x * ROW_WAVES + (threadIdx.x >> 6)) * 64; r0 < rows; r0 += nw * 64) {
+      const int r = r0 + lane;
+      const bool f = r < rows && dirty[r] != 0;
+      uint64_t mk = __ballot(f);
+      if (f) dirty[r] = 0;
+      while (mk) {
+        const int k = __builtin_ctzll(mk);
+        mk &= mk - 1;
+        float* dst = g + t0 + (int64_t)(r0 + k) * D;
+        for (int c = lane * 4; c < D; c += 256) *reinterpret_cast<f32x4*>(dst + c) = zero;
+      }
+    }
+    return;
+  }
+  const int64_t nd = n - tn, nb = gridDim.x - row_blocks;
+  for (int64_t k = (((int64_t)blockIdx.x - row_blocks) * NT + threadIdx.x) * 4; k < nd; k += nb * NT * 4) {
+    if (k + 3 < nd) {
+      *reinterpret_cast<f32x4*>(g + (k < t0 ? k : k + tn)) = zero;
+    } else {
+      for (int64_t j = k; j < nd; ++j) g[j < t0 ? j : j + tn] = 0.f;
+    }
+  }
+}
+
 inline unsigned grid_for(int64_t n) {
   int64_t b = (n / 4 + NT - 1) / NT;
   if (b > 8192) b = 8192;
@@ -234,7 +392,7 @@
   if (threadIdx.x == 0) flags[id] = 0;
 }
 __global__ __launch_bounds__(NT) void rows_accumulate_kernel(float* grad, int D, const int32_t* ids, const float* rows,
-                                                            float scale) {
+                                                            float scale, int32_t* dirty) {
   const int sidx = blockIdx.x;
   const int id = ids[sidx];
   if (id < 0) return;
@@ -242,6 +400,7 @@
   const float* src = rows + (int64_t)sidx * D;
   for (int c = threadIdx.x * 4; c < D; c += NT * 4)
     *reinterpret_cast<f32x4*>(dst + c) += *reinterpret_cast<const f32x4*>(src + c) * scale;
+  if (dirty && threadIdx.x == 0) dirty[id] = 1;
 }
 }
 
@@ -261,14 +420,19 @@
   return 0;
 }
 
+extern "C" int ste_rows_accumulate_rows(float* grad, int D, const int32_t* ids, const float* rows, int cap,
+                                        float scale, int32_t* dirty, void* stream) {
+  if (cap <= 0 || (D & 3) || !grad || !ids || !rows) return STE_ERR_ARG;
+  hipLaunchKernelGGL(rows_accumulate_kernel, dim3(cap), dim3(NT), 0, (hipStream_t)stream, grad, D, ids, rows, scale,
+                     dirty);
+  STE_CHECK_LAUNCH();
+  return 0;
+}
+
 extern "C" int ste_rows_accumulate(float* grad, int D, const int32_t* ids, const float* rows, int cap, float scale,
                                    void* stream) {
-  if (cap <= 0 || (D & 3) || !grad || !ids || !rows) return STE_ERR_ARG;
-  hipLaunchKernelGGL(rows_accumulate_kernel, dim3(cap), dim3(NT), 0, (hipStream_t)stream, grad, D, ids, rows, scale);
-  STE_CHECK_LAUNCH();
-  return 0;
-}
-
+  return ste_rows_accumulate_rows(grad, D, ids, rows, cap, scale, nullptr, stream);
+}
 
 
 extern "C" int ste_text_embed_fwd(const int64_t* ids, int B, int L, int D, int pad_idx, const float* word,
@@ -284,9 +448,9 @@
   return ste_colsum_ws_floats((int64_t)B * L, D);
 }
 
-extern "C" int ste_text_embed_bwd(const int64_t* ids, const int32_t* pos_ids, const float* dout, int B, int L, int D,
-                                  int pad_idx, float* dword, float* dpos, float* dtype0, float* ws, int64_t ws_floats,
-                                  void* stream) {
+extern "C" int ste_text_embed_bwd_rows(const int64_t* ids, const int32_t* pos_ids, const float* dout, int B, int L,
+                                       int D, int pad_idx, float* dword, float* dpos, float* dtype0, float* ws,
+                                       int64_t ws_floats, int32_t* dirty, void* stream) {
   const int rows = B * L;
   if (rows <= 0 || (D & 3) || D > 1024) return STE_ERR_SHAPE;
   hipStream_t s = (hipStream_t)stream;
@@ -294,29 +458,78 @@
   const size_t lds = rows <= EMB_LDS_IDS ? (size_t)rows * 4 : 0;
   if (dword) {
     hipLaunchKernelGGL(embed_rows_ordered_kernel<int64_t>, grid, dim3(EMB_WAVES * 64), lds, s, ids, rows, D, pad_idx,
-                       dout, dword);
+                       dout, dword, dirty);
     STE_CHECK_LAUNCH();
   }
   if (dpos) {
     hipLaunchKernelGGL(embed_rows_ordered_kernel<int32_t>, grid, dim3(EMB_WAVES * 64), lds, s, pos_ids, rows, D,
-                       pad_idx, dout, dpos);
+                       pad_idx, dout, dpos, (int32_t*)nullptr);
     STE_CHECK_LAUNCH();
   }
   if (dtype0) return ste_colsum(dout, 0, rows, D, D, dtype0, ws, ws_floats, stream);
   return 0;
 }
 
-extern "C" int ste_sumsq(const float* g, int64_t n, double* acc, double* part, void* stream) {
+extern "C" int ste_text_embed_bwd(const int64_t* ids, const int32_t* pos_ids, const float* dout, int B, int L, int D,
+                                  int pad_idx, float* dword, float* dpos, float* dtype0, float* ws, int64_t ws_floats,
+                                  void* stream) {
+  return ste_text_embed_bwd_rows(ids, pos_ids, dout, B, L, D, pad_idx, dword, dpos, dtype0, ws, ws_floats, nullptr,
+                                 stream);
+}
+
+static int sumsq_launch(const float* g, int64_t n, int64_t t0, int rows, int D, const int32_t* dirty, double* acc,
+                        double* part, void* stream) {
   if (n <= 0) return 0;
   if (((uintptr_t)g) & 15) return STE_ERR_ARG;
   unsigned gr = grid_for(n);
   if (gr > 2048) gr = 2048;
-  hipLaunchKernelGGL(sumsq_kernel, dim3(gr), dim3(NT), 0, (hipStream_t)stream, g, n, acc, part);
+  if (dirty)
+    hipLaunchKernelGGL(sumsq_kernel<true>, dim3(gr), dim3(NT), 0, (hipStream_t)stream, g, n, acc, part, t0,
+                       t0 + (int64_t)rows * D, D, dirty);
+  else
+    hipLaunchKernelGGL(sumsq_kernel<false>, dim3(gr), dim3(NT), 0, (hipStream_t)stream, g, n, acc, part, (int64_t)0,
+                       (int64_t)0, 1, (const int32_t*)nullptr);
   STE_CHECK_LAUNCH();
   if (part) {
     hipLaunchKernelGGL(sumsq_final_kernel, dim3(1), dim3(64), 0, (hipStream_t)stream, part, (int)gr, acc);
     STE_CHECK_LAUNCH();
   }
+  return 0;
+}
+
+extern "C" int ste_sumsq(const float* g, int64_t n, double* acc, double* part, void* stream) {
+  return sumsq_launch(g, n, 0, 0, 1, nullptr, acc, part, stream);
+}
+
+static bool table_ok(int64_t n, int64_t t0, int rows, int D) {
+  return rows > 0 && D > 0 && !(D & 3) && t0 >= 0 && !(t0 & 3) && t0 + (int64_t)rows * D <= n;
+}
+
+extern "C" int ste_sumsq_rows(const float* g, int64_t n, int64_t t0, int rows, int D, const int32_t* dirty,
+                              double* acc, double* part, void* stream) {
+  if (!dirty || !table_ok(n, t0, rows, D)) return STE_ERR_ARG;
+  return sumsq_launch(g, n, t0, rows, D, dirty, acc, part, stream);
+}
+
+extern "C" int ste_zero_rows(float* g, int64_t n, int64_t t0, int rows, int D, int32_t* dirty, void* stream) {
+  if (!g || !dirty || (((uintptr_t)g) & 15) || !table_ok(n, t0, rows, D)) return STE_ERR_ARG;
+  int row_blocks = (rows + ROW_WAVES * 64 - 1) / (ROW_WAVES * 64);
+  if (row_blocks > 2048) row_blocks = 2048;
+  unsigned dense = grid_for(n - (int64_t)rows * D);
+  if (dense > 2048) dense = 2048;
+  hipLaunchKernelGGL(zero_rows_kernel, dim3(row_blocks + dense), dim3(NT), 0, (hipStream_t)stream, g, n, t0, rows, D,
+                     dirty, row_blocks);
+  STE_CHECK_LAUNCH();
+  return 0;
+}
+
+extern "C" int ste_rows_live(const float* m, const float* v, int rows, int D, int32_t* live, void* stream) {
+  if (rows <= 0 || D <= 0 || (D & 3) || !m || !v || !live || ((((uintptr_t)m) | ((uintptr_t)v)) & 15))
+    return STE_ERR_ARG;
+  int blocks = (rows + ROW_WAVES - 1) / ROW_WAVES;
+  if (blocks > 8192) blocks = 8192;
+  hipLaunchKernelGGL(rows_live_kernel, dim3(blocks), dim3(NT), 0, (hipStream_t)stream, m, v, rows, D, live);
+  STE_CHECK_LAUNCH();
   return 0;
 }
 
@@ -339,3 +552,25 @@
   STE_CHECK_LAUNCH();
   return 0;
 }
+
+extern "C" int ste_adamw_rows(float* p, const float* g, float* m, float* v, void* p_bf16, int rows, int D,
+                              const int32_t* dirty, int32_t* live, float lr, float beta1, float beta2, float eps,
+                              float wd, int step, const double* sumsq, float max_norm, void* stream) {
+  if (rows <= 0) return 0;
+  if (step < 1 || D <= 0 || (D & 3) || !dirty || !live) return STE_ERR_ARG;
+  if ((((uintptr_t)p) | ((uintptr_t)g) | ((uintptr_t)m) | ((uintptr_t)v)) & 15) return STE_ERR_ARG;
+  if (p_bf16 && (((uintptr_t)p_bf16) & 7)) return STE_ERR_ARG;
+  const float bc1 = 1.f - powf(beta1, (float)step);
+  const float bc2s = sqrtf(1.f - powf(beta2, (float)step));
+  int blocks = (rows + ROW_WAVES - 1) / ROW_WAVES;
+  if (blocks > 8192) blocks = 8192;
+  const char* ent = STE_AB_ENV("STE_ADAMW_NT");
+  if (!(ent && ent[0] == '0'))
+    hipLaunchKernelGGL(adamw_rows_kernel<true>, dim3(blocks), dim3(NT), 0, (hipStream_t)stream, p, g, m, v,
+                       (bf16*)p_bf16, rows, D, dirty, live, lr, beta1, beta2, eps, wd, bc1, bc2s, sumsq, max_norm);
+  else
+    hipLaunchKernelGGL(adamw_rows_kernel<false>, dim3(blocks), dim3(NT), 0, (hipStream_t)stream, p, g, m, v,
+                       (bf16*)p_bf16, rows, D, dirty, live, lr, beta1, beta2, eps, wd, bc1, bc2s, sumsq, max_norm);
+  STE_CHECK_LAUNCH();
+  return 0;
+}
diff --git a/speech_transcript_embeddings_amd/engine.py b/speech_transcript_embeddings_amd/engine.py
--- a/speech_transcript_embeddings_amd/engine.py
+++ b/speech_transcript_embeddings_amd/engine.py
@@ -720,7 +720,8 @@
         self._ln_bwd(dx, ctx["t_emb"], ctx["t_st"], "text_encoder.embeddings.LayerNorm", dx=demb,
                      in_drop_p=ctx["t_hp"], in_seed=_site_seed(ctx["t_seed"], 1))
         if gw is not None or gp is not None or gt is not None:
-            ops.text_embed_bwd(ctx["t_ids"], ctx["t_pos"], demb, c.pad_token_id, gw, gp, gt)
+            ops.text_embed_bwd(ctx["t_ids"], ctx["t_pos"], demb, c.pad_token_id, gw, gp, gt,
+                               dirty=s.word_dirty if gw is not None else None)
 
     def _w32(self, name):
         w = self.s.p(name)
diff --git a/speech_transcript_embeddings_amd/ops.py b/speech_transcript_embeddings_amd/ops.py
--- a/speech_transcript_embeddings_amd/ops.py
+++ b/speech_transcript_embeddings_amd/ops.py
@@ -738,12 +738,13 @@
          ptr(pos_ids), _s())
 
 
-def text_embed_bwd(ids, pos_ids, dout, pad_idx, dword, dpos, dtype0):
+def text_embed_bwd(ids, pos_ids, dout, pad_idx, dword, dpos, dtype0, dirty=None):
     B, L = ids.shape
     ws = _red_ws(dout.device, int(fn("ste_text_embed_bwd_ws_floats")(B, L, dout.shape[-1]))) if dtype0 is not None \
         else None
-    call("ste_text_embed_bwd", ptr(ids), ptr(pos_ids), ptr(dout), B, L, dout.shape[-1], pad_idx, ptr(dword),
-         ptr(dpos), ptr(dtype0), *_ws_args(ws), _s())
+    assert dirty is None or (dirty.dtype == torch.int32 and dword is not None and dirty.numel() == dword.shape[0])
+    call("ste_text_embed_bwd_rows", ptr(ids), ptr(pos_ids), ptr(dout), B, L, dout.shape[-1], pad_idx, ptr(dword),
+         ptr(dpos), ptr(dtype0), *_ws_args(ws), ptr(dirty), _s())
 
 
 SUMSQ_PARTS = 2048
@@ -761,6 +762,46 @@
     _traced("adamw", nbytes, lambda: call("ste_adamw", ptr(p), ptr(g), ptr(m), ptr(v), ptr(p_bf16), p.numel(), float(lr),
                                           float(beta1), float(beta2), float(eps), float(wd), int(step), ptr(sumsq_acc),
                                           float(max_norm), _s()))
+
+
+def _flag_rows(flags, rows):
+    assert flags.dtype == torch.int32 and flags.is_contiguous() and flags.numel() == rows
+
+
+def zero_rows(g, t0, rows, D, dirty):
+    _flag_rows(dirty, rows)
+    call("ste_zero_rows", ptr(g), g.numel(), int(t0), int(rows), int(D), ptr(dirty), _s())
+
+
+def sumsq_rows(g, t0, rows, D, dirty, acc, part=None):
+    if ATOMIC_SUMS:
+        part = None
+    assert part is None or (part.dtype == torch.float64 and part.numel() >= SUMSQ_PARTS)
+    _flag_rows(dirty, rows)
+    nbytes = 4 * (g.numel() - (rows - int(dirty.ne(0).sum())) * D) if HBM_TRACE is not None else 0
+    _traced("sumsq", nbytes, lambda: call("ste_sumsq_rows", ptr(g), g.numel(), int(t0), int(rows), int(D), ptr(dirty),
+                                          ptr(acc), ptr(part), _s()))
+
+
+def adamw_rows(p, g, m, v, p_bf16, rows, D, dirty, live, *, lr, beta1, beta2, eps, wd, step, sumsq_acc=None,
+               max_norm=1.0):
+    assert p.numel() == rows * D
+    _flag_rows(dirty, rows)
+    _flag_rows(live, rows)
+    nbytes = 0
+    if HBM_TRACE is not None:
+        act = int((dirty | live).ne(0).sum())
+        sh = 2 if p_bf16 is not None else 0
+        nbytes = D * (act * (28 + sh) + (rows - act) * (8 + sh))
+    _traced("adamw", nbytes, lambda: call("ste_adamw_rows", ptr(p), ptr(g), ptr(m), ptr(v), ptr(p_bf16), int(rows), int(D),
+                                          ptr(dirty), ptr(live), float(lr), float(beta1), float(beta2), float(eps),
+                                          float(wd), int(step), ptr(sumsq_acc), float(max_norm), _s()))
+
+
+def rows_live(m, v, rows, D, live):
+    assert m.numel() == rows * D and v.numel() == rows * D
+    _flag_rows(live, rows)
+    call("ste_rows_live", ptr(m), ptr(v), int(rows), int(D), ptr(live), _s())
 
 
 def cast_bf16(x, y):
@@ -817,5 +858,7 @@
          ptr(out_ids), ptr(rows), out_ids.numel(), ptr(count), _s())
 
 
-def rows_accumulate(grad2d, ids, rows, scale):
-    call("ste_rows_accumulate", ptr(grad2d), grad2d.shape[1], ptr(ids), ptr(rows), ids.numel(), float(scale), _s())
+def rows_accumulate(grad2d, ids, rows, scale, dirty=None):
+    assert dirty is None or (dirty.dtype == torch.int32 and dirty.numel() == grad2d.shape[0])
+    call("ste_rows_accumulate_rows", ptr(grad2d), grad2d.shape[1], ptr(ids), ptr(rows), ids.numel(), float(scale),
+         ptr(dirty), _s())
diff --git a/speech_transcript_embeddings_amd/store.py b/speech_transcript_embeddings_amd/store.py
--- a/speech_transcript_embeddings_amd/store.py
+++ b/speech_transcript_embeddings_amd/store.py
@@ -7,6 +7,7 @@
 from . import ops
 
 ALIGN = 8
+WORDS = "text_encoder.embeddings.word_embeddings.weight"
 
 
 def _fuse_groups(names):
@@ -114,6 +115,13 @@
         self.master = torch.zeros(self.numel, device=self.device, dtype=torch.float32)
         self.shadow = torch.zeros(self.numel, device=self.device, dtype=torch.bfloat16)
         self.grad = torch.zeros(self.n_grad, device=self.device, dtype=torch.float32)
+        w = self.slots.get(WORDS)
+        self.word_table = self.word_dirty = None
+        if (w is not None and w.segment == "enc" and len(w.shape) == 2 and w.shape[1] % 4 == 0
+                and self.device.type == "cuda"):
+            self.word_table = (w.offset, w.shape[0], w.shape[1])
+            self.word_dirty = torch.zeros(w.shape[0], device=self.device, dtype=torch.int32)
+        self._grad_version = self.grad._version
         for n, s in self.slots.items():
             p = params[n]
             view = self.master[s.offset:s.offset + s.numel].view(s.shape)
@@ -265,6 +273,31 @@
         reset = any(self.params[n].grad is None for n in names)
         if reset:
             self.grad.zero_()
+            self.mark_words_dirty()
             for n in names:
                 self.params[n].grad = self.g(n)
         return reset
+
+    def words_dirty(self):
+        if self.word_dirty is not None and self.grad._version != self._grad_version:
+            self.mark_words_dirty()
+        return self.word_dirty
+
+    def mark_words_dirty(self):
+        if self.word_dirty is not None:
+            self.word_dirty.fill_(1)
+        self._grad_version = self.grad._version
+
+    def own_grad_write(self, write):
+        clean = self.grad._version == self._grad_version
+        out = write()
+        if clean:
+            self._grad_version = self.grad._version
+        return out
+
+    def zero_grad(self):
+        d = self.words_dirty()
+        if d is None:
+            self.grad.zero_()
+        else:
+            ops.zero_rows(self.grad, *self.word_table, d)
diff --git a/speech_transcript_embeddings_amd/train.py b/speech_transcript_embeddings_amd/train.py
--- a/speech_transcript_embeddings_amd/train.py
+++ b/speech_transcript_embeddings_amd/train.py
@@ -1,6 +1,7 @@
 from __future__ import annotations
 
 import math
+import os
 
 import torch
 import torch.distributed as dist
@@ -42,6 +43,10 @@
         self.exp_avg_sq = torch.zeros(st.n_grad, device=st.device, dtype=F32)
         self.sumsq = torch.zeros(1, device=st.device, dtype=torch.float64)
         self.sumsq_part = torch.zeros(ops.SUMSQ_PARTS, device=st.device, dtype=torch.float64)
+        self.word_live = None
+        if getattr(st, "word_table", None) is not None:
+            self.word_live = torch.zeros(st.word_table[1], device=st.device, dtype=torch.int32)
+        self._live_versions = self._moment_versions()
         self.t = 0
         self.last_factor = 1.0
         self.tail = None
@@ -49,6 +54,19 @@
     def sync(self):
         if self.tail is not None:
             torch.cuda.current_stream(self.store.device).wait_event(self.tail)
+
+    def _moment_versions(self):
+        return self.exp_avg._version, self.exp_avg_sq._version
+
+    def rebuild_live(self):
+        t0, rows, D = self.store.word_table
+        ops.rows_live(self.exp_avg[t0:t0 + rows * D], self.exp_avg_sq[t0:t0 + rows * D], rows, D, self.word_live)
+        self._live_versions = self._moment_versions()
+
+    def _live(self):
+        if self._live_versions != self._moment_versions():
+            self.rebuild_live()
+        return self.word_live
 
     def _ref_groups(self):
         named = [(n, p) for n, p in self.model.named_parameters() if p.requires_grad]
@@ -124,24 +142,48 @@
             self.last_factor = pgs[0]["lr"] / bases[0] if bases[0] else 1.0
         g0 = pgs[0]
         self.wd, self.betas, self.eps = float(g0["weight_decay"]), tuple(g0["betas"]), float(g0["eps"])
+        if self.word_live is not None:
+            self.rebuild_live()
 
     def total_norm(self):
         self.sync()
         return math.sqrt(float(self.sumsq.item()))
 
-    def step(self, lr_factor: float = 1.0, phases=None, on_phase=None):
+    def step(self, lr_factor: float = 1.0, phases=None, on_phase=None, sparse_words=False):
         st = self.store
         self.t += 1
         self.last_factor = lr_factor
         self.sumsq.zero_()
+        tab = st.word_table if sparse_words and self.word_live is not None else None
+        if tab is not None:
+            dirty, live = st.words_dirty(), self._live()
+            t0, t1 = tab[0], tab[0] + tab[1] * tab[2]
+        elif self.word_live is not None:
+            self._live_versions = None
         if self.max_norm is not None:
-            ops.sumsq(st.grad[: st.n_grad], self.sumsq, self.sumsq_part)
+            if tab is not None:
+                ops.sumsq_rows(st.grad[: st.n_grad], *tab, dirty, self.sumsq, self.sumsq_part)
+            else:
+                ops.sumsq(st.grad[: st.n_grad], self.sumsq, self.sumsq_part)
+        hyper = dict(beta1=self.betas[0], beta2=self.betas[1], eps=self.eps, wd=self.wd, step=self.t,
+                     sumsq_acc=self.sumsq if self.max_norm is not None else None, max_norm=self.max_norm or 1.0)
+
+        def dense(a, b, lr):
+            if b > a:
+                ops.adamw(st.master[a:b], st.grad[a:b], self.exp_avg[a:b], self.exp_avg_sq[a:b], st.shadow[a:b],
+                          lr=lr * lr_factor, **hyper)
 
         def upd(a, b, lr):
-            ops.adamw(st.master[a:b], st.grad[a:b], self.exp_avg[a:b], self.exp_avg_sq[a:b], st.shadow[a:b],
-                      lr=lr * lr_factor, beta1=self.betas[0], beta2=self.betas[1], eps=self.eps, wd=self.wd,
-                      step=self.t, sumsq_acc=self.sumsq if self.max_norm is not None else None,
-                      max_norm=self.max_norm or 1.0)
+            if tab is None or b <= t0 or t1 <= a:
+                dense(a, b, lr)
+            elif a <= t0 and t1 <= b:
+                dense(a, t0, lr)
+                ops.adamw_rows(st.master[t0:t1], st.grad[t0:t1], self.exp_avg[t0:t1], self.exp_avg_sq[t0:t1],
+                               st.shadow[t0:t1], tab[1], tab[2], dirty, live, lr=lr * lr_factor, **hyper)
+                dense(t1, b, lr)
+            else:
+                dense(a, b, lr)
+                self._live_versions = None
         events = {}
         if phases is None:
             for gr in self.groups:
@@ -164,7 +206,10 @@
 
     def zero_grad(self):
         self.sync()
-        self.store.grad.zero_()
+        if self.word_live is not None:
+            self.store.zero_grad()
+        else:
+            self.store.grad.zero_()
 
 
 class GradSync:
@@ -174,6 +219,7 @@
 
     def __init__(self, store, bucket_mb: int = 256, pad_id: int = 1, word_capacity: int | None = None):
         self.store = store
+        self._rows = store if getattr(store, "word_dirty", None) is not None else None
         self.bucket = max(1, bucket_mb * 1024 * 1024 // 4)
         self.pad_id = pad_id
         self.works = []
@@ -241,9 +287,12 @@
         for a, b in ranges:
             for c in range(a, b, self.bucket):
                 t = g[c:min(b, c + self.bucket)]
-                if op == dist.ReduceOp.SUM:
-                    t.mul_(1.0 / ws)
-                self.works.append(dist.all_reduce(t, op=op, async_op=True))
+
+                def reduce(t=t):
+                    if op == dist.ReduceOp.SUM:
+                        t.mul_(1.0 / ws)
+                    return dist.all_reduce(t, op=op, async_op=True)
+                self.works.append(reduce() if self._rows is None else self._rows.own_grad_write(reduce))
 
     def ensure_capacity(self, n_ids: int) -> int:
         if not self.active() or self.words is None:
@@ -324,6 +373,8 @@
             if ids is not None and self.sparse_pays(n):
                 self._sparse_words(ids, n)
             else:
+                if self._rows is not None:
+                    self._rows.mark_words_dirty()
                 self._reduce([(self.words.offset, self.words.offset + self.words.numel)])
 
     def finish(self):
@@ -338,8 +389,10 @@
                 cur = torch.cuda.current_stream(all_ids.device)
                 for t in (all_ids, all_rows, *keep):
                     t.record_stream(cur)
+            mark = () if self._rows is None else (self._rows.word_dirty,)
             for r in range(ws):
-                ops.rows_accumulate(g2, all_ids[r * cap:(r + 1) * cap], all_rows[r * cap:(r + 1) * cap], 1.0 / ws)
+                ops.rows_accumulate(g2, all_ids[r * cap:(r + 1) * cap], all_rows[r * cap:(r + 1) * cap], 1.0 / ws,
+                                    *mark)
             self.sparse = None
 
 
@@ -450,8 +503,10 @@
     def __init__(self, model: EnhancedAudioTextModel, lr=2.1e-3, warmup=100, total_steps=10000, temperature=0.1,
                  alignment_weight=0.5, corrupt_gamma=0.35, max_norm=1.0, pad_value=1.0, gather_embeddings=True,
                  accumulation_steps=1, in_batch_weight=0.0, micro_batch=None, max_text_length=None,
-                 overlap_optimizer=False):
+                 overlap_optimizer=False, sparse_words=True):
         self.model = model
+        self.sparse_words = (bool(sparse_words) and getattr(model.store, "word_table", None) is not None
+                             and os.environ.get("STE_SPARSE_WORDS", "1") != "0")
         self.acc = max(1, int(accumulation_steps))
         self._micro = 0
         self._ids = []
@@ -553,7 +608,10 @@
         ops.l2norm_bwd(an, nrm[2 * B:], dan, g_a)
         if self._micro == 0:
             self._await_optimizer()
-            st.grad.zero_()
+            if self.sparse_words:
+                st.zero_grad()
+            else:
+                st.grad.zero_()
             self._ids = []
         self._ids.append(ctx["t_ids"].reshape(-1))
         self._micro += 1
@@ -582,14 +640,15 @@
             with torch.cuda.stream(self._opt_stream):
                 self.gradsync.finish()
                 eng.param_events = self.opt.step(self.sched.factor(), phases=self._phases,
-                                                 on_phase=self.model.store.refresh_transposes_in)
+                                                 on_phase=self.model.store.refresh_transposes_in,
+                                                 sparse_words=self.sparse_words)
                 self.sched.step()
                 self._opt_tail = torch.cuda.Event()
                 self._opt_tail.record()
             self.opt.tail = self._opt_tail
         else:
             self.gradsync.finish()
-            self.opt.step(self.sched.factor())
+            self.opt.step(self.sched.factor(), sparse_words=self.sparse_words)
             self.sched.step()
             self.model.store.refresh_transposes(eng._side_stream())
         self._micro = 0
```

Measured after the change: 494.5 pairs/s, median of 6. Within noise of the previous version (+0.8%).
